# agent-charon/MinGraph-UNet

Hardware: AMD Instinct MI355X
Metric: segmented Mpix/sec, full MinGraph-UNet forward (U-Net + patch-graph GAT), 512x512 batch (higher is better)
Workload: dtype f32

## Files before the change

### include/mgunet.h

```cpp
#ifndef MGUNET_H
#define MGUNET_H

#include <stddef.h>
#include <stdint.h>

#ifdef __cplusplus
extern "C" {
#endif

#define MGU_OK 0
#define MGU_ERR_INVALID -1
#define MGU_ERR_HIP -2
#define MGU_ERR_STATE -3
#define MGU_ERR_NOMEM -4

#define MGU_DTYPE_F32 0
#define MGU_DTYPE_BF16 1

typedef struct mgu_ctx mgu_ctx;

typedef struct {
  const char* name;
  const void* ptr;
  int64_t numel;
} mgu_tensor_desc;

int mgu_create(int device_id, mgu_ctx** out);
void mgu_destroy(mgu_ctx* ctx);
const char* mgu_last_error(mgu_ctx* ctx);
const char* mgu_version(void);

int mgu_unet_configure(mgu_ctx* ctx, int in_channels, int num_classes, int init_features, int depth, int dtype);
int64_t mgu_unet_param_count(mgu_ctx* ctx);
int mgu_unet_load_weights(mgu_ctx* ctx, const mgu_tensor_desc* named, int n, void* hip_stream);
int mgu_unet_refresh_weights(mgu_ctx* ctx, void* hip_stream);

int mgu_unet_workspace_bytes(mgu_ctx* ctx, int B, int H, int W, int training, size_t* out);
int mgu_unet_reserve(mgu_ctx* ctx, int B, int H, int W, int training);
int mgu_unet_forward(mgu_ctx* ctx, const void* x_dev, int B, int H, int W,
                     int64_t xs_n, int64_t xs_c, int64_t xs_h, int64_t xs_w,
                     void* logits_dev, void* const* cat_dev, void* const* feat_dev,
                     int training, void* hip_stream);
int mgu_conv2d_nhwc(mgu_ctx* ctx, const void* in_dev, int B, int H, int W, int Cin, const void* w_oihw_dev,
                    const void* bias_dev, const void* scale_dev, const void* shift_dev, int Cout, int ksize,
                    int relu, void* out_dev, int ld_out, int c_off, void* hip_stream);
typedef struct mgu_conv_weights mgu_conv_weights;
int mgu_conv2d_prepare(mgu_ctx* ctx, const void* w_oihw_dev, int Cout, int Cin, int ksize, mgu_conv_weights** out, void* hip_stream);
void mgu_conv2d_release(mgu_ctx* ctx, mgu_conv_weights* w);
int mgu_conv2d_prepared_nhwc(mgu_ctx* ctx, const mgu_conv_weights* w, const void* in_dev, int B, int H, int W, const void* bias_dev,
                             const void* scale_dev, const void* shift_dev, int relu, void* out_dev, int ld_out, int c_off,
                             void* hip_stream);
int mgu_conv_transpose2x2_nhwc(mgu_ctx* ctx, const void* in_dev, int B, int H, int W, int Cin, const void* w_iohw_dev,
                               const void* bias_dev, int Cout, void* out_dev, int ld_out, int c_off, void* hip_stream);
int mgu_maxpool2x2_nhwc(mgu_ctx* ctx, const void* in_dev, int ld_in, int B, int H, int W, int C, void* out_dev,
                        void* hip_stream);
int mgu_argmax_classes(mgu_ctx* ctx, const void* logits_dev, int64_t npix, int num_classes,
                       int64_t* pred_dev, void* hip_stream);

int64_t mgu_unet_param_offset(mgu_ctx* ctx, const char* name);
int mgu_cross_entropy(mgu_ctx* ctx, const void* logits_dev, const int64_t* labels_dev, int64_t npix, int num_classes,
                      float grad_scale, void* dlogits_dev, float* loss_dev, void* hip_stream);
int mgu_sync_check(mgu_ctx* ctx, void* hip_stream);
int mgu_unet_backward(mgu_ctx* ctx, const void* dlogits_dev, void* flat_grad_dev, void* hip_stream);
int mgu_unet_train_record_dims(mgu_ctx* ctx, const char* layer, int* B_out, int* H_out, int* W_out, int* Cin_out, int* Cout_out);
int mgu_unet_train_record_copy(mgu_ctx* ctx, const char* layer, void* in_dev, void* z_dev, void* y_dev, void* mean_dev, void* invstd_dev,
                               void* hip_stream);
int mgu_conv2d_wgrad_nhwc(mgu_ctx* ctx, const void* in_dev, int ld_in, const void* dz_dev, int B, int H, int W, int Cin, int Cout,
                          int ksize, void* dw_oihw_dev, void* hip_stream);
int mgu_conv2d_dgrad_nhwc(mgu_ctx* ctx, const void* dz_dev, const void* w_oihw_dev, int B, int H, int W, int Cin, int Cout, int ksize,
                          void* din_dev, int ld_out, void* hip_stream);
int mgu_conv_transpose2x2_wgrad_nhwc(mgu_ctx* ctx, const void* in_dev, const void* dout_dev, int ld_d, int c_off, int B, int H, int W,
                                     int Cin, int Cout, void* dw_iohw_dev, void* dbias_dev, void* hip_stream);
int mgu_conv_transpose2x2_dgrad_nhwc(mgu_ctx* ctx, const void* dout_dev, int ld_d, int c_off, const void* w_iohw_dev, int B, int H,
                                     int W, int Cin, int Cout, void* din_dev , void* hip_stream);
int mgu_bn_relu_train_nhwc(mgu_ctx* ctx, const void* z_dev, const void* gamma_dev, const void* beta_dev, int64_t M, int C, void* y_dev,
                           int ld_y, void* mean_dev, void* invstd_dev, void* run_mean_dev, void* run_var_dev, void* hip_stream);
int mgu_bn_relu_backward_nhwc(mgu_ctx* ctx, const void* dy_dev, int ld_dy, const void* z_dev, const void* gamma_dev, const void* beta_dev,
                              const void* mean_dev, const void* invstd_dev, int64_t M, int C, void* dz_dev, void* dgamma_dev,
                              void* dbeta_dev, void* dbias_dev, void* hip_stream);
int mgu_conv_bn_relu_train_nhwc(mgu_ctx* ctx, const void* in_dev, int ld_in, int B, int H, int W, int Cin, const void* w_oihw_dev,
                                const void* bias_dev, const void* gamma_dev, const void* beta_dev, int Cout, void* z_dev, void* y_dev,
                                int ld_y, void* pooled_dev, void* mean_dev, void* invstd_dev, void* run_mean_dev, void* run_var_dev,
                                int* stats_fused_out, int* pool_fused_out, void* hip_stream);
int mgu_bn_relu_conv_backward_nhwc(mgu_ctx* ctx, const void* in_dev, int ld_in, const void* z_dev, const void* dy_dev, int ld_dy,
                                   const void* gamma_dev, const void* beta_dev, const void* mean_dev, const void* invstd_dev,
                                   const void* w_oihw_dev, int B, int H, int W, int Cin, int Cout, void* dz_dev, void* dgamma_dev,
                                   void* dbeta_dev, void* dbias_dev, void* dw_oihw_dev, void* din_dev, int ld_din, void* hip_stream);
int mgu_reduction_slots_absmax(mgu_ctx* ctx, double* absmax_out, void* hip_stream);
int mgu_maxpool2x2_backward_nhwc(mgu_ctx* ctx, const void* y_dev, int ld_y, const void* dpool_dev, void* dskip_dev, int ld_d, int B, int H,
                                 int W, int C, void* hip_stream);

int mgu_adam_step(mgu_ctx* ctx, void* flat_param_dev, const void* flat_grad_dev, void* exp_avg_dev, void* exp_avg_sq_dev,
                  int64_t n, float lr, double beta1, double beta2, float eps, float weight_decay, int step,
                  float grad_scale, void* hip_stream);

int mgu_sgd_step(mgu_ctx* ctx, void* flat_param_dev, const void* flat_grad_dev, void* momentum_buf_dev, int64_t n, float lr,
                 float momentum, float weight_decay, int step, float grad_scale, void* hip_stream);

#define MGU_OPTIM_CTRL_BYTES 64
#define MGU_OPTIM_ADAM 0
#define MGU_OPTIM_ADAMW 1
#define MGU_OPTIM_SGD 2
typedef struct {
  int kind;
  float lr;
  double beta1, beta2;
  float eps, weight_decay;
  float momentum;
  float grad_scale;
  float max_norm;
  int skip_nonfinite;
  float ema_decay;
  int ema_warmup;
} mgu_optim_desc;
int64_t mgu_grad_norm_chunk(int64_t n);
int mgu_grad_norm_blocks(int64_t n);
int mgu_grad_norm(mgu_ctx* ctx, const void* grad_dev, int64_t n, float grad_scale, void* ctrl_dev, void* hip_stream);
int mgu_optim_step(mgu_ctx* ctx, const mgu_optim_desc* desc, void* flat_param_dev, const void* flat_grad_dev, void* exp_avg_dev,
                   void* exp_avg_sq_dev, void* ema_dev, void* ctrl_dev, int64_t n, void* hip_stream);
int mgu_grad_accumulate(mgu_ctx* ctx, void* acc_dev, const void* grad_dev, int64_t n, int first, void* hip_stream);

#define MGU_COMM_ID_BYTES 128
int mgu_comm_get_unique_id(void* id_out );
int mgu_comm_init_rank(mgu_ctx* ctx, const void* id , int rank, int world_size);
int mgu_comm_destroy(mgu_ctx* ctx);
void* mgu_comm_handle(mgu_ctx* ctx);
int mgu_comm_world_size(mgu_ctx* ctx);
int mgu_allreduce_grads(mgu_ctx* ctx, void* flat_grad_dev, int64_t n, void* rccl_comm, void* hip_stream);
int mgu_unet_backward_allreduce(mgu_ctx* ctx, const void* dlogits_dev, void* flat_grad_dev, void* hip_stream);

int mgu_unet_request_patch_mean(mgu_ctx* ctx, int patch, void* out_dev);

int mgu_csr_transpose_device(mgu_ctx* ctx, const int32_t* rowptr_dev, const int32_t* col_dev, int64_t E, int num_nodes,
                             int32_t* rowptr_src_dev, int32_t* eid_src_dev, int32_t* tgt_of_edge_dev, void* hip_stream);
int mgu_gat_layer_backward(mgu_ctx* ctx, const void* X_dev, int N, int Fin, const int32_t* rowptr_dev, const int32_t* col_dev, int64_t E,
                           const int32_t* rowptr_src_dev, const int32_t* eid_src_dev, const int32_t* tgt_of_edge_dev,
                           const int32_t* graph_ptr_dev, int num_graphs, const void* W_dev, const void* a_dev, int heads, int Fout_head,
                           int concat, float alpha, const void* dout_dev, void* dX_dev, void* dW_dev, void* da_dev, void* hip_stream);
int mgu_dropout_mask(mgu_ctx* ctx, unsigned long long seed, unsigned long long stream, int64_t n, float p, void* mask_dev, void* hip_stream);
int mgu_gat_layer_forward_train(mgu_ctx* ctx, const void* X_dev, int N, int Fin, const int32_t* rowptr_dev, const int32_t* col_dev, int64_t E,
                                const int32_t* graph_ptr_dev, int num_graphs, const void* W_dev, const void* a_dev, int heads, int Fout_head,
                                int concat, float alpha, const void* edge_mask_dev, const void* out_mask_dev, void* out_dev, void* hip_stream);
int mgu_gat_layer_backward_train(mgu_ctx* ctx, const void* X_dev, int N, int Fin, const int32_t* rowptr_dev, const int32_t* col_dev, int64_t E,
                                 const int32_t* rowptr_src_dev, const int32_t* eid_src_dev, const int32_t* tgt_of_edge_dev,
                                 const int32_t* graph_ptr_dev, int num_graphs, const void* W_dev, const void* a_dev, int heads, int Fout_head,
                                 int concat, float alpha, const void* edge_mask_dev, const void* out_mask_dev, const void* dout_dev,
                                 void* dX_dev, void* dW_dev, void* da_dev, void* hip_stream);

int mgu_patch_graph_build(int H, int W, int patch, int64_t* coo, int32_t* rowptr, int32_t* col,
                          int64_t* E_out, int* nph_out, int* npw_out);
int mgu_coo_to_csr(const int64_t* coo, int64_t E, int num_nodes, int32_t* rowptr, int32_t* col);
int mgu_coo_to_csr_device(mgu_ctx* ctx, const int64_t* coo_dev, int64_t E, int num_nodes, int32_t* rowptr_dev, int32_t* col_dev,
                          int* status_dev, void* hip_stream);
int mgu_patch_mean(mgu_ctx* ctx, const void* feat_dev, int feat_dtype , int B, int H, int W, int C,
                   int patch, void* out_dev, void* hip_stream);

int mgu_gat_layer_forward(mgu_ctx* ctx, const void* X_dev, int N, int Fin,
                          const int32_t* rowptr_dev, const int32_t* col_dev, int64_t E,
                          const int32_t* graph_ptr_dev, int num_graphs,
                          const void* W_dev, const void* a_dev, int heads, int Fout_head,
                          int concat, float alpha, void* out_dev, void* hip_stream);

typedef struct mgu_gat_weights mgu_gat_weights;
int mgu_gat_prepare(mgu_ctx* ctx, const void* W_dev, const void* a_dev, int heads, int Fout_head, int Fin, int has_edges,
                    mgu_gat_weights** out, void* hip_stream);
void mgu_gat_release(mgu_ctx* ctx, mgu_gat_weights* w);
int mgu_gat_layer_forward_prepared(mgu_ctx* ctx, const mgu_gat_weights* w, const void* X_dev, int N, const int32_t* rowptr_dev,
                                   const int32_t* col_dev, int64_t E, const int32_t* graph_ptr_dev, int num_graphs, int concat,
                                   float alpha, void* out_dev, void* hip_stream);

int mgu_ncut_edge_weights(mgu_ctx* ctx, const float* feats_dev, int N, int D, const int64_t* edge_index_dev, int64_t E,
                          float* w_dev, void* hip_stream);
int mgu_ncut_forward(mgu_ctx* ctx, const float* feats_dev, int N, int D, const int32_t* rowptr_src_dev,
                     const int32_t* col_tgt_dev, int64_t E, const float* assign_dev, int K, int assign_is_logits,
                     float* soft_dev, int32_t* hard_dev, float* loss_dev, void* hip_stream);
int mgu_ncut_backward(mgu_ctx* ctx, const float* feats_dev, int N, int D, const int32_t* rowptr_src_dev, const int32_t* col_tgt_dev,
                      const int32_t* rowptr_tgt_dev, const int32_t* col_src_dev, int64_t E, const float* soft_dev, int K,
                      int assign_is_logits, const float* gloss_dev, const float* gsoft_dev, float* dassign_dev, float* dfeats_dev,
                      void* hip_stream);
int mgu_relu_backward(mgu_ctx* ctx, const float* dy_dev, const float* y_dev, int64_t n, float* dz_dev, void* hip_stream);

int mgu_region_mean_pool(mgu_ctx* ctx, const float* feats_dev, const int32_t* hard_dev, int B, int Np, int D, int K,
                         float* out_dev, void* hip_stream);
int mgu_region_fuse_nhwc(mgu_ctx* ctx, const float* fu_nhwc_dev, int Cu, const float* region_emb_dev, const int32_t* hard_dev,
                         int B, int H, int W, int nph, int npw, int K, int D, float* out_nhwc_dev, void* hip_stream);

int mgu_tv_loss(mgu_ctx* ctx, const void* x_dev, int B, int C, int H, int W, int64_t xs_n, int64_t xs_c, int64_t xs_h, int64_t xs_w,
                float weight, float* loss_dev, void* hip_stream);
int mgu_dice_loss(mgu_ctx* ctx, const void* logits_dev, const int64_t* labels_dev, int B, int64_t HW, int num_classes, int64_t ls_n,
                  int64_t ls_c, int64_t ls_p, float smooth, float* loss_dev, void* hip_stream);
int mgu_feature_consistency_loss(mgu_ctx* ctx, const void* f_unet_dev, const void* f_graph_dev, const void* y_dev, int B, int N, int D,
                                 float margin, float* loss_dev, void* hip_stream);
int mgu_tv_loss_backward(mgu_ctx* ctx, const void* x_dev, int B, int C, int H, int W, int64_t xs_n, int64_t xs_c, int64_t xs_h,
                         int64_t xs_w, float weight, float grad_scale, const float* grad_scale_dev, void* dx_dev, int64_t ds_n,
                         int64_t ds_c, int64_t ds_h, int64_t ds_w, void* hip_stream);
int mgu_dice_loss_backward(mgu_ctx* ctx, const void* logits_dev, const int64_t* labels_dev, int B, int64_t HW, int num_classes,
                           int64_t ls_n, int64_t ls_c, int64_t ls_p, float smooth, float grad_scale, const float* grad_scale_dev,
                           void* dlogits_dev, int64_t ds_n, int64_t ds_c, int64_t ds_p, int accumulate, float* loss_dev, void* hip_stream);
int mgu_feature_consistency_loss_backward(mgu_ctx* ctx, const void* f_unet_dev, const void* f_graph_dev, const void* y_dev, int B, int N,
                                          int D, float margin, float grad_scale, const float* grad_scale_dev, void* d_f_unet_dev,
                                          void* d_f_graph_dev, void* hip_stream);
int mgu_loss_sync_check(mgu_ctx* ctx, void* hip_stream);
int mgu_lovasz_softmax(mgu_ctx* ctx, const void* logits_dev, const int64_t* labels_dev, int B, int64_t HW, int num_classes, int64_t ls_n,
                       int64_t ls_c, int64_t ls_p, int classes_mode, int per_image, int64_t ignore_index, float* loss_dev,
                       float* errors_dev, int32_t* ranks_dev, void* hip_stream);
int mgu_lovasz_softmax_backward(mgu_ctx* ctx, const void* logits_dev, const int64_t* labels_dev, int B, int64_t HW, int num_classes,
                                int64_t ls_n, int64_t ls_c, int64_t ls_p, int classes_mode, int per_image, int64_t ignore_index,
                                float grad_scale, const float* grad_scale_dev, void* dlogits_dev, int64_t ds_n, int64_t ds_c, int64_t ds_p,
                                int accumulate, float* loss_dev, void* hip_stream);
int mgu_lovasz_tile(void);
int mgu_pixel_ce(mgu_ctx* ctx, const void* logits_dev, const int64_t* labels_dev, int B, int64_t HW, int num_classes, int64_t ls_n,
                 int64_t ls_c, int64_t ls_p, const float* class_weight_dev, float label_smoothing, float focal_gamma,
                 double keep_fraction, int64_t min_kept, int per_image, int64_t ignore_index, float* loss_dev, float* pixel_loss_dev,
                 int32_t* kept_dev, void* hip_stream);
int mgu_pixel_ce_backward(mgu_ctx* ctx, const void* logits_dev, const int64_t* labels_dev, int B, int64_t HW, int num_classes,
                          int64_t ls_n, int64_t ls_c, int64_t ls_p, const float* class_weight_dev, float label_smoothing,
                          float focal_gamma, double keep_fraction, int64_t min_kept, int per_image, int64_t ignore_index,
                          float grad_scale, const float* grad_scale_dev, void* dlogits_dev, int64_t ds_n, int64_t ds_c, int64_t ds_p,
                          int accumulate, int zero_to, float* loss_dev, void* hip_stream);
int mgu_pixel_ce_map(mgu_ctx* ctx, const void* logits_dev, const int64_t* labels_dev, int B, int64_t HW, int num_classes, int64_t ls_n,
                     int64_t ls_c, int64_t ls_p, const float* class_weight_dev, const float* pixel_weight_dev, float label_smoothing,
                     float focal_gamma, double keep_fraction, int64_t min_kept, int per_image, int64_t ignore_index, float* loss_dev,
                     float* pixel_loss_dev, int32_t* kept_dev, void* hip_stream);
int mgu_pixel_ce_map_backward(mgu_ctx* ctx, const void* logits_dev, const int64_t* labels_dev, int B, int64_t HW, int num_classes,
                              int64_t ls_n, int64_t ls_c, int64_t ls_p, const float* class_weight_dev, const float* pixel_weight_dev,
                              float label_smoothing, float focal_gamma, double keep_fraction, int64_t min_kept, int per_image,
                              int64_t ignore_index, float grad_scale, const float* grad_scale_dev, void* dlogits_dev, int64_t ds_n,
                              int64_t ds_c, int64_t ds_p, int accumulate, int zero_to, float* loss_dev, void* hip_stream);
int mgu_pixel_ce_tile(void);
int mgu_elliptical_shape_loss_masks(mgu_ctx* ctx, const uint8_t* masks_dev, int num_objects, int H, int W, float epsilon, float* loss_dev,
                                    void* hip_stream);
int mgu_elliptical_shape_loss_probs(mgu_ctx* ctx, const void* probs_dev, int B, int num_classes, int H, int W, int64_t ps_n, int64_t ps_c,
                                    int64_t ps_p, float epsilon, float* loss_dev, void* hip_stream);

int mgu_segmentation_eval(mgu_ctx* ctx, const void* logits_dev, const int64_t* labels_dev, int B, int64_t HW, int num_classes,
                          int64_t* confusion_dev, int64_t* pred_dev, int loss_kind, float dice_smooth, double* loss_acc_dev,
                          void* hip_stream);
int mgu_confusion_matrix(mgu_ctx* ctx, const int64_t* true_dev, const int64_t* pred_dev, int64_t n, int num_classes,
                         int64_t* confusion_dev, void* hip_stream);

int mgu_connected_components(mgu_ctx* ctx, const void* src_dev, int src_kind, int B, int H, int W, int C, int connectivity, int64_t background,
                             int64_t num_classes, int min_area, int32_t* labels_dev, int64_t* counts_dev, int64_t* offsets_dev,
                             void* hip_stream);
int mgu_object_stats(mgu_ctx* ctx, const int32_t* labels_dev, const void* src_dev, int src_kind, int B, int H, int W, int C,
                     const int64_t* offsets_dev, int64_t capacity, int64_t* class_dev, int64_t* area_dev, int32_t* bbox_dev, int64_t* sums_dev,
                     void* hip_stream);
int mgu_match_objects(mgu_ctx* ctx, int B, const int64_t* gt_offsets_dev, const int64_t* gt_class_dev, const int32_t* gt_bbox_dev,
                      int64_t gt_capacity, const int64_t* pred_offsets_dev, const int64_t* pred_class_dev, const int32_t* pred_bbox_dev,
                      int64_t pred_capacity, double iou_thresh, int64_t* totals_dev, void* hip_stream);
int mgu_object_scores(mgu_ctx* ctx, const int32_t* labels_dev, const float* probs_dev, int B, int H, int W, int C, const int64_t* offsets_dev,
                      int64_t capacity, const int64_t* class_dev, const int64_t* area_dev, float* scores_dev, void* hip_stream);

#define MGU_D2_NONE (1 << 30)
int mgu_distance_transform(mgu_ctx* ctx, const int32_t* labels_dev, int B, int H, int W, int32_t* d2_dev, void* hip_stream);
int mgu_split_objects(mgu_ctx* ctx, const int32_t* labels_dev, int B, int H, int W, int min_distance, int64_t min_radius_sq, int min_area,
                      int32_t* labels_out_dev, int64_t* counts_dev, int64_t* offsets_dev, int32_t* d2_out_dev, uint8_t* seeds_out_dev,
                      void* hip_stream);

int mgu_border_weights(mgu_ctx* ctx, const int32_t* labels_dev, int B, int H, int W, const int64_t* classes_dev, const float* class_weight_dev,
                       int num_classes, double w0, double sigma, int64_t background_class, int32_t* d1sq_dev, int32_t* d2sq_dev,
                       int32_t* nearest_dev, float* weight_dev, int64_t* target_dev, void* hip_stream);

int mgu_clean_masks(mgu_ctx* ctx, const void* src_dev, int src_kind, int B, int H, int W, int C, int64_t num_classes, int close_radius_sq,
                    int fill_holes, int64_t max_hole_area, int open_radius_sq, int64_t* out_dev, int64_t* counts_dev, void* hip_stream);

int mgu_boundary_tables(mgu_ctx* ctx, const void* pred_dev, int pred_kind, const int64_t* target_dev, int B, int H, int W, int C,
                        int64_t num_classes, int max_d2, int band_r2, int64_t* hist_dev, int64_t* stats_dev, int64_t* band_dev,
                        void* hip_stream);

int mgu_object_overlaps(mgu_ctx* ctx, const int32_t* gt_labels_dev, const int64_t* gt_offsets_dev, int64_t gt_capacity,
                        const int32_t* pred_labels_dev, const int64_t* pred_offsets_dev, int64_t pred_capacity, int B, int H, int W,
                        int64_t pair_capacity, int64_t* pair_ptr_dev, int64_t* pair_gt_dev, int64_t* pair_inter_dev, int32_t* status_dev,
                        void* hip_stream);
int mgu_match_masks(mgu_ctx* ctx, int B, const int64_t* pair_ptr_dev, const int64_t* pair_gt_dev, const int64_t* pair_inter_dev,
                    int64_t pair_capacity, const int64_t* gt_offsets_dev, const int64_t* gt_class_dev, const int64_t* gt_area_dev,
                    int64_t gt_capacity, const int64_t* pred_offsets_dev, const int64_t* pred_class_dev, const int64_t* pred_area_dev,
                    int64_t pred_capacity, const float* scores_dev, const double* thresholds_dev, int T, int64_t* match_gt_dev,
                    double* match_iou_dev, int64_t* totals_dev, void* hip_stream);
int mgu_panoptic_totals(mgu_ctx* ctx, int B, const int64_t* pair_ptr_dev, const int64_t* pair_gt_dev, const int64_t* pair_inter_dev,
                        int64_t pair_capacity, const int64_t* gt_offsets_dev, const int64_t* gt_class_dev, const int64_t* gt_area_dev,
                        int64_t gt_capacity, const int64_t* pred_offsets_dev, const int64_t* pred_class_dev, const int64_t* pred_area_dev,
                        int64_t pred_capacity, int num_classes, uint64_t* pq_dev, void* hip_stream);

int mgu_object_moments(mgu_ctx* ctx, const int32_t* labels_dev, int B, int H, int W, const int64_t* offsets_dev, int64_t capacity,
                       const int32_t* bbox_dev, uint64_t* moments_dev, void* hip_stream);
int mgu_object_shapes(mgu_ctx* ctx, const int32_t* labels_dev, int B, int H, int W, const int64_t* offsets_dev, int64_t capacity,
                      const int64_t* area_dev, const int32_t* bbox_dev, const int64_t* sums_dev, const uint64_t* moments_dev, float epsilon,
                      int min_pixels, float* centroid_dev, float* cov_dev, float* axes_dev, float* angle_dev, float* fill_dev, float* term_dev,
                      uint8_t* status_dev, void* hip_stream);
int mgu_elliptical_shape_loss_objects(mgu_ctx* ctx, int B, const int64_t* offsets_dev, int64_t capacity, const float* term_dev,
                                      const uint8_t* status_dev, const int64_t* class_dev, int64_t keep_class, float* loss_dev,
                                      void* hip_stream);

int mgu_tta_views(mgu_ctx* ctx, const float* img_dev, int B, int C, int H, int W, const int64_t* in_strides, int G, const int32_t* views,
                  float* out_dev, void* hip_stream);
int mgu_tta_merge(mgu_ctx* ctx, const float* logits0_dev, const float* logits1_dev, int B, int C, int H, int W, int K, const int32_t* views,
                  float* probs_dev, int64_t* labels_dev, float* conf_dev, void* hip_stream);

int mgu_tile_gather(mgu_ctx* ctx, const float* img_dev, int B, int C, int H, int W, const int64_t* in_strides, int Th, int Tw, int overlap_y,
                    int overlap_x, int t0, int n, float* out_dev, void* hip_stream);
int mgu_tile_gather_u8(mgu_ctx* ctx, const uint8_t* img_dev, int B, int H, int W, int bgr, const float* mean3, const float* std3, int Th, int Tw,
                       int overlap_y, int overlap_x, int t0, int n, float* out_dev, void* hip_stream);
int mgu_tile_accumulate(mgu_ctx* ctx, const float* tiles_dev, int is_prob, int B, int C, int H, int W, int Th, int Tw, int overlap_y, int overlap_x,
                        const float* wy_dev, const float* wx_dev, int t0, int n, float* acc_dev,
                        int64_t* labels_dev, float* conf_dev, void* hip_stream);
int mgu_tile_finish(mgu_ctx* ctx, const float* acc_dev, int B, int C, int H, int W, int64_t* labels_dev, float* conf_dev, void* hip_stream);

int mgu_resize_bilinear_nhwc(mgu_ctx* ctx, const void* in_dev, int ld_in, int B, int Hi, int Wi, int C, void* out_dev, int ld_out, int c_off,
                             int Ho, int Wo, void* hip_stream);
int mgu_region_map_gather_nhwc(mgu_ctx* ctx, const float* table_dev, int R, int D, const int64_t* ids_dev, int64_t npix, float* out_dev,
                               int ld_out, int c_off, void* hip_stream);

int mgu_preprocess_image_u8(mgu_ctx* ctx, const uint8_t* img_dev, int Hs, int Ws, int channels , int bgr, int H, int W,
                            const float* mean3, const float* std3, void* out_dev, int64_t os_c, int64_t os_h, int64_t os_w, void* hip_stream);
int mgu_preprocess_mask_u8(mgu_ctx* ctx, const uint8_t* mask_dev, int Hs, int Ws, int H, int W, int num_classes, int64_t* out_dev,
                           void* hip_stream);
int mgu_augment_flip_rotate(mgu_ctx* ctx, const float* img_in, float* img_out, int B, int C, int H, int W, const int64_t* in_strides,
                            const int64_t* out_strides, const float* fill_c, const int64_t* mask_in, int64_t* mask_out, int64_t mask_fill,
                            const int32_t* params_dev, void* hip_stream);
int mgu_preprocess_image_u8_aug(mgu_ctx* ctx, const uint8_t* img_dev, int Hs, int Ws, int channels, int bgr, int H, int W, const float* mean3,
                                const float* std3, void* out_dev, int64_t os_c, int64_t os_h, int64_t os_w, int flip, const int32_t* fix6,
                                void* hip_stream);
int mgu_preprocess_mask_u8_aug(mgu_ctx* ctx, const uint8_t* mask_dev, int Hs, int Ws, int H, int W, int num_classes, int flip, const int32_t* fix6,
                               int64_t mask_fill, int64_t* out_dev, void* hip_stream);
int mgu_augment_affine_color(mgu_ctx* ctx, const uint8_t* img_u8, int B, int Hs, int Ws, int bgr, const uint8_t* mask_u8, int num_classes,
                             float* out, int H, int W, const int64_t* out_strides, const float* mean3, const float* std3,
                             const uint8_t* fill_rgb, int64_t* mask_out, int64_t mask_fill, const int32_t* params_dev, int need_mean,
                             void* hip_stream);
int mgu_augment_luma_tile(void);
int mgu_augment_luma_sums(mgu_ctx* ctx, const uint8_t* img_u8, int B, int Hs, int Ws, int bgr, int64_t* sums_dev, void* hip_stream);
int mgu_sobel_edges_u8(mgu_ctx* ctx, const uint8_t* rgb_dev, int H, int W, uint8_t* out_dev, void* hip_stream);
int mgu_equalize_hist_rgb_u8(mgu_ctx* ctx, const uint8_t* rgb_dev, int H, int W, uint8_t* out_dev, void* hip_stream);
int mgu_patch_mean_u8(mgu_ctx* ctx, const uint8_t* img_dev, int H, int W, int channels, int patch, int per_channel, float* out_dev,
                      void* hip_stream);
int mgu_gaussian_blur_u8(mgu_ctx* ctx, const uint8_t* img_dev, int B, int H, int W, int channels, const int32_t* kx_host, int kw,
                         const int32_t* ky_host, int kh, uint8_t* out_dev, void* hip_stream);
int mgu_patch_smooth_mean_u8(mgu_ctx* ctx, const uint8_t* rgb_dev, int B, int H, int W, int patch, const int32_t* kx_host, int kw,
                             const int32_t* ky_host, int kh, int per_channel, float* out_dev, int ld_out, int col0, void* hip_stream);
int mgu_clahe_u8(mgu_ctx* ctx, const uint8_t* img_dev, int B, int H, int W, int channels, int grid_y, int grid_x, double clip_limit,
                 uint8_t* out_dev, uint8_t* luts_dev, void* hip_stream);
int mgu_patch_clahe_mean_u8(mgu_ctx* ctx, const uint8_t* rgb_dev, int B, int H, int W, int patch, int grid_y, int grid_x, double clip_limit,
                            int per_channel, float* out_dev, int ld_out, int col0, void* hip_stream);
int mgu_refine_probs(mgu_ctx* ctx, const float* src_dev, int is_prob, const uint8_t* guide_dev, int B, int H, int W, int C, int G, int radius,
                     const int32_t* space_lut, const int32_t* range_lut, int shift, int iterations, float* probs_dev, int64_t* labels_dev,
                     float* conf_dev, int64_t* changed_dev, void* hip_stream);
int mgu_slic_labels(mgu_ctx* ctx, const uint8_t* rgb_dev, int B, int H, int W, int step, int mq, int passes, const uint16_t* lin_host,
                    const int32_t* m_host, const uint16_t* f_host, int32_t* raw_labels_dev, int32_t* centres_dev, void* hip_stream);
int mgu_regions_connect(mgu_ctx* ctx, const int32_t* raw_labels_dev, int B, int H, int W, int min_area, int rounds, int32_t* labels_dev,
                        int64_t* counts_dev, int64_t* offsets_dev, void* hip_stream);
int mgu_regions_adjacency(mgu_ctx* ctx, const int32_t* labels_dev, const int64_t* offsets_dev, int B, int H, int W, int64_t node_capacity,
                          int64_t edge_capacity, int32_t* rowptr_dev, int32_t* col_dev, int32_t* border_dev, int32_t* status_dev,
                          void* hip_stream);
int mgu_regions_features_u8(mgu_ctx* ctx, const uint8_t* rgb_dev, const int32_t* labels_dev, const int64_t* offsets_dev, int B, int H, int W,
                            const uint16_t* lin_host, const int32_t* m_host, const uint16_t* f_host, int64_t node_capacity, float* feat_dev,
                            int64_t* stats_dev, void* hip_stream);
int mgu_regions_pool_nhwc(mgu_ctx* ctx, const float* feat_dev, int ld, int c_off, int D, const int32_t* labels_dev, const int64_t* offsets_dev,
                          int B, int H, int W, int64_t node_capacity, float* out_dev, void* hip_stream);
int mgu_patch_node_features_u8(mgu_ctx* ctx, const uint8_t* rgb_dev, int B, int H, int W, int patch, const float* img_dev, int64_t is_n,
                               int64_t is_c, int64_t is_h, int64_t is_w, int repeat, const float* unet_rows_dev, int unet_cols, int per_channel,
                               float* out_dev, int ld_out, void* hip_stream);
int mgu_patch_labels(mgu_ctx* ctx, const void* src_dev, int src_kind, int B, int H, int W, int C, int patch, int32_t* counts_dev,
                     int64_t* labels_dev, float* purity_dev, void* hip_stream);
int mgu_graphcut_rev_index(mgu_ctx* ctx, const int64_t* coo_dev, int64_t E, int num_nodes, const int32_t* rowptr_dev, const int32_t* col_dev,
                           int32_t* rev_dev, int32_t* perm_dev, int* status_dev, void* hip_stream);
int mgu_graphcut_capacities(mgu_ctx* ctx, int B, int N, const int64_t* coo_dev, int64_t E, const float* prior_dev, const int32_t* counts_dev,
                            int num_classes, int fg_class, const float* intensity_dev, const float* feat_dev, int D, float gamma,
                            float sigma_intensity, float sigma_features, float smoothness, float unit, int32_t* cap_source_dev,
                            int32_t* cap_sink_dev, int32_t* cap_edge_dev, void* hip_stream);
int mgu_graphcut_solve(mgu_ctx* ctx, int B, int N, int64_t E, const int32_t* rowptr_dev, const int32_t* col_dev, const int32_t* rev_dev,
                       const int32_t* perm_dev, const int32_t* cap_source_dev, const int32_t* cap_sink_dev, const int32_t* cap_edge_dev,
                       int max_rounds, int relabel_period, int threads, uint8_t* labels_dev, int64_t* flow_dev, int32_t* rounds_dev,
                       int32_t* converged_dev, void* hip_stream);
int mgu_graphcut_energy(mgu_ctx* ctx, int B, int N, const int64_t* coo_dev, int64_t E, const uint8_t* labels_dev, const int32_t* cap_source_dev,
                        const int32_t* cap_sink_dev, const int32_t* cap_edge_dev, int64_t* energy_dev, void* hip_stream);
int mgu_graphcut_label_costs(mgu_ctx* ctx, int64_t rows, int K, const float* prob_dev, const int32_t* counts_dev, float unit, int32_t* costs_dev,
                             void* hip_stream);
int mgu_graphcut_expand(mgu_ctx* ctx, int B, int N, int64_t E, int K, const int32_t* rowptr_dev, const int32_t* col_dev, const int32_t* rev_dev,
                        const int32_t* perm_dev, const int32_t* costs_dev, const int32_t* cap_edge_dev, const uint8_t* init_dev, int max_cycles,
                        int max_rounds, int relabel_period, int threads, uint8_t* labels_dev, int64_t* energy_dev, int32_t* moves_dev,
                        int32_t* accepted_dev, int32_t* rounds_dev, int32_t* converged_dev, void* hip_stream);
int mgu_graphcut_energy_multi(mgu_ctx* ctx, int B, int N, const int64_t* coo_dev, int64_t E, int K, const uint8_t* labels_dev, const int32_t* costs_dev,
                              const int32_t* cap_edge_dev, int64_t* energy_dev, void* hip_stream);
int mgu_colorize_labels(mgu_ctx* ctx, const int64_t* labels_dev, int64_t npix, const uint8_t* palette_dev, int num_classes, uint8_t* vis_dev,
                        uint8_t* labels_u8_dev, void* hip_stream);

int mgu_channel_affine_nhwc(mgu_ctx* ctx, const float* x_dev, int ldx, int64_t M, int C, const float* scale_dev,
                            const float* shift_dev, int act, float* y_dev, int ldy, void* hip_stream);
int mgu_channel_sum_nhwc(mgu_ctx* ctx, const float* x_dev, int ldx, int64_t M, int C, float* out_dev, void* hip_stream);

int mgu_channel_sum_images_nhwc(mgu_ctx* ctx, const float* x_dev, int ldx, int B, int64_t M, int C, float* out_dev, void* hip_stream);

int mgu_frame_sad_tile(void);
int mgu_frame_shifts(mgu_ctx* ctx, const uint8_t* frames_u8, int T, int H, int W, int channels, int bgr, int radius, int factor,
                     int32_t* shifts_dev, int64_t* cost_dev, int64_t* surface_dev, void* hip_stream);
int mgu_track_align(mgu_ctx* ctx, const int32_t* labels_dev, const int64_t* offsets_dev, int64_t capacity, const int32_t* shifts_dev, int T,
                    int H, int W, int32_t* prev_aligned_dev, int32_t* next_cropped_dev, int64_t* vis_prev_dev, int64_t* vis_next_dev,
                    void* hip_stream);
int mgu_track_ids(mgu_ctx* ctx, const int64_t* offsets_dev, int T, int64_t capacity, const int64_t* link_dev, const int64_t* class_dev,
                  const int64_t* first_ids_dev, int64_t* next_id_dev, int64_t* track_id_dev, int32_t* track_len_dev, int64_t* track_class_dev,
                  int64_t track_capacity, int32_t* status_dev, void* hip_stream);

int mgu_mask_runs(mgu_ctx* ctx, const int32_t* labels_dev, const int64_t* offsets_dev, int64_t capacity, int B, int H, int W,
                  int64_t run_capacity, int64_t* run_ptr_dev, int32_t* run_start_dev, int32_t* run_length_dev, int32_t* status_dev,
                  void* hip_stream);
int mgu_runs_to_labels(mgu_ctx* ctx, const int64_t* run_ptr_dev, const int32_t* run_start_dev, const int32_t* run_length_dev,
                       int64_t run_capacity, const int64_t* offsets_dev, int64_t capacity, int B, int H, int W, int32_t* labels_dev,
                       int32_t* status_dev, void* hip_stream);
int mgu_object_outlines(mgu_ctx* ctx, const int32_t* labels_dev, const int64_t* offsets_dev, int64_t capacity, int B, int H, int W,
                        int connectivity, int64_t loop_capacity, int64_t vertex_capacity, int64_t* loop_ptr_dev, int64_t* vertex_ptr_dev,
                        int32_t* vertices_dev, int64_t* loop_area2_dev, int32_t* status_dev, void* hip_stream);
int mgu_polygons_to_labels(mgu_ctx* ctx, const int64_t* loop_ptr_dev, const int64_t* vertex_ptr_dev, const int32_t* vertices_dev,
                           int64_t loop_capacity, int64_t vertex_capacity, const int64_t* offsets_dev, int64_t capacity, int B, int H, int W,
                           int frac_bits, int64_t crossing_capacity, int32_t* labels_dev, int32_t* status_dev, void* hip_stream);

double mgu_unet_flops(mgu_ctx* ctx, int B, int H, int W);
double mgu_unet_mfma_flops(mgu_ctx* ctx, int B, int H, int W);
int mgu_profile_enable(mgu_ctx* ctx, int on);
typedef struct {
  const char* name;
  double ms, flops_alg, flops_mfma;
  int launches, pipe;
} mgu_kernel_stat;
int mgu_profile_read_kernels(mgu_ctx* ctx, mgu_kernel_stat* out, int cap, int* n_out);
int mgu_profile_read(mgu_ctx* ctx, double* conv_ms, int* conv_launches, double* total_ms);
int64_t mgu_convt_asm_launches(mgu_ctx* ctx);

#ifdef __cplusplus
}
#endif
#endif
```

### mingraph-unet_amd/csrc/common.h

```cpp
#pragma once
#include <hip/hip_runtime.h>
#include <stdint.h>

#include "device.h"

namespace mgu {

inline int grid_for(int64_t work, int threads, int cap) {
  int64_t b = (work + threads - 1) / threads;
  if (b < 1) b = 1;
  if (b > cap) b = cap;
  return (int)b;
}
inline bool aligned16(const void* p) { return ((uintptr_t)p & 15) == 0; }

struct Tuning {
  bool first_mfma = true;
  bool use_wino = true;
  int wino_prec = 1;
  bool convt_frag = true;
  bool wino_cp = true;
  int wino_ppb_cap = 32;
  bool wgrad_halo = true;
  bool wino_wgrad = true;
  bool convt_dgrad_x3 = true;
  bool wgrad_x3 = true;
  bool wgrad_thin = true;
  bool wino_dgrad = true;
  bool gat_fused = true;
  bool head_fused = true;
  bool wino_asm = true;
  bool convt_asm = true;
  int fwd_groups = 2;
  int lovasz_passes = 4;
};
const Tuning& default_tuning();
hipError_t ensure_dyn_lds(const void* func, size_t bytes, bool (&done)[64]);

struct IgemmDesc {
  const Tuning* tn;
  const float* in;
  const float* w;
  const float* wu;
  const float* scale;
  const float* shift;
  float* out;
  int M;
  int H, W;
  int Cp;
  int ldin;
  int KS;
  int K;
  int Kp;
  int N;
  int ldout;
  int coff;
  int relu;
  int out_mode;
  int ct_cout;
  int Hout, Wout;
  float* pool;
  int ldpool;
  double* stat_slots;
  int split_n;
  float* out2;
  int ld2;
};

struct WinoHead {
  const float* w;
  const float* b;
  float* logits;
  float* psum;
  int ncls;
  int psum_bytes;
};
inline size_t wino_head_psum_bytes(int B, int H, int W) { return (size_t)B * (H / 16) * (W / 16) * 8 * 32 * sizeof(float); }

inline const Tuning& tun(const IgemmDesc& d) { return d.tn ? *d.tn : default_tuning(); }
enum class ConvKernel {
  None,
  WinoAsmWide, WinoAsmCp1r2, WinoAsmCp1r4,
  WinoAsmCp1r2Head,
  WinoCp2, WinoCp1, WinoCp2Stats, WinoCp1Stats,
  WinoCp1Head,
  WinoF32Wide, WinoF32Narrow,
  WinoX3Wide, WinoX3Narrow,
  HaloF32, HaloBf16Np8, HaloBf16Np4,
  TilesF32, TilesBf16,
  ConvtX3, ConvtBf16f, ConvtX3Dgrad,
  ConvtX3Asm,
};
ConvKernel pick_conv(const IgemmDesc& d, int dtype, const WinoHead* head = nullptr);
hipError_t launch_conv(const IgemmDesc& d, ConvKernel k, int dtype, hipStream_t s, const WinoHead* head = nullptr);
inline bool conv_fuses_head(ConvKernel k) { return k == ConvKernel::WinoAsmCp1r2Head || k == ConvKernel::WinoCp1Head; }
inline hipError_t launch_igemm_f32(const IgemmDesc& d, hipStream_t s) { return launch_conv(d, pick_conv(d, 0), 0, s); }
inline hipError_t launch_igemm_bf16(const IgemmDesc& d, hipStream_t s) { return launch_conv(d, pick_conv(d, 1), 1, s); }
const char* conv_kernel_name(ConvKernel k, const IgemmDesc& d);
const char* conv_dgrad_name(ConvKernel k, const IgemmDesc& d);
struct ConvCost {
  double mfma;
  int pipe;
};
ConvCost conv_cost(ConvKernel k, const IgemmDesc& d);
inline bool conv_is_wino(ConvKernel k) { return k >= ConvKernel::WinoAsmWide && k <= ConvKernel::WinoX3Narrow; }
inline bool conv_fuses_pool(ConvKernel k) {
  return conv_is_wino(k) || (k >= ConvKernel::HaloF32 && k <= ConvKernel::HaloBf16Np4);
}
inline bool conv_reads_panel(ConvKernel k) {
  return !conv_is_wino(k) && k != ConvKernel::ConvtX3 && k != ConvKernel::ConvtX3Asm && k != ConvKernel::ConvtBf16f &&
         k != ConvKernel::ConvtX3Dgrad;
}
inline bool conv_reads_convt_x3(ConvKernel k) {
  return k == ConvKernel::ConvtX3 || k == ConvKernel::ConvtX3Asm;
}
bool wino_layer(const Tuning& t, int KS, int Cp);
bool wino_dgrad_layer(const Tuning& t, int KS, int Cop);
bool convt_x3_layer(const Tuning& t, int Cin, int Cout);
bool convt_x3_dgrad_layer(const Tuning& t, int Cin, int Cout);
bool convt_bf16f_layer(const Tuning& t, int Cin, int Cout);
bool wino_head_layer(const Tuning& t, int dtype, int Cin, int ncls, int patch, int B, int H, int W);
inline bool wino_wide(const IgemmDesc& d) { return d.N > 32; }
struct WinoPlan {
  int tiles_x, tiles_y, total, nblk, ppb, ngroups, per_xcd;
};
WinoPlan wino_plan(const IgemmDesc& d);
int wino_grid_blocks(const IgemmDesc& d);
hipError_t launch_convt_x3(const IgemmDesc& d, hipStream_t s);
bool convt_x3_asm_shape(const IgemmDesc& d);
hipError_t launch_convt_x3_asm(const IgemmDesc& d, hipStream_t s);
hipError_t launch_convt_bf16f(const IgemmDesc& d, hipStream_t s);
hipError_t launch_convt_x3_dgrad(const IgemmDesc& d, hipStream_t s);
bool first_mfma_applicable(int dtype, int Cin, int Cp, int Cout, int ldout, int coff, int64_t H, int64_t W);
hipError_t launch_first_mfma(int dtype, const void* in, const float* wfm, const float* scale, const float* shift, void* out, int B, int H,
                             int W, int ldout, int coff, int relu, hipStream_t s);
hipError_t launch_first_mfma_direct(int dtype, const float* x, int64_t sn, int64_t sc, int64_t sh, int64_t sw, int cin, const float* wfm,
                                    const float* scale, const float* shift, void* out, int B, int H, int W, int ldout, int coff, int relu,
                                    hipStream_t s);
bool first_conv_applicable(int dtype, int Cin, int Cp, int Cout, int ldout, int coff);
hipError_t launch_first_conv(int dtype, const void* in, const float* wf, const float* scale, const float* shift, void* out, int B, int H, int W,
                             int Cin, int Cout, int ldout, int coff, int relu, hipStream_t s);
hipError_t launch_wino_f32(const IgemmDesc& d, ConvKernel k, hipStream_t s, const WinoHead* head = nullptr);
hipError_t launch_patch_sum_combine(const float* psum, float* out, int nodes, hipStream_t s);
hipError_t launch_wino_cp_asm(const IgemmDesc& d, ConvKernel k, hipStream_t s, const WinoHead* head = nullptr);

struct PackItem {
  const float* w;
  float* U;
  int Cout, Cin, Cp, Np, dgrad;
  unsigned blk0;
  int kind;
  int mode;
};
static_assert(sizeof(PackItem) == 48, "PackItem must have no padding");
PackItem pack_wino(const float* w, float* U, int Cout, int Cin, int Cp, int dgrad, int prec);
PackItem pack_first_w(const float* w, float* wf, int Cout, int Cin);
PackItem pack_first_mfma(const float* w, float* wfm, int Cout, int Cin);
PackItem pack_convt_x3(const float* w, float* Wx, int Cin, int Cout, int dgrad);
PackItem pack_bias_tile(const float* bias, float* shift, int C, int reps);
PackItem pack_dgrad_panel(const float* w, float* wp, int Cout, int Cin, int Cop, int KS, int Kp);
PackItem pack_conv_panel(const float* w, void* wp, int dtype, int Cout, int Cin, int Cp, int KS, int Kp);
PackItem pack_convt_panel(const float* w, void* wp, int dtype, int Cin, int Cout, int Kp);
PackItem pack_convt_bf16f(const float* w, float* Wf, int Cin, int Cout);
PackItem pack_convt_dgrad_panel(const float* w, float* wp, int Cin, int Cout, int Kp);
size_t wino_u_floats(int Cout, int Cp);
size_t convt_x3_floats(int Cin, int Cout);
size_t convt_x3_dgrad_floats(int Cin, int Cout);
size_t convt_bf16f_floats(int Cin, int Cout);
size_t first_mfma_floats();
constexpr int PACK_MAX = 64;
struct PackBatch {
  int n;
  unsigned total_blocks;
  PackItem it[PACK_MAX];
};
bool pack_batch_prepare(PackBatch& b);
hipError_t launch_pack_batch(const PackBatch* batch_dev, unsigned total_blocks, hipStream_t s);
hipError_t launch_pack_one(const PackItem& it, hipStream_t s);

struct WgradDesc {
  const Tuning* tn;
  const float* z;
  int ldz, zoff;
  const float* in;
  int ldin, inoff, Cp;
  int KS;
  int M, H, W;
  int Hs, Ws;
  int N, K, Kp;
  float* dw;
  size_t dw_capacity;
  int groups;
  int rows_per_split;
};
inline const Tuning& tun(const WgradDesc& d) { return d.tn ? *d.tn : default_tuning(); }
enum class WgradKernel {
  Thin,
  WinoX3,
  Wino,
  Halo,
  Tiles,
};
WgradKernel pick_wgrad(const WgradDesc& d);
const char* wgrad_kernel_name(WgradKernel k);
struct WgradCost {
  double mfma;
  int pipe;
};
WgradCost wgrad_cost(WgradKernel k, double alg);
hipError_t launch_wgrad_f32(WgradDesc& d, hipStream_t s);
hipError_t launch_wino_wgrad_f32(WgradDesc& d, bool x3, hipStream_t s);
hipError_t launch_wgrad_thin(WgradDesc& d, hipStream_t s);

constexpr int STAT_ROWS = 576;
constexpr int CHAN_REDUCE_ROWS = 512;
size_t chan_reduce_work_bytes(int Cmax);
hipError_t launch_bn_stats(const float* z, int ldz, int64_t M, int C, double* work, double* sums, hipStream_t s);
hipError_t launch_bn_finalize(const double* sum, const double* sumsq, int64_t M, float eps, float momentum,
                              const float* gamma, const float* beta, float* mean, float* invstd, float* scale,
                              float* shift, float* run_mean, float* run_var, int C, hipStream_t s);
hipError_t launch_bn_finalize_slots(double* slots, int nrows, double* sums, int64_t M, float eps, float momentum, const float* gamma,
                                    const float* beta, float* mean, float* invstd, float* scale, float* shift, float* run_mean,
                                    float* run_var, int C, hipStream_t s);
hipError_t launch_bn_apply_relu(const float* z, const float* scale, const float* shift, float* y, int ldy, int64_t M, int C,
                                hipStream_t s);
hipError_t launch_bn_apply_relu_pool(const float* z, const float* scale, const float* shift, float* y, int ldy, float* pooled, int B, int H,
                                     int W, int C, hipStream_t s);
hipError_t launch_bn_bwd_reduce(const float* dy, int lddy, const float* fwd_scale, const float* fwd_shift, const float* z, int ldz,
                                const float* mean, const float* invstd, int64_t M, int C, double* work, double* sums,
                                float* dbeta, float* dgamma, hipStream_t s);
hipError_t launch_bn_bwd_apply(const float* dy, int lddy, const float* fwd_scale, const float* fwd_shift, const float* z, const float* mean,
                               const float* invstd, const float* gamma, const double* sums, int64_t M, int C, float* dz,
                               double* work, float* dbias, hipStream_t s);
hipError_t launch_bn_bwd_apply_deferred(const float* dy, int lddy, const float* fsc, const float* fsh, const float* z, const float* mean,
                                        const float* invstd, const float* gamma, const double* sums, int64_t M, int C, float* dz,
                                        double* work, int* rows, hipStream_t s);
hipError_t launch_colsum(const float* z, int ldz, int64_t M, int C, double* work, float* out, hipStream_t s);
hipError_t launch_maxpool2_bwd_add(const float* y, int ldy, const float* dpool, float* dskip, int ldd, int B, int H, int W,
                                   int C, hipStream_t s);
hipError_t launch_zero_pad_region(float* buf, int ld, int coff, int C, int B, int H, int W, int h2, int w2, hipStream_t s);
hipError_t launch_ce(const float* logits, const int64_t* labels, int64_t M, int C, long long ignore_index, float grad_scale,
                     float* dlogits, int ldd, double* acc, int* err_word, float* loss_out, hipStream_t s);
hipError_t launch_unpack_conv_grad(const float* dwp, int groups, size_t panel_stride, float* g, int Cout, int Cin, int Cp, int KS,
                                   int Kp, hipStream_t s, double* fold_slots = nullptr, int fold_rows = 0, int fold_n = 0, float* fold_out = nullptr);
hipError_t launch_unpack_convt_grad(const float* dwp, int groups, size_t panel_stride, float* g, int Cin, int Cout, int Kp, hipStream_t s);
hipError_t launch_sgd(float* p, const float* g, float* buf, int64_t n, float lr, float momentum, float wd, int step, float grad_scale,
                      hipStream_t s);
hipError_t launch_adam(float* p, const float* g, float* m, float* v, int64_t n, float lr, double b1, double b2, float eps,
                       float wd, int step, float grad_scale, hipStream_t s);

hipError_t launch_pack_input(const float* x, void* out, int dtype, int B, int C, int Cp, int H, int W, int64_t sn, int64_t sc,
                             int64_t sh, int64_t sw, hipStream_t s);
hipError_t launch_maxpool2(const void* in, int ldin, void* out, int dtype, int B, int H, int W, int C, hipStream_t s);
bool patch_mean_head_fusable(int dtype, int C, int ncls);
hipError_t launch_patch_mean(const void* feat, int dtype, float* out, int B, int H, int W, int C, int patch, hipStream_t s,
                             const float* head_w = nullptr, const float* head_b = nullptr, float* logits = nullptr, int ncls = 0);
hipError_t launch_bn_fold(const float* bias, const float* gamma, const float* beta, const float* mean, const float* var,
                          float eps, float* scale, float* shift, int C, hipStream_t s);
hipError_t launch_conv1x1_head(const void* in, int dtype, int ldin, int C, const float* w, const float* bias, float* out,
                               int ldout, int ncls, int64_t npix, hipStream_t s);
hipError_t launch_argmax(const float* logits, int64_t npix, int C, int64_t* pred, hipStream_t s);

hipError_t launch_gat_wa_rows(const float* W, const float* a, float* panel, int row0, int heads, int Fh, int Fin, int Kp, hipStream_t s);
bool gat_fused_applicable(int Fin, int heads, int Fh, int64_t E);
size_t gat_fused_scratch_floats(int Fin, int heads, int Fh);
hipError_t launch_gat_prep(const float* W, const float* a, float* wa, unsigned* Wx, int heads, int Fh, int Fin, hipStream_t s);
hipError_t launch_gat_stmax(const float* x, const float* wa, int N, int Fin, int heads, const int32_t* rowptr, const int32_t* col,
                            const int32_t* gp, int G, float alpha, float* st, int32_t* node_graph, unsigned long long* gmax, int gstride,
                            unsigned gen, hipStream_t s);
hipError_t launch_gat_fused(const float* x, int Fin, const float* st, const int32_t* rowptr, const int32_t* col, const int32_t* gp, int G,
                            const unsigned long long* gmax, const unsigned* Wx, int N, int heads, int Fh, int concat, float alpha, float* out,
                            int gstride, unsigned gen, hipStream_t s);
hipError_t launch_gat_node_graph(const int32_t* gp, int G, int nodes_per_graph, int N, int32_t* node_graph, hipStream_t s);
hipError_t launch_gat_edge_max(const float* st, const int32_t* rowptr, const int32_t* col, const int32_t* node_graph, int N,
                               int heads, float alpha, unsigned long long* gmax_enc, int gstride, unsigned gen, hipStream_t s);
hipError_t launch_gat_aggregate(const float* wh, int P, const float* st, const int32_t* rowptr, const int32_t* col,
                                const int32_t* node_graph, const unsigned long long* gmax_enc, int N, int64_t E, int heads, int Fh,
                                int concat, float alpha, float* out, int gstride, unsigned gen, hipStream_t s);

}
```

### mingraph-unet_amd/csrc/ctx.h

```cpp
#pragma once
#include <stdarg.h>
#include <stdio.h>
#include <stdlib.h>
#include <string.h>

#include <map>
#include <string>
#include <vector>

#include "../../include/mgunet.h"
#include "common.h"

struct Layer {
  std::string prefix;
  std::string conv;
  std::string bn;
  int Cin = 0, Cp = 0, Cout = 0, KS = 3;
  bool convt = false;
  int K = 0, Kp = 0, N = 0, Np = 0;
  float *wp = nullptr, *scale = nullptr, *shift = nullptr;
  bool first = false;
  bool ctb = false;
  bool ctx3 = false;
  bool wino = false;
  mutable bool wp_dirty = false;
  float* wu = nullptr;
  float* wug = nullptr;
  mutable bool wug_valid = false;
  float* wf = nullptr;
  float* wfm = nullptr;
  float* wxg = nullptr;
  mutable bool wxg_valid = false;
  const float *w_src = nullptr, *b_src = nullptr, *gamma = nullptr, *beta = nullptr;
  float *run_mean = nullptr, *run_var = nullptr;
  int64_t off_w = 0, off_b = 0, off_gamma = 0, off_beta = 0;
  float *mean = nullptr, *invstd = nullptr, *tscale = nullptr, *tshift = nullptr;
  int level = 0;
};

struct FwdRecord {
  const float* in = nullptr;
  int ldin = 0;
  float* z = nullptr;
  float* y = nullptr;
  int ldy = 0;
  int B = 0, H = 0, W = 0;
};

struct Block {
  int up = -1;
  int conv1 = 0, conv2 = 0;
  int level = 0;
};

struct mgu_ctx {
  int device = 0;
  mgu::Tuning tn;
  std::string err;
  bool configured = false, loaded = false;
  std::vector<mgu::PackBatch> pack_host;
  mgu::PackBatch* pack_dev = nullptr;
  int pack_dev_cap = 0;
  bool want_train = false;
  bool fold_dirty = false;
  int* err_word = nullptr;
  void* redws = nullptr;
  size_t redws_bytes = 0;
  void* pm_out = nullptr;
  int pm_patch = 0;
  void* pmws = nullptr;
  size_t pmws_bytes = 0;
  void* wuws = nullptr;
  size_t wuws_bytes = 0;
  unsigned long long* gmaxbuf = nullptr;
  int gmax_cap = 0;
  unsigned gmax_gen = 0;
  struct mgu_gat_weights* gat_tmp = nullptr;
  void* lossws = nullptr;
  size_t lossws_bytes = 0;
  void* optws = nullptr;
  size_t optws_bytes = 0;
  void* imgws = nullptr;
  size_t imgws_bytes = 0;
  void* ncws = nullptr;
  size_t ncws_bytes = 0;
  void* objws = nullptr;
  size_t objws_bytes = 0;
  void* labtab = nullptr;
  std::vector<unsigned char> labtab_host;
  int in_ch = 0, ncls = 0, feat = 0, depth = 0, dtype = 0, Cp0 = 0;
  std::vector<Layer> layers;
  std::vector<Block> enc, dec;
  Block bott;
  int head = 0;
  int64_t nparams = 0;
  float* arena = nullptr;
  size_t arena_floats = 0;
  void* ws = nullptr;
  size_t ws_bytes = 0;
  void* gbws = nullptr;
  size_t gbws_bytes = 0;
  void* gws = nullptr;
  size_t gws_bytes = 0;
  void* tws = nullptr;
  size_t tws_bytes = 0;
  bool have_train_fwd = false;
  int tB = 0, tH = 0, tW = 0;
  std::vector<FwdRecord> fwd;
  void* comm = nullptr;
  int comm_world = 1, comm_rank = 0;
  hipStream_t comm_stream = nullptr;
  hipEvent_t comm_ev[16] = {};
  int comm_ev_next = 0;
  bool prof = false;
  std::vector<hipEvent_t> ev;
  struct ProfRec {
    const char* name;
    double alg, mfma;
    int pipe;
  };
  std::vector<ProfRec> prec;
  int ev_used = 0;
  hipEvent_t ev_total[2] = {nullptr, nullptr};
  hipStream_t fwd_stream = nullptr;
  hipEvent_t fwd_ev[2] = {nullptr, nullptr};
  int64_t convt_asm_launches = 0;
  int panel_packs = 0;
};

namespace mgud {

inline int rup(int v, int m) { return (v + m - 1) / m * m; }
extern std::string g_create_err;

inline Layer make_layer(int dtype, int Cin, int Cp, int Cout, int KS, bool convt) {
  Layer L;
  L.Cin = Cin, L.Cp = Cp, L.Cout = Cout, L.KS = KS, L.convt = convt;
  L.K = KS * KS * Cp, L.Kp = rup(L.K, dtype == MGU_DTYPE_BF16 ? 64 : 32);
  L.N = convt ? 4 * Cout : Cout, L.Np = rup(L.N, 128);
  return L;
}

inline int fail(mgu_ctx* c, int code, const char* fmt, ...) {
  char buf[512];
  va_list ap;
  va_start(ap, fmt);
  vsnprintf(buf, sizeof buf, fmt, ap);
  va_end(ap);
  if (c) c->err = buf; else g_create_err = buf;
  return code;
}

#define HIPCHK(c, call)                                                                                       \
  do {                                                                                                        \
    hipError_t e_ = (call);                                                                                   \
    if (e_ != hipSuccess) return mgud::fail(c, MGU_ERR_HIP, "%s failed: %s", #call, hipGetErrorString(e_));   \
  } while (0)

inline int ensure(mgu_ctx* c, void** p, size_t* have, size_t need) {
  if (*have >= need) return MGU_OK;
  if (*p) {
    HIPCHK(c, hipDeviceSynchronize());
    HIPCHK(c, hipFree(*p));
    *p = nullptr;
    *have = 0;
  }
  hipError_t e = hipMalloc(p, need);
  if (e != hipSuccess) return fail(c, MGU_ERR_NOMEM, "hipMalloc(%zu) failed: %s", need, hipGetErrorString(e));
  *have = need;
  return MGU_OK;
}

inline int err_word_dev(mgu_ctx* c, int** dev) {
  if (!c->err_word) {
    HIPCHK(c, hipHostMalloc((void**)&c->err_word, sizeof(int), hipHostMallocMapped));
    *c->err_word = 0;
  }
  HIPCHK(c, hipHostGetDevicePointer((void**)dev, c->err_word, 0));
  return MGU_OK;
}
inline const char* err_word_message(int w) {
  return (w & 2) ? "the GAT backward found no edge whose score equals the forward's graph-wide maximum (mgu_gat_layer_backward): its "
                   "max term was not applied"
                 : "a label outside [0, num_classes) (and != ignore_index -100) reached a loss kernel of this context (mgu_cross_entropy / "
                   "mgu_dice_loss; F.one_hot / CrossEntropyLoss raise on it)";
}

struct Carve {
  size_t off = 0;
  size_t take(size_t bytes) {
    const size_t o = off;
    off += (bytes + 255) / 256 * 256;
    return o;
  }
};

struct ProfScope {
  mgu_ctx* c;
  hipStream_t s;
  int idx = -1;
  ProfScope(mgu_ctx* c_, hipStream_t s_, const char* name = "conv/GEMM", double alg = 0, double mfma = 0, int pipe = -1) : c(c_), s(s_) {
    if (!c || !c->prof) return;
    if ((size_t)c->ev_used >= c->prec.size()) c->prec.resize(c->ev_used + 1);
    c->prec[c->ev_used] = {name, alg, mfma, pipe};
    if ((size_t)(2 * c->ev_used + 2) > c->ev.size()) {
      hipEvent_t a, b;
      if (hipEventCreate(&a) != hipSuccess || hipEventCreate(&b) != hipSuccess) return;
      c->ev.push_back(a);
      c->ev.push_back(b);
    }
    idx = c->ev_used++;
    (void)hipEventRecord(c->ev[2 * idx], s);
  }
  ~ProfScope() {
    if (idx >= 0) (void)hipEventRecord(c->ev[2 * idx + 1], s);
  }
};

inline void level_dims(int H, int W, int depth, std::vector<int>& hs, std::vector<int>& wsz) {
  hs.assign(depth + 1, 0);
  wsz.assign(depth + 1, 0);
  hs[0] = H;
  wsz[0] = W;
  for (int i = 1; i <= depth; ++i) {
    hs[i] = hs[i - 1] / 2;
    wsz[i] = wsz[i - 1] / 2;
  }
}

inline mgu::IgemmDesc layer_desc(const mgu_ctx* c, const Layer& L, const void* in, int ldin, int B, int H, int W, void* out, int ldout, int coff) {
  mgu::IgemmDesc d;
  memset(&d, 0, sizeof d);
  d.tn = &c->tn;
  d.in = (const float*)in;
  d.w = L.wp, d.wu = L.wu, d.out = (float*)out;
  d.M = B * H * W, d.H = H, d.W = W;
  d.Cp = L.Cp, d.ldin = ldin, d.KS = L.KS, d.K = L.K, d.Kp = L.Kp;
  d.N = L.N, d.ldout = ldout, d.coff = coff;
  d.out_mode = L.convt ? 1 : 0, d.ct_cout = L.Cout;
  return d;
}
inline mgu::IgemmDesc dgrad_desc(const mgu_ctx* c, const Layer& L, const FwdRecord& r, const float* dz, int lddz, const float* panel,
                            float* out, int ldout, int Hout = 0, int Wout = 0) {
  const int KS = L.convt ? 2 : L.KS, Cop = rup(L.Cout, 4);
  mgu::IgemmDesc d;
  memset(&d, 0, sizeof d);
  d.tn = &c->tn;
  d.in = dz, d.w = panel, d.out = out;
  d.M = r.B * r.H * r.W, d.H = r.H, d.W = r.W;
  d.Cp = Cop, d.ldin = lddz, d.KS = KS, d.K = KS * KS * Cop, d.Kp = rup(d.K, 32);
  d.N = L.Cin, d.ldout = ldout, d.Hout = Hout, d.Wout = Wout;
  return d;
}
inline mgu::IgemmDesc gemm_desc(const mgu_ctx* c, const float* in, int M, int K, const float* panel, int Kp, int N, float* out, int ldout,
                           int split_n, float* out2, int ld2) {
  mgu::IgemmDesc d;
  memset(&d, 0, sizeof d);
  d.tn = &c->tn;
  d.in = in, d.w = panel, d.out = out;
  d.M = M, d.H = 1, d.W = M;
  d.Cp = K, d.ldin = K, d.KS = 1, d.K = K, d.Kp = Kp;
  d.N = N, d.ldout = ldout;
  d.split_n = split_n, d.out2 = out2, d.ld2 = ld2;
  return d;
}
inline mgu::WgradDesc wgrad_desc(const mgu_ctx* c, const float* z, int ldz, const float* in, int ldin, int inoff, int Cp, int KS, int B, int H,
                            int W, int Hs, int Ws, int N, float* dw, size_t dw_capacity) {
  mgu::WgradDesc d;
  memset(&d, 0, sizeof d);
  d.tn = &c->tn;
  d.z = z, d.ldz = ldz;
  d.in = in, d.ldin = ldin, d.inoff = inoff, d.Cp = Cp;
  d.KS = KS;
  d.M = B * H * W, d.H = H, d.W = W, d.Hs = Hs, d.Ws = Ws;
  d.N = N, d.K = KS * KS * Cp, d.Kp = rup(d.K, 32);
  d.dw = dw, d.dw_capacity = dw_capacity;
  return d;
}

struct ConvReq {
  const void* in = nullptr;
  int ldin = 0, B = 0, H = 0, W = 0;
  void* out = nullptr;
  int ldout = 0, coff = 0, relu = 0;
  const float *scale = nullptr, *shift = nullptr;
  int Hout = 0, Wout = 0;
};
struct ConvFusions {
  void* pool = nullptr;
  int ldpool = 0;
  double* stat_slots = nullptr;
  const mgu::WinoHead* head = nullptr;
};
struct ConvTaken {
  bool pool = false, stats = false, head = false;
  int stat_rows = 0;
};
int run_layer(mgu_ctx* c, const Layer& L, const ConvReq& q, hipStream_t s, const ConvFusions& f = {}, ConvTaken* took = nullptr);
inline int red_cleared_on_error(mgu_ctx* c, int rc, hipStream_t s) {
  if (rc != MGU_OK && c && c->redws) (void)hipMemsetAsync(c->redws, 0, c->redws_bytes, s);
  return rc;
}

void gat_destroy(mgu_ctx* c);
int gat_check_layer(mgu_ctx* c, const char* fn, int Fin, int heads, int Fh, bool train = false, int N = 0);
int gmax_buffer(mgu_ctx* c, const int32_t** graph_ptr, int* num_graphs, int heads, unsigned long long** buf, unsigned* gen);
size_t gat_panel_floats(int heads, int Fh, int Fin);
int gat_pack_panel(mgu_ctx* c, const float* W, const float* a, float* panel, int heads, int Fh, int Fin, bool clear, hipStream_t s);
int gat_prologue(mgu_ctx* c, const float* X, int N, int Fin, const float* panel, int heads, int Fh, const int32_t* rowptr, const int32_t* col,
                 int64_t E, const int32_t* gp, int G, float alpha, unsigned long long* gmax, unsigned gen, float* wh, float* st,
                 int32_t* node_graph, float* gm, bool record, hipStream_t s);

int64_t cc_chunks(int64_t HW);
int cc_roots_i32(mgu_ctx* c, const int32_t* map, int B, int H, int W, int* P, hipStream_t s, bool conn8 = true);
int cc_number_roots(mgu_ctx* c, int* P, unsigned* area, int min_area, int B, int64_t HW, int* cnt, long long* choff, int32_t* labels,
                    int64_t* counts, int64_t* offsets, hipStream_t s);

int comm_bucket(mgu_ctx* c, float* flat, int64_t lo, int64_t hi, hipStream_t s);
int comm_join(mgu_ctx* c, hipStream_t s);

int repack_weights(mgu_ctx* c, hipStream_t s);
struct BwdScratch {
  float *dwp = nullptr, *dgp = nullptr;
  size_t dwp_floats = 0, dgp_floats = 0;
  double *red = nullptr, *sums = nullptr;
  bool clear = false;
};
int conv_dgrad(mgu_ctx* c, const Layer& L, const FwdRecord& r, const float* dz, float* out, int ldout, const BwdScratch& w, bool record,
               hipStream_t s);
int convt_dgrad(mgu_ctx* c, const Layer& U, const FwdRecord& r, const float* dout, int ld_d, int Hout, int Wout, float* out,
                const BwdScratch& w, bool record, hipStream_t s);
int conv_wgrad(mgu_ctx* c, const Layer& L, const FwdRecord& r, const float* dz, float* dw, const BwdScratch& w, bool record, hipStream_t s,
               int* fold_rows = nullptr, float* dbias = nullptr);
int convt_wgrad(mgu_ctx* c, const Layer& U, const FwdRecord& r, const float* dout, int ld_d, int c_off, int Hout, int Wout, float* dw,
                const BwdScratch& w, hipStream_t s);
int ensure_red(mgu_ctx* c, int Cmax);
int conv_bn_relu_train(mgu_ctx* c, const Layer& L, const FwdRecord& r, double* sums, double* red, hipStream_t s, float* pooled = nullptr,
                       ConvTaken* took = nullptr);
struct LayerGrads {
  float *dw = nullptr, *dbias = nullptr, *dgamma = nullptr, *dbeta = nullptr;
};
int conv_bn_relu_backward(mgu_ctx* c, const Layer& L, const FwdRecord& r, const float* dy, int lddy, float* dz, const LayerGrads& g,
                          float* din, int ld_din, const BwdScratch& w, hipStream_t s);
size_t train_ws_bytes(const mgu_ctx* c, int B, int H, int W);
int unet_forward_train(mgu_ctx* c, const float* x, int64_t xs_n, int64_t xs_c, int64_t xs_h, int64_t xs_w, int B, int H,
                       int W, float* logits, void* const* cat_dev, void* const* feat_dev, hipStream_t s);

}
```

### mingraph-unet_amd/csrc/gat_api.hip

```cpp
#include <algorithm>

#include "ctx.h"

using namespace mgu;
using namespace mgud;

struct mgu_gat_weights {
  int heads = 0, Fh = 0, Fin = 0;
  bool fused = false;
  float* buf = nullptr;
};

int mgud::gat_check_layer(mgu_ctx* c, const char* fn, int Fin, int heads, int Fh, bool train, int N) {
  if (heads < 1 || Fh < 4 || (Fh & 3) || Fin < 4 || (Fin & 3))
    return fail(c, MGU_ERR_INVALID, "%s needs Fin %% 4 == 0, Fout_head %% 4 == 0, heads >= 1 (Fin=%d Fout=%d heads=%d)", fn, Fin, Fh, heads);
  const int64_t HF = (int64_t)heads * Fh;
  if (!train && (heads > 32 || HF > 1024))
    return fail(c, MGU_ERR_INVALID, "%s supports heads <= 32 and heads * Fout_head <= 1024 (got %d x %d)", fn, heads, Fh);
  if (train && HF > 256) return fail(c, MGU_ERR_INVALID, "%s supports heads * Fout_head <= 256 (got %d x %d)", fn, heads, Fh);
  if (train && N * HF >= (1ll << 31)) return fail(c, MGU_ERR_INVALID, "%s: N * heads * Fout_head must be < 2^31", fn);
  return MGU_OK;
}

size_t mgud::gat_panel_floats(int heads, int Fh, int Fin) { return (size_t)rup(heads * Fh + 2 * heads, 128) * rup(Fin, 32); }

int mgud::gat_pack_panel(mgu_ctx* c, const float* W, const float* a, float* panel, int heads, int Fh, int Fin, bool clear, hipStream_t s) {
  const int HF = heads * Fh, Kp = rup(Fin, 32);
  if (clear) HIPCHK(c, hipMemsetAsync(panel, 0, gat_panel_floats(heads, Fh, Fin) * sizeof(float), s));
  HIPCHK(c, launch_pack_one(pack_conv_panel(W, panel, 0, HF, Fin, Fin, 1, Kp), s));
  HIPCHK(c, launch_gat_wa_rows(W, a, panel, HF, heads, Fh, Fin, Kp, s));
  return MGU_OK;
}

int mgud::gmax_buffer(mgu_ctx* c, const int32_t** graph_ptr, int* num_graphs, int heads, unsigned long long** buf, unsigned* gen) {
  if (*num_graphs < 1 || !*graph_ptr) *num_graphs = 1, *graph_ptr = nullptr;
  const int need = *num_graphs * heads;
  if (need > c->gmax_cap) {
    const int cap = (std::max(need, 256) + 15) / 16 * 16;
    if (c->gmaxbuf) {
      HIPCHK(c, hipDeviceSynchronize());
      HIPCHK(c, hipFree(c->gmaxbuf));
      c->gmaxbuf = nullptr;
    }
    HIPCHK(c, hipMalloc((void**)&c->gmaxbuf, (size_t)64 * cap * sizeof(unsigned long long)));
    HIPCHK(c, hipMemset(c->gmaxbuf, 0, (size_t)64 * cap * sizeof(unsigned long long)));
    c->gmax_cap = cap, c->gmax_gen = 0;
  }
  if (c->gmax_gen == 0xffffffffu) {
    HIPCHK(c, hipDeviceSynchronize());
    HIPCHK(c, hipMemset(c->gmaxbuf, 0, (size_t)64 * c->gmax_cap * sizeof(unsigned long long)));
    c->gmax_gen = 0;
  }
  *buf = c->gmaxbuf;
  *gen = ++c->gmax_gen;
  return MGU_OK;
}

namespace {

int prepare_into(mgu_ctx* c, mgu_gat_weights* p, const float* W, const float* a, int heads, int Fh, int Fin, int64_t E_hint, hipStream_t s) {
  const bool fused = c->tn.gat_fused && gat_fused_applicable(Fin, heads, Fh, E_hint);
  const bool fresh = !p->buf || p->heads != heads || p->Fh != Fh || p->Fin != Fin || p->fused != fused;
  if (fresh) {
    if (p->buf) {
      HIPCHK(c, hipDeviceSynchronize());
      (void)hipFree(p->buf);
      p->buf = nullptr;
    }
    p->heads = heads, p->Fh = Fh, p->Fin = Fin, p->fused = fused;
    const size_t bytes = (fused ? gat_fused_scratch_floats(Fin, heads, Fh) : gat_panel_floats(heads, Fh, Fin)) * sizeof(float);
    hipError_t e = hipMalloc((void**)&p->buf, bytes);
    if (e != hipSuccess) return fail(c, MGU_ERR_NOMEM, "hipMalloc(%zu) failed: %s", bytes, hipGetErrorString(e));
  }
  if (!fused) return gat_pack_panel(c, W, a, p->buf, heads, Fh, Fin, fresh, s);
  HIPCHK(c, launch_gat_prep(W, a, p->buf, reinterpret_cast<unsigned*>(p->buf + (size_t)2 * heads * Fin), heads, Fh, Fin, s));
  return MGU_OK;
}

void free_weights(mgu_gat_weights* p) {
  if (p->buf) (void)hipFree(p->buf);
  delete p;
}

int forward_prepared(mgu_ctx* c, const mgu_gat_weights* p, const float* X, int N, const int32_t* rowptr, const int32_t* col, int64_t E,
                     const int32_t* graph_ptr, int num_graphs, int concat, float alpha, float* out, hipStream_t s) {
  const int heads = p->heads, Fh = p->Fh, Fin = p->Fin, HF = heads * Fh;
  unsigned long long* gmax;
  unsigned gen;
  int rc = gmax_buffer(c, &graph_ptr, &num_graphs, heads, &gmax, &gen);
  if (rc) return rc;
  Carve cv;
  if (p->fused && E > 0) {
    const size_t o_st = cv.take((size_t)N * 2 * heads * 4);
    if ((rc = ensure(c, &c->gws, &c->gws_bytes, cv.off))) return rc;
    float* st = (float*)((char*)c->gws + o_st);
    int32_t* node_graph = nullptr;
    const float* wa = p->buf;
    const unsigned* wx = reinterpret_cast<const unsigned*>(p->buf + (size_t)2 * heads * Fin);
    {
      ProfScope ps(c, s, "gat_stmax_kernel");
      HIPCHK(c, launch_gat_stmax(X, wa, N, Fin, heads, rowptr, col, graph_ptr, num_graphs, alpha, st, node_graph, gmax, c->gmax_cap, gen, s));
    }
    ProfScope ps(c, s, "gat_fused2_kernel");
    HIPCHK(c, launch_gat_fused(X, Fin, st, rowptr, col, graph_ptr, num_graphs, gmax, wx, N, heads, Fh, concat, alpha, out, c->gmax_cap, gen, s));
    return MGU_OK;
  }
  if (p->fused) return fail(c, MGU_ERR_STATE, "internal: aggregate-first weights on the gather path");
  const size_t o_wh = cv.take((size_t)N * HF * 4), o_st = cv.take((size_t)N * 2 * heads * 4), o_ng = cv.take((size_t)N * 4);
  if ((rc = ensure(c, &c->gws, &c->gws_bytes, cv.off))) return rc;
  char* g = (char*)c->gws;
  float *wh = (float*)(g + o_wh), *st = (float*)(g + o_st);
  int32_t* node_graph = num_graphs > 1 ? (int32_t*)(g + o_ng) : nullptr;
  if ((rc = gat_prologue(c, X, N, Fin, p->buf, heads, Fh, rowptr, col, E, graph_ptr, num_graphs, alpha, gmax, gen, wh, st, node_graph, nullptr,
                         true, s)))
    return rc;
  ProfScope ps(c, s, "gat_aggregate_kernel");
  HIPCHK(c, launch_gat_aggregate(wh, HF, st, rowptr, col, node_graph, gmax, N, E, heads, Fh, concat, alpha, out, c->gmax_cap, gen, s));
  return MGU_OK;
}

}

extern "C" {

int mgu_gat_prepare(mgu_ctx* c, const void* W_dev, const void* a_dev, int heads, int Fout_head, int Fin, int has_edges,
                    mgu_gat_weights** out, void* hip_stream) {
  if (!c) return MGU_ERR_INVALID;
  if (!W_dev || !a_dev || !out) return fail(c, MGU_ERR_INVALID, "NULL buffer");
  int rc = gat_check_layer(c, "mgu_gat_prepare", Fin, heads, Fout_head);
  if (rc) return rc;
  HIPCHK(c, hipSetDevice(c->device));
  mgu_gat_weights* p = new mgu_gat_weights();
  rc = prepare_into(c, p, (const float*)W_dev, (const float*)a_dev, heads, Fout_head, Fin, has_edges ? 1 : 0, (hipStream_t)hip_stream);
  if (rc) {
    free_weights(p);
    return rc;
  }
  *out = p;
  return MGU_OK;
}

void mgu_gat_release(mgu_ctx* c, mgu_gat_weights* p) {
  if (!p) return;
  if (c) (void)hipSetDevice(c->device);
  (void)hipDeviceSynchronize();
  free_weights(p);
}

int mgu_gat_layer_forward_prepared(mgu_ctx* c, const mgu_gat_weights* p, const void* X_dev, int N, const int32_t* rowptr_dev,
                                   const int32_t* col_dev, int64_t E, const int32_t* graph_ptr_dev, int num_graphs, int concat, float alpha,
                                   void* out_dev, void* hip_stream) {
  if (!c) return MGU_ERR_INVALID;
  if (!p || N < 0 || E < 0) return fail(c, MGU_ERR_INVALID, "bad GAT arguments");
  if (N == 0) return MGU_OK;
  if (!X_dev || !rowptr_dev || !out_dev || (E > 0 && !col_dev)) return fail(c, MGU_ERR_INVALID, "NULL buffer");
  if (p->fused && E == 0) return fail(c, MGU_ERR_INVALID, "weights were prepared with has_edges = 1 but the graph has no edges");
  HIPCHK(c, hipSetDevice(c->device));
  return forward_prepared(c, p, (const float*)X_dev, N, rowptr_dev, col_dev, E, graph_ptr_dev, num_graphs, concat, alpha, (float*)out_dev,
                          (hipStream_t)hip_stream);
}

int mgu_gat_layer_forward(mgu_ctx* c, const void* X_dev, int N, int Fin, const int32_t* rowptr_dev, const int32_t* col_dev, int64_t E,
                          const int32_t* graph_ptr_dev, int num_graphs, const void* W_dev, const void* a_dev, int heads,
                          int Fout_head, int concat, float alpha, void* out_dev, void* hip_stream) {
  if (!c) return MGU_ERR_INVALID;
  if (N < 0 || E < 0) return fail(c, MGU_ERR_INVALID, "bad GAT arguments");
  int rc = gat_check_layer(c, "mgu_gat_layer_forward", Fin, heads, Fout_head);
  if (rc) return rc;
  if (N == 0) return MGU_OK;
  if (!X_dev || !rowptr_dev || !W_dev || !a_dev || !out_dev || (E > 0 && !col_dev)) return fail(c, MGU_ERR_INVALID, "NULL buffer");
  HIPCHK(c, hipSetDevice(c->device));
  hipStream_t s = (hipStream_t)hip_stream;
  if (!c->gat_tmp) c->gat_tmp = new mgu_gat_weights();
  if ((rc = prepare_into(c, c->gat_tmp, (const float*)W_dev, (const float*)a_dev, heads, Fout_head, Fin, E, s))) return rc;
  return forward_prepared(c, c->gat_tmp, (const float*)X_dev, N, rowptr_dev, col_dev, E, graph_ptr_dev, num_graphs, concat, alpha,
                          (float*)out_dev, s);
}

}

void mgud::gat_destroy(mgu_ctx* c) {
  if (c->gat_tmp) free_weights(c->gat_tmp);
  c->gat_tmp = nullptr;
  if (c->gmaxbuf) (void)hipFree(c->gmaxbuf);
  c->gmaxbuf = nullptr;
}
```

### mingraph-unet_amd/csrc/gat_fused.hip

```cpp
#include <algorithm>

#include "common.h"
#include <atomic>
#include "gat_common.h"

namespace mgu {


__device__ __forceinline__ int gf_graph_of(const int32_t* __restrict__ gp, int G, int node) {
  int lo = 0, hi = G;
  while (hi - lo > 1) {
    const int mid = (lo + hi) >> 1;
    if (gp[mid] <= node) lo = mid; else hi = mid;
  }
  return lo;
}

template <int CTRL>
__device__ __forceinline__ float dpp_add(float v) {
  return v + __int_as_float(__builtin_amdgcn_update_dpp(0, __float_as_int(v), CTRL, 0xF, 0xF, true));
}
template <int LPN>
__device__ __forceinline__ float node_sum(float v) {
  v = dpp_add<0xB1>(v);
  v = dpp_add<0x4E>(v);
  v = dpp_add<0x104>(v);
  if (LPN == 16) v = dpp_add<0x108>(v);
  return v;
}

template <int FIN, int H>
__global__ __launch_bounds__(256) void gat_stmax_kernel(const float* __restrict__ x, const float* __restrict__ wa, int N,
                                                        const int32_t* __restrict__ rowptr, const int32_t* __restrict__ col,
                                                        const int32_t* __restrict__ gp, int G, float alpha, float* __restrict__ st,
                                                        int32_t* __restrict__ node_graph, gmax_t* __restrict__ gmax, int gstride, unsigned gen) {
  constexpr int LPN = FIN / 4;
  constexpr int NPW = 64 / LPN;
  constexpr int EPT = 4;
  const int lane = threadIdx.x & 63;
  const int q = lane % LPN, ln = lane / LPN;
  const int n = (blockIdx.x * 4 + (threadIdx.x >> 6)) * NPW + ln;
  const bool live = n < N;
  const int nd = live ? n : N - 1;
  f32x4 ws[H], wt[H];
#pragma unroll
  for (int h = 0; h < H; ++h) {
    ws[h] = *reinterpret_cast<const f32x4*>(wa + h * FIN + 4 * q);
    wt[h] = *reinterpret_cast<const f32x4*>(wa + (H + h) * FIN + 4 * q);
  }
  auto dot = [](const f32x4 a, const f32x4 b) { return fmaf(a[0], b[0], fmaf(a[1], b[1], fmaf(a[2], b[2], a[3] * b[3]))); };
  const int k0 = rowptr[nd], deg = (rowptr[nd + 1] - k0) & (live ? -1 : 0);
  const f32x4 xv = *reinterpret_cast<const f32x4*>(x + (size_t)nd * FIN + 4 * q);
  float s[H], t[H], m[H];
#pragma unroll
  for (int h = 0; h < H; ++h) {
    s[h] = node_sum<LPN>(dot(xv, ws[h]));
    t[h] = node_sum<LPN>(dot(xv, wt[h]));
    m[h] = -INFINITY;
  }
  int g = 0;
  if (gp && G > 1) {
    const int n_first = (blockIdx.x * 4 + (threadIdx.x >> 6)) * NPW;
    const int g_first = gf_graph_of(gp, G, min(n_first, N - 1));
    g = g_first;
    if (min(n_first + NPW - 1, N - 1) >= gp[g_first + 1]) g = gf_graph_of(gp, G, nd);
  }
  if (live && q == 0) {
#pragma unroll
    for (int h = 0; h < H; ++h) {
      st[(size_t)n * (2 * H) + h] = s[h];
      st[(size_t)n * (2 * H) + H + h] = t[h];
    }
    if (node_graph) node_graph[n] = g;
  }
  const int maxdeg = (int)wave_max_u32((unsigned)deg);
  for (int e0 = 0; e0 < maxdeg; e0 += EPT) {
    f32x4 xs[EPT];
#pragma unroll
    for (int u = 0; u < EPT; ++u) {
      const int j = col[e0 + u < deg ? k0 + e0 + u : 0];
      xs[u] = *reinterpret_cast<const f32x4*>(x + (size_t)j * FIN + 4 * q);
    }
#pragma unroll
    for (int u = 0; u < EPT; ++u)
#pragma unroll
      for (int h = 0; h < H; ++h) {
        const float sv = node_sum<LPN>(dot(xs[u], ws[h]));
        m[h] = e0 + u < deg ? fmaxf(m[h], sv) : m[h];
      }
  }
  const int g0 = __builtin_amdgcn_readfirstlane(g);
  const bool uniform = __all(g == g0 || !live);
  const int slot = (blockIdx.x * 4 + (threadIdx.x >> 6)) & (GMAX_SLOTS - 1);
  __shared__ float wmax_s[4][H];
  __shared__ int wgraph_s[4];
  const int wv = threadIdx.x >> 6;
  float ew[H];
#pragma unroll
  for (int h = 0; h < H; ++h) {
    float e = -INFINITY;
    if (q == 0 && deg > 0) {
      e = m[h] + t[h];
      e = e > 0.f ? e : alpha * e;
    }
    if (uniform) e = wave_max_f32(e);
    ew[h] = e;
  }
  if (lane == 0) {
    wgraph_s[wv] = uniform ? g0 : -1;
#pragma unroll
    for (int h = 0; h < H; ++h) wmax_s[wv][h] = ew[h];
  }
  constexpr int nwaves = 4;
  __syncthreads();
  bool merged = uniform;
  for (int w2 = 0; w2 < nwaves; ++w2) merged = merged && wgraph_s[w2] == g0;
  if (merged) {
    if (wv == 0 && lane < H) {
      float e = wmax_s[0][lane];
      for (int w2 = 1; w2 < nwaves; ++w2) e = fmaxf(e, wmax_s[w2][lane]);
      if (e > -INFINITY) gmax_add(gmax, gstride, slot, g0 * H + lane, gen, e);
    }
  } else {
#pragma unroll
    for (int h = 0; h < H; ++h) {
      if (uniform) {
        if (lane == 0 && ew[h] > -INFINITY) gmax_add(gmax, gstride, slot, g0 * H + h, gen, ew[h]);
      } else if (ew[h] > -INFINITY) {
        gmax_add(gmax, gstride, slot, g * H + h, gen, ew[h]);
      }
    }
  }
}

hipError_t launch_gat_stmax(const float* x, const float* wa, int N, int Fin, int heads, const int32_t* rowptr, const int32_t* col,
                            const int32_t* gp, int G, float alpha, float* st, int32_t* node_graph, unsigned long long* gmax, int gstride,
                            unsigned gen, hipStream_t s) {
  if (N == 0) return hipSuccess;
  const int npw = 64 / (Fin / 4);
  const dim3 grid((N + 4 * npw - 1) / (4 * npw)), block(256);
#define MGU_SM(FIN, H) hipLaunchKernelGGL((gat_stmax_kernel<FIN, H>), grid, block, 0, s, x, wa, N, rowptr, col, gp, G, alpha, st, node_graph, gmax, gstride, gen)
  if (Fin == 32 && heads == 1) MGU_SM(32, 1);
  else if (Fin == 32 && heads == 2) MGU_SM(32, 2);
  else if (Fin == 32 && heads == 4) MGU_SM(32, 4);
  else if (Fin == 64 && heads == 1) MGU_SM(64, 1);
  else if (Fin == 64 && heads == 2) MGU_SM(64, 2);
  else if (Fin == 64 && heads == 4) MGU_SM(64, 4);
  else return hipErrorInvalidValue;
#undef MGU_SM
  return hipGetLastError();
}

__global__ __launch_bounds__(256) void gat_prep_kernel(const float* __restrict__ W, const float* __restrict__ a, float* __restrict__ wa,
                                                       unsigned* __restrict__ Wx, int heads, int Fh, int Fin, int nb_wx) {
  const int b = blockIdx.x, t = threadIdx.x;
  if (b < 2 * heads) {
    __shared__ float red[256];
    const int which = b / heads, h = b - which * heads;
    const int nfl = 256 / Fin, kl = t % Fin, fl = t / Fin;
    float sum = 0.f;
    if (fl < nfl)
      for (int f = fl; f < Fh; f += nfl) sum += a[h * 2 * Fh + which * Fh + f] * W[(size_t)(h * Fh + f) * Fin + kl];
    red[t] = sum;
    __syncthreads();
    if (fl == 0) {
      float tot = 0.f;
      for (int i = 0; i < nfl; ++i) tot += red[i * Fin + kl];
      wa[b * Fin + kl] = tot;
    }
  } else if (b < 2 * heads + nb_wx) {
    const int i = (b - 2 * heads) * 256 + t;
    const int nks = Fin / 16, nnt = Fh / 32;
    if (i < heads * nnt * nks * 64) {
      const int lane = i & 63, ks = (i >> 6) % nks, item = (i >> 6) / nks;
      const int h = item / nnt, nt = item % nnt;
      const float* wr = W + (size_t)(h * Fh + 32 * nt + (lane & 31)) * Fin + 16 * ks + 8 * (lane >> 5);
      u32x4 p0, p1, p2;
#pragma unroll
      for (int e = 0; e < 4; ++e) {
        unsigned q0, q1, q2;
        split3_pack(wr[2 * e], wr[2 * e + 1], q0, q1, q2);
        p0[e] = q0, p1[e] = q1, p2[e] = q2;
      }
      u32x4* dst = reinterpret_cast<u32x4*>(Wx) + ((size_t)(item * nks + ks) * 3) * 64 + lane;
      dst[0] = p0, dst[64] = p1, dst[128] = p2;
    }
  }
}

size_t gat_fused_scratch_floats(int Fin, int heads, int Fh) { return (size_t)2 * heads * Fin + (size_t)heads * Fh * Fin * 3 / 2 + 64; }

hipError_t launch_gat_prep(const float* W, const float* a, float* wa, unsigned* Wx, int heads, int Fh, int Fin, hipStream_t s) {
  const int nb_wx = (heads * (Fh / 32) * (Fin / 16) * 64 + 255) / 256;
  hipLaunchKernelGGL(gat_prep_kernel, dim3(2 * heads + nb_wx), dim3(256), 0, s, W, a, wa, Wx, heads, Fh, Fin, nb_wx);
  return hipGetLastError();
}


template <int FIN, int NT, int H>
__global__ __launch_bounds__(256, FIN == 32 ? 3 : 2) void gat_fused2_kernel(const float* __restrict__ x, const float* __restrict__ st,
                                                         const int32_t* __restrict__ rowptr, const int32_t* __restrict__ col,
                                                         const int32_t* __restrict__ gp, int G, const gmax_t* __restrict__ gmax,
                                                         const unsigned* __restrict__ Wx, int N, int ntiles, int concat, float alpha,
                                                         float* __restrict__ out, int gstride, unsigned gen) {
  constexpr int LPN = FIN / 4;
  constexpr int NPW = 64 / LPN;
  constexpr int NPP = 4 * NPW;
  constexpr int PASSES = 32 / NPP;
  constexpr int TRIP = FIN == 32 ? 4 : 8;
  constexpr int P2 = 2 * H;
  constexpr int FO = 32 * NT;
  constexpr int KS = FIN / 16;
  constexpr int NG = 4 / NT;
  constexpr int HPW = (H + NG - 1) / NG;
  constexpr int NGE = H < NG ? H : NG;
  static_assert(H == 1 || H == 2 || H == 4, "heads");
  static_assert(NT == 1 || NT == 2, "n tiles");
  using fH = f32x4;
  constexpr int APITCH = FIN * 2 + 16;
  __shared__ __attribute__((aligned(16))) unsigned char agg_s[H][3][32 * APITCH];
  constexpr int RLD = 32 + 4;
  __shared__ __attribute__((aligned(16))) float exch_s[NT][NGE][32 * RLD];
  __shared__ __attribute__((aligned(16))) float wts_s[32][TRIP][4];
  __shared__ __attribute__((aligned(16))) int cols_s[32][TRIP];
  auto load_heads = [](const float* p) {
    fH v = {0.f, 0.f, 0.f, 0.f};
    if constexpr (H == 4) {
      v = *reinterpret_cast<const fH*>(p);
    } else if constexpr (H == 2) {
      const f32x2 t = *reinterpret_cast<const f32x2*>(p);
      v[0] = t[0], v[1] = t[1];
    } else {
      v[0] = p[0];
    }
    return v;
  };
  const int lane = threadIdx.x & 63;
  const int wave = __builtin_amdgcn_readfirstlane(threadIdx.x >> 6);
  const int q = lane % LPN, ln = lane / LPN;
  const int lr = lane & 31, lh = lane >> 5;
  const int wnt = wave % NT, wg = wave / NT;
  const bool gemm_wave = wg < H;

  u32x4 bw[HPW][KS][3];
#pragma unroll
  for (int k = 0; k < HPW; ++k)
#pragma unroll
    for (int ks = 0; ks < KS; ++ks)
#pragma unroll
      for (int pc = 0; pc < 3; ++pc) {
        const int item = min(wg + k * NG, H - 1) * NT + wnt;
        bw[k][ks][pc] = *reinterpret_cast<const u32x4*>(Wx + ((size_t)((item * KS + ks) * 3 + pc) * 64 + lane) * 4);
      }

  const int nwg = gridDim.x, b = blockIdx.x;
  const int xcd = b & 7, wgx = nwg >> 3;
  const int tq = ntiles >> 3, tr = ntiles & 7;
  const int t_begin = xcd < tr ? xcd * (tq + 1) : tr * (tq + 1) + (xcd - tr) * tq;
  const int t_count = tq + (xcd < tr ? 1 : 0);
  int g_cur = 0, g_hi = (gp && G > 1) ? 0 : N;
  int g_cached = -1;
  fH gm_cached = {0.f, 0.f, 0.f, 0.f};
  constexpr bool XPF = FIN == 32;
  struct Meta {
    int rs[PASSES], deg[PASSES], c0[PASSES];
    fH tj[PASSES];
  };
  Meta m_cur, m_nxt, m_nn;
  auto meta_rows = [&](const int n0t, Meta& m, const bool with_t) {
#pragma unroll
    for (int p = 0; p < PASSES; ++p) {
      const int node = n0t + p * NPP + wave * NPW + ln;
      const bool live = node < N;
      const int nd = live ? node : min(n0t, N - 1);
      m.rs[p] = rowptr[nd];
      m.deg[p] = (rowptr[nd + 1] - m.rs[p]) & (live ? -1 : 0);
      if (with_t) m.tj[p] = load_heads(st + (size_t)nd * P2 + H);
    }
  };
  auto meta_t = [&](const int n0t, Meta& m) {
#pragma unroll
    for (int p = 0; p < PASSES; ++p) {
      const int node = n0t + p * NPP + wave * NPW + ln;
      m.tj[p] = load_heads(st + (size_t)(node < N ? node : min(n0t, N - 1)) * P2 + H);
    }
  };
  auto meta_cols = [&](Meta& m) {
#pragma unroll
    for (int p = 0; p < PASSES; ++p) m.c0[p] = col[(q < TRIP && q < m.deg[p]) ? m.rs[p] + q : 0];
  };
  f32x4 xj0[XPF ? PASSES : 1][TRIP];
  fH sj0[XPF ? PASSES : 1];
  auto fetch_rows = [&](const int nl, const int c_own, f32x4 (&xr)[TRIP], fH& sr) {
    if (q < TRIP) cols_s[nl][q] = c_own;
    sr = load_heads(st + (size_t)c_own * P2);
    __builtin_amdgcn_wave_barrier();
    int cs[TRIP];
#pragma unroll
    for (int u4 = 0; u4 < TRIP; u4 += 4) {
      const int4 ca = *reinterpret_cast<const int4*>(&cols_s[nl][u4]);
      cs[u4] = ca.x, cs[u4 + 1] = ca.y, cs[u4 + 2] = ca.z, cs[u4 + 3] = ca.w;
    }
#pragma unroll
    for (int u = 0; u < TRIP; ++u)
      xr[u] = *reinterpret_cast<const f32x4*>(x + (size_t)cs[u] * FIN + 4 * q);
    __builtin_amdgcn_wave_barrier();
  };
  auto fetch_trip0 = [&](const Meta& m) {
    if constexpr (XPF) {
#pragma unroll
      for (int p = 0; p < PASSES; ++p) fetch_rows(p * NPP + wave * NPW + ln, m.c0[p], xj0[p], sj0[p]);
    }
  };
  const int ti0 = b >> 3;
  auto tile_n0 = [&](const int ti) { return (t_begin + min(ti, t_count - 1)) * 32; };
  if (ti0 < t_count) {
    meta_rows(tile_n0(ti0), m_cur, true);
    meta_cols(m_cur);
    meta_rows(tile_n0(ti0 + wgx), m_nxt, true);
    fetch_trip0(m_cur);
    meta_cols(m_nxt);
  }
  m_nn = m_nxt;
  for (int ti = ti0; ti < t_count; ti += wgx) {
    const int n0 = tile_n0(ti);
    meta_rows(tile_n0(ti + 2 * wgx), m_nn, false);
    if (n0 >= g_hi) {
      g_cur = gf_graph_of(gp, G, n0);
      g_hi = gp[g_cur + 1];
    }
    const bool one_graph = min(n0 + 31, N - 1) < g_hi;
    if (one_graph && g_cur != g_cached) {
#pragma unroll
      for (int h = 0; h < H; ++h) gm_cached[h] = gmax_read_wave(gmax, gstride, g_cur * H + h, gen);
      g_cached = g_cur;
    }
#pragma unroll
    for (int p = 0; p < PASSES; ++p) {
      const int nl = p * NPP + wave * NPW + ln;
      const int rs = m_cur.rs[p], deg = m_cur.deg[p];
      const fH tj = m_cur.tj[p];
      fH gm = gm_cached;
      if (!one_graph) {
        const int g = gf_graph_of(gp, G, min(n0 + nl, N - 1));
#pragma unroll
        for (int h = 0; h < H; ++h) gm[h] = gmax_read_lane(gmax, gstride, g * H + h, gen);
      }
      f32x4 acc[H];
      fH D = {0.f, 0.f, 0.f, 0.f};
#pragma unroll
      for (int h = 0; h < H; ++h) acc[h] = f32x4{0.f, 0.f, 0.f, 0.f};
      const int maxdeg = (int)wave_max_u32((unsigned)deg);
      const bool single = maxdeg <= TRIP;
      for (int e0 = 0; e0 < maxdeg; e0 += TRIP) {
        const bool own = q < TRIP && e0 + q < deg;
        f32x4 xj[TRIP];
        fH sj;
        if (XPF && e0 == 0) {
#pragma unroll
          for (int u = 0; u < TRIP; ++u) xj[u] = xj0[XPF ? p : 0][u];
          sj = sj0[XPF ? p : 0];
        } else {
          const int c_own = e0 == 0 ? m_cur.c0[p] : col[own ? rs + e0 + q : 0];
          fetch_rows(nl, c_own, xj, sj);
        }
        fH w = {0.f, 0.f, 0.f, 0.f};
#pragma unroll
        for (int h = 0; h < H; ++h) {
          float ev = sj[h] + tj[h];
          ev = fmaxf(ev, alpha * ev);
          w[h] = own ? __expf(ev - gm[h]) : 0.f;
        }
        if (single) {
#pragma unroll
          for (int h = 0; h < H; ++h) {
            float d = w[h];
            d = dpp_add<0xB1>(d);
            d = dpp_add<0x4E>(d);
            if (TRIP == 8) d = dpp_add<0x141>(d);
            w[h] *= __builtin_amdgcn_rcpf(d + 1e-10f);
          }
        }
        if (q < TRIP) *reinterpret_cast<fH*>(&wts_s[nl][q][0]) = w;
        __builtin_amdgcn_wave_barrier();
#pragma unroll
        for (int u = 0; u < TRIP; ++u) {
          const fH wu = *reinterpret_cast<const fH*>(&wts_s[nl][u][0]);
          if (!single) D += wu;
#pragma unroll
          for (int h = 0; h < H; ++h) acc[h] += wu[h] * xj[u];
        }
        __builtin_amdgcn_wave_barrier();
      }
#pragma unroll
      for (int h = 0; h < H; ++h) {
        f32x4 a = acc[h];
        if (!single) a = a * __builtin_amdgcn_rcpf(D[h] + 1e-10f);
        unsigned p0a, p1a, p2a, p0b, p1b, p2b;
        split3_pack(a[0], a[1], p0a, p1a, p2a);
        split3_pack(a[2], a[3], p0b, p1b, p2b);
        *reinterpret_cast<u32x2*>(&agg_s[h][0][nl * APITCH + 8 * q]) = u32x2{p0a, p0b};
        *reinterpret_cast<u32x2*>(&agg_s[h][1][nl * APITCH + 8 * q]) = u32x2{p1a, p1b};
        *reinterpret_cast<u32x2*>(&agg_s[h][2][nl * APITCH + 8 * q]) = u32x2{p2a, p2b};
      }
    }
    m_cur = m_nxt;
    fetch_trip0(m_cur);
#pragma unroll
    for (int p = 0; p < PASSES; ++p) m_nxt.rs[p] = m_nn.rs[p], m_nxt.deg[p] = m_nn.deg[p];
    meta_t(tile_n0(ti + 2 * wgx), m_nxt);
    lds_barrier_fenced();
    f32x16 c[HPW];
#pragma unroll
    for (int k = 0; k < HPW; ++k)
#pragma unroll
      for (int r = 0; r < 16; ++r) c[k][r] = 0.f;
#pragma unroll
    for (int k = 0; k < HPW; ++k) {
      const int hh = min(wg + k * NG, H - 1);
#pragma unroll
      for (int ks = 0; ks < KS; ++ks) {
        u32x4 pa[3];
#pragma unroll
        for (int pc = 0; pc < 3; ++pc) pa[pc] = *reinterpret_cast<const u32x4*>(&agg_s[hh][pc][lr * APITCH + ks * 32 + lh * 16]);
        f32x16 t = c[k];
        t = mfma_bf16(pa[2], bw[k][ks][0], t);
        t = mfma_bf16(pa[0], bw[k][ks][2], t);
        t = mfma_bf16(pa[1], bw[k][ks][1], t);
        t = mfma_bf16(pa[1], bw[k][ks][0], t);
        t = mfma_bf16(pa[0], bw[k][ks][1], t);
        t = mfma_bf16(pa[0], bw[k][ks][0], t);
        c[k] = t;
      }
    }
    __builtin_amdgcn_sched_barrier(0);
    meta_cols(m_nxt);
    asm volatile("" ::"v"(c[0][0]));
    auto elu = [](const float v) { return v > 0.f ? v : (__expf(v) - 1.f); };
    static_assert(H % NG == 0 || H < NG, "head groups are full");
    const bool full = n0 + 32 <= N;
    int et = threadIdx.x;
    asm volatile("" : "+v"(et));
    const int elr = et & 31, elh = (et >> 5) & 1;
    if (concat) {
      if (gemm_wave) {
#pragma unroll
        for (int k = 0; k < HPW; ++k) {
          const int hh = wg + k * NG;
          float* const o = out + (size_t)n0 * (H * FO) + hh * FO + wnt * 32 + elr;
#pragma unroll
          for (int r4 = 0; r4 < 16; r4 += 4) {
            float v[4];
#pragma unroll
            for (int e = 0; e < 4; ++e) v[e] = elu(c[k][r4 + e]);
#pragma unroll
            for (int e = 0; e < 4; ++e) {
              const int row = e + 8 * (r4 >> 2) + 4 * elh;
              if (full || n0 + row < N) o[(size_t)row * (H * FO)] = v[e];
            }
            __builtin_amdgcn_sched_barrier(0);
          }
        }
      }
      lds_barrier_fenced();
    } else {
      if (gemm_wave) {
#pragma unroll
        for (int r4 = 0; r4 < 16; r4 += 4) {
#pragma unroll
          for (int r = r4; r < r4 + 4; ++r) {
            float sum = elu(c[0][r]);
#pragma unroll
            for (int k = 1; k < HPW; ++k) sum += elu(c[k][r]);
            const int row = (r & 3) + 8 * (r >> 2) + 4 * elh;
            exch_s[wnt][wg][row * RLD + elr] = sum;
          }
          __builtin_amdgcn_sched_barrier(0);
        }
      }
      lds_barrier_fenced();
      constexpr float invH = 1.f / H;
      const int row = et >> 3, qd = et & 7;
#pragma unroll
      for (int nt = 0; nt < NT; ++nt) {
        f32x4 sum = *reinterpret_cast<const f32x4*>(&exch_s[nt][0][row * RLD + 4 * qd]);
#pragma unroll
        for (int g2 = 1; g2 < NGE; ++g2) sum += *reinterpret_cast<const f32x4*>(&exch_s[nt][g2][row * RLD + 4 * qd]);
        if (full || n0 + row < N)
          *reinterpret_cast<f32x4*>(out + (size_t)(n0 + row) * FO + nt * 32 + 4 * qd) = sum * invH;
      }
    }
  }
}

bool gat_fused_applicable(int Fin, int heads, int Fh, int64_t E) {
  return (Fin == 32 || Fin == 64) && (Fh == 32 || Fh == 64) && (heads == 1 || heads == 2 || heads == 4) && Fin <= Fh && E > 0;
}

template <int FIN, int NT, int H>
static hipError_t launch_fused2_t(const float* x, const float* st, const int32_t* rowptr, const int32_t* col, const int32_t* gp, int G,
                                  const unsigned long long* gmax, const unsigned* Wx, int N, int concat, float alpha, float* out, int gstride,
                                  unsigned gen, hipStream_t s) {
  const int ntiles = (N + 31) / 32;
  static std::atomic<int> resident_of[64];
  int dev = 0;
  (void)hipGetDevice(&dev);
  std::atomic<int>& slot = resident_of[dev >= 0 && dev < 64 ? dev : 0];
  int resident = slot.load(std::memory_order_relaxed);
  if (!resident) {
    int cus = 256, occ = 2;
    (void)hipDeviceGetAttribute(&cus, hipDeviceAttributeMultiprocessorCount, dev);
    if (hipOccupancyMaxActiveBlocksPerMultiprocessor(&occ, reinterpret_cast<const void*>(&gat_fused2_kernel<FIN, NT, H>), 256, 0) != hipSuccess || occ < 1)
      occ = 2;
    resident = std::max(8, cus * occ / 8 * 8);
    slot.store(resident, std::memory_order_relaxed);
  }
  const int nwg = std::min((ntiles + 7) / 8 * 8, resident);
  hipLaunchKernelGGL((gat_fused2_kernel<FIN, NT, H>), dim3(nwg), dim3(256), 0, s, x, st, rowptr, col, gp, G, gmax, Wx, N, ntiles,
                     concat, alpha, out, gstride, gen);
  return hipGetLastError();
}

hipError_t launch_gat_fused(const float* x, int Fin, const float* st, const int32_t* rowptr, const int32_t* col, const int32_t* gp, int G,
                            const unsigned long long* gmax, const unsigned* Wx, int N, int heads, int Fh, int concat, float alpha, float* out,
                            int gstride, unsigned gen, hipStream_t s) {
  if (N == 0) return hipSuccess;
#define MGU_GF2(FIN, NT, H) return launch_fused2_t<FIN, NT, H>(x, st, rowptr, col, gp, G, gmax, Wx, N, concat, alpha, out, gstride, gen, s)
#define MGU_GF2_H(FIN, NT)               \
  do {                                   \
    if (heads == 1) MGU_GF2(FIN, NT, 1); \
    if (heads == 2) MGU_GF2(FIN, NT, 2); \
    if (heads == 4) MGU_GF2(FIN, NT, 4); \
  } while (0)
  if (Fin == 32 && Fh == 32) MGU_GF2_H(32, 1);
  if (Fin == 32 && Fh == 64) MGU_GF2_H(32, 2);
  if (Fin == 64 && Fh == 64) MGU_GF2_H(64, 2);
#undef MGU_GF2_H
#undef MGU_GF2
  return hipErrorInvalidValue;
}

}
```

### mingraph-unet_amd/csrc/mgunet_api.hip

```cpp
#include "ctx.h"

#include <algorithm>

using namespace mgu;
using namespace mgud;

namespace mgud {
std::string g_create_err;
}

namespace {

struct WsPlan {
  size_t xin, tmp, tmp_slice, bott, total;
  std::vector<size_t> pooled;
};

int fwd_groups(const mgu_ctx* c, int B) { return c->tn.fwd_groups >= 2 && B >= 2 ? 2 : 1; }
int group_images(const mgu_ctx* c, int B) { return (B + fwd_groups(c, B) - 1) / fwd_groups(c, B); }

WsPlan plan_ws(const mgu_ctx* c, int B, int H, int W) {
  std::vector<int> hs, wsz;
  level_dims(H, W, c->depth, hs, wsz);
  auto out = [&](const Block& b, int l) { return (size_t)B * hs[l] * wsz[l] * c->layers[b.conv2].Cout; };
  WsPlan p;
  Carve k;
  const size_t es = c->dtype == MGU_DTYPE_BF16 ? 2 : 4;
  p.xin = k.take((size_t)B * H * W * c->Cp0 * es);
  size_t tmax = out(c->bott, c->bott.level);
  for (const Block& b : c->enc) tmax = std::max(tmax, out(b, b.level));
  const int G = fwd_groups(c, B);
  p.tmp_slice = (tmax / B * group_images(c, B) * es + 255) / 256 * 256;
  p.tmp = k.take(G == 1 ? tmax * es : G * p.tmp_slice);
  for (const Block& b : c->enc) p.pooled.push_back(k.take(out(b, b.level + 1) * es));
  p.bott = k.take(out(c->bott, c->bott.level) * es);
  p.total = k.off;
  return p;
}

template <class F>
void weight_forms(const mgu_ctx* c, Layer& L, F form) {
  const int dtype = c->dtype;
  L.wino = dtype == MGU_DTYPE_F32 && !L.convt && wino_layer(c->tn, L.KS, L.Cp);
  L.ctx3 = dtype == MGU_DTYPE_F32 && L.convt && convt_x3_layer(c->tn, L.Cin, L.Cout);
  L.ctb = dtype == MGU_DTYPE_BF16 && L.convt && convt_bf16f_layer(c->tn, L.Cin, L.Cout);
  L.first = !L.convt && L.KS == 3 && first_conv_applicable(dtype, L.Cin, L.Cp, L.Cout, 8, 0);
  form(L.wp, (size_t)L.Np * L.Kp);
  form(L.scale, (size_t)L.Np);
  form(L.shift, (size_t)L.Np);
  if (L.wino) form(L.wu, wino_u_floats(L.Cout, L.Cp));
  if (L.wino && rup(L.Cout, 4) % 16 == 0) form(L.wug, wino_u_floats(L.Cin, rup(L.Cout, 4)));
  if (L.ctx3) form(L.wu, convt_x3_floats(L.Cin, L.Cout));
  if (L.ctb) form(L.wu, convt_bf16f_floats(L.Cin, L.Cout));
  if (L.ctx3) form(L.wxg, convt_x3_dgrad_floats(L.Cin, L.Cout));
  if (dtype == MGU_DTYPE_F32 && !L.convt && L.bn.empty())
    form(L.wxg, (size_t)rup(L.Cin, 128) * rup(L.KS * L.KS * rup(L.Cout, 4), 32));
  if (L.first) form(L.wf, 9 * 4 * (size_t)L.Cout);
  if (L.first) form(L.wfm, first_mfma_floats());
  if (!L.bn.empty()) {
    form(L.mean, (size_t)L.Np);
    form(L.invstd, (size_t)L.Np);
    form(L.tscale, (size_t)L.Np);
    form(L.tshift, (size_t)L.Np);
  }
}

}

extern "C" {

const char* mgu_version(void) { return "mgunet 0.2 (gfx950: fp32 Winograd / bf16 MFMA forward, fp32 training step, GAT, RCCL gradient exchange)"; }

int mgu_create(int device_id, mgu_ctx** out) {
  if (!out) return fail(nullptr, MGU_ERR_INVALID, "out == NULL");
  int n = 0;
  hipError_t e = hipGetDeviceCount(&n);
  if (e != hipSuccess || n <= 0)
    return fail(nullptr, MGU_ERR_HIP, "no HIP device available (%s): libmgunet has no CPU fallback",
                e != hipSuccess ? hipGetErrorString(e) : "device count 0");
  if (device_id < 0 || device_id >= n) return fail(nullptr, MGU_ERR_INVALID, "device %d out of range [0,%d)", device_id, n);
  e = hipSetDevice(device_id);
  if (e != hipSuccess) return fail(nullptr, MGU_ERR_HIP, "hipSetDevice: %s", hipGetErrorString(e));
  mgu_ctx* c = new mgu_ctx();
  c->device = device_id;
  auto flag = [](const char* name) { const char* v = getenv(name); return v && v[0] == '1'; };
  auto num = [](const char* name, int dflt) { const char* v = getenv(name); return v && v[0] ? atoi(v) : dflt; };
  Tuning& t = c->tn;
  t.first_mfma = !flag("MGU_NO_FIRST_MFMA");
  t.use_wino = !flag("MGU_NO_WINOGRAD");
  t.wino_prec = num("MGU_WINO_PREC", t.wino_prec) ? 1 : 0;
  t.wino_cp = !flag("MGU_NO_WINO_CP");
  t.convt_frag = !flag("MGU_NO_CONVT_FRAG");
  t.wino_ppb_cap = std::max(1, num("MGU_WINO_PPB_CAP", 32));
  t.wgrad_halo = !flag("MGU_NO_WGRAD_HALO");
  t.wino_wgrad = !flag("MGU_NO_WINO_WGRAD");
  t.wgrad_x3 = !flag("MGU_NO_WGRAD_X3");
  t.convt_dgrad_x3 = !flag("MGU_NO_CONVT_DGRAD_X3");
  t.wgrad_thin = !flag("MGU_NO_THIN_WGRAD");
  t.wino_dgrad = !flag("MGU_NO_WINO_DGRAD");
  t.gat_fused = !flag("MGU_NO_GAT_FUSED");
  t.wino_asm = num("MGU_WINO_ASM", 1) > 0;
  t.convt_asm = num("MGU_CONVT_ASM", 1) > 0;
  t.head_fused = num("MGU_HEAD_FUSED", 1) > 0;
  t.fwd_groups = num("MGU_FWD_GROUPS", t.fwd_groups) >= 2 ? 2 : 1;
  t.lovasz_passes = num("MGU_LOVASZ_PASSES", t.lovasz_passes) == 3 ? 3 : 4;
  *out = c;
  return MGU_OK;
}

void mgu_destroy(mgu_ctx* c) {
  if (!c) return;
  (void)hipSetDevice(c->device);
  (void)hipDeviceSynchronize();
  (void)mgu_comm_destroy(c);
  if (c->arena) (void)hipFree(c->arena);
  if (c->ws) (void)hipFree(c->ws);
  if (c->gws) (void)hipFree(c->gws);
  if (c->pmws) (void)hipFree(c->pmws);
  if (c->gbws) (void)hipFree(c->gbws);
  if (c->pack_dev) (void)hipFree(c->pack_dev);
  if (c->tws) (void)hipFree(c->tws);
  if (c->redws) (void)hipFree(c->redws);
  if (c->wuws) (void)hipFree(c->wuws);
  if (c->ncws) (void)hipFree(c->ncws);
  if (c->objws) (void)hipFree(c->objws);
  if (c->labtab) (void)hipFree(c->labtab);
  if (c->lossws) (void)hipFree(c->lossws);
  if (c->imgws) (void)hipFree(c->imgws);
  if (c->optws) (void)hipFree(c->optws);
  gat_destroy(c);
  if (c->err_word) (void)hipHostFree(c->err_word);
  for (auto e : c->ev) (void)hipEventDestroy(e);
  for (auto e : c->ev_total)
    if (e) (void)hipEventDestroy(e);
  for (auto e : c->fwd_ev)
    if (e) (void)hipEventDestroy(e);
  if (c->fwd_stream) (void)hipStreamDestroy(c->fwd_stream);
  delete c;
}

const char* mgu_last_error(mgu_ctx* c) { return c ? c->err.c_str() : g_create_err.c_str(); }

int mgu_unet_configure(mgu_ctx* c, int in_ch, int ncls, int feat, int depth, int dtype) {
  if (!c) return MGU_ERR_INVALID;
  if (in_ch < 1 || ncls < 1 || feat < 4 || (feat & 3) || depth < 1 || depth > 8)
    return fail(c, MGU_ERR_INVALID, "unsupported UNet(%d,%d,%d,%d): init_features must be a positive multiple of 4, depth 1..8",
                in_ch, ncls, feat, depth);
  if (dtype != MGU_DTYPE_F32 && dtype != MGU_DTYPE_BF16) return fail(c, MGU_ERR_INVALID, "unknown dtype %d", dtype);
  if (dtype == MGU_DTYPE_BF16 && ((feat & 7) || ncls > 4))
    return fail(c, MGU_ERR_INVALID, "bf16 storage needs init_features %% 8 == 0 (16-byte lanes of 8 bf16) and <= 4 classes");
  HIPCHK(c, hipSetDevice(c->device));
  c->in_ch = in_ch, c->ncls = ncls, c->feat = feat, c->depth = depth, c->dtype = dtype;
  c->Cp0 = rup(in_ch, dtype == MGU_DTYPE_BF16 ? 8 : 4);
  c->layers.clear();
  c->enc.clear();
  c->dec.clear();
  auto add = [&](const std::string& prefix, const char* conv, const char* bn, int cin, int cp, int cout, int KS, bool convt, int level) {
    Layer L = make_layer(dtype, cin, cp, cout, KS, convt);
    L.prefix = prefix, L.conv = conv, L.bn = bn, L.level = level;
    c->layers.push_back(L);
    return (int)c->layers.size() - 1;
  };
  auto add_block = [&](const std::string& prefix, int cin, int cp, int cout, int level, int up) {
    Block b;
    b.up = up, b.level = level;
    b.conv1 = add(prefix, "conv1", "bn1", cin, cp, cout, 3, false, level);
    b.conv2 = add(prefix, "conv2", "bn2", cout, cout, cout, 3, false, level);
    return b;
  };
  int cin = in_ch, cp = c->Cp0, f = feat;
  for (int i = 0; i < depth; ++i) {
    c->enc.push_back(add_block("encoder.encoder_blocks." + std::to_string(i) + ".", cin, cp, f, i, -1));
    cin = cp = f;
    f *= 2;
  }
  c->bott = add_block("encoder.bottleneck.", cin, cp, f, depth, -1);
  int prev = f;
  for (int b = 0; b < depth; ++b) {
    const int i = depth - 1 - b, ci = feat << i;
    const std::string prefix = "decoder.decoder_blocks." + std::to_string(b) + ".";
    const int up = add(prefix, "upsample", "", prev, prev, prev / 2, 1, true, i + 1);
    c->dec.push_back(add_block(prefix + "conv_block.", ci + prev / 2, ci + prev / 2, ci, i, up));
    prev = ci;
  }
  c->head = add("decoder.", "final_conv", "", prev, prev, ncls, 1, false, 0);
  c->fwd.assign(c->layers.size(), FwdRecord{});
  {
    int64_t off = 0;
    auto conv = [&](Layer& L) {
      L.off_w = off, off += (int64_t)L.Cout * L.Cin * L.KS * L.KS * (L.convt ? 4 : 1);
      L.off_b = off, off += L.Cout;
    };
    auto bn = [&](Layer& L) {
      L.off_gamma = off, off += L.Cout;
      L.off_beta = off, off += L.Cout;
    };
    auto block = [&](const Block& b) {
      if (b.up >= 0) conv(c->layers[b.up]);
      conv(c->layers[b.conv1]), conv(c->layers[b.conv2]);
      bn(c->layers[b.conv1]), bn(c->layers[b.conv2]);
    };
    for (const Block& b : c->enc) block(b);
    block(c->bott);
    for (const Block& b : c->dec) block(b);
    conv(c->layers[c->head]);
    c->nparams = off;
  }
  size_t total = 0;
  for (auto& L : c->layers) weight_forms(c, L, [&](float*&, size_t n) { total += n; });
  if (c->arena) HIPCHK(c, hipFree(c->arena));
  c->arena = nullptr;
  HIPCHK(c, hipMalloc((void**)&c->arena, total * sizeof(float)));
  HIPCHK(c, hipMemset(c->arena, 0, total * sizeof(float)));
  c->arena_floats = total;
  float* p = c->arena;
  for (auto& L : c->layers) weight_forms(c, L, [&](float*& form, size_t n) { form = p, p += n; });
  c->configured = true;
  c->have_train_fwd = false;
  c->loaded = false;
  return MGU_OK;
}

int64_t mgu_unet_param_count(mgu_ctx* c) {
  if (!c || !c->configured) return -1;
  return c->nparams;
}

int64_t mgu_unet_param_offset(mgu_ctx* c, const char* name) {
  if (!c || !c->configured || !name) return -1;
  const std::string key(name);
  for (auto& L : c->layers) {
    if (key == L.prefix + L.conv + ".weight") return L.off_w;
    if (key == L.prefix + L.conv + ".bias") return L.off_b;
    if (!L.bn.empty()) {
      if (key == L.prefix + L.bn + ".weight") return L.off_gamma;
      if (key == L.prefix + L.bn + ".bias") return L.off_beta;
    }
  }
  return -1;
}

int mgu_unet_load_weights(mgu_ctx* c, const mgu_tensor_desc* named, int n, void* hip_stream) {
  if (!c) return MGU_ERR_INVALID;
  if (!c->configured) return fail(c, MGU_ERR_STATE, "mgu_unet_configure must precede mgu_unet_load_weights");
  if (!named || n <= 0) return fail(c, MGU_ERR_INVALID, "empty state_dict");
  HIPCHK(c, hipSetDevice(c->device));
  hipStream_t s = (hipStream_t)hip_stream;
  std::map<std::string, const mgu_tensor_desc*> sd;
  for (int i = 0; i < n; ++i)
    if (named[i].name) sd[named[i].name] = &named[i];
  auto get = [&](const std::string& key, int64_t numel, const float** out) -> int {
    auto it = sd.find(key);
    if (it == sd.end()) return fail(c, MGU_ERR_INVALID, "state_dict is missing key '%s'", key.c_str());
    if (it->second->numel != numel)
      return fail(c, MGU_ERR_INVALID, "state_dict key '%s' has %lld elements, expected %lld", key.c_str(),
                  (long long)it->second->numel, (long long)numel);
    if (!it->second->ptr) return fail(c, MGU_ERR_INVALID, "state_dict key '%s' has a NULL pointer", key.c_str());
    *out = (const float*)it->second->ptr;
    return MGU_OK;
  };
  for (auto& L : c->layers) {
    const float *w, *b;
    const std::string cw = L.prefix + L.conv;
    int rc;
    if (L.convt) {
      if ((rc = get(cw + ".weight", (int64_t)L.Cin * L.Cout * 4, &w))) return rc;
      if ((rc = get(cw + ".bias", L.Cout, &b))) return rc;
      L.w_src = w, L.b_src = b;
    } else {
      if ((rc = get(cw + ".weight", (int64_t)L.Cout * L.Cin * L.KS * L.KS, &w))) return rc;
      if ((rc = get(cw + ".bias", L.Cout, &b))) return rc;
      L.w_src = w, L.b_src = b;
      if (!L.bn.empty()) {
        const float *g, *be, *rm, *rv;
        const std::string bn = L.prefix + L.bn;
        if ((rc = get(bn + ".weight", L.Cout, &g))) return rc;
        if ((rc = get(bn + ".bias", L.Cout, &be))) return rc;
        if ((rc = get(bn + ".running_mean", L.Cout, &rm))) return rc;
        if ((rc = get(bn + ".running_var", L.Cout, &rv))) return rc;
        L.gamma = g, L.beta = be, L.run_mean = const_cast<float*>(rm), L.run_var = const_cast<float*>(rv);
      }
    }
  }
  int rc = repack_weights(c, s);
  if (rc) return rc;
  c->loaded = true;
  return MGU_OK;
}

int mgu_unet_refresh_weights(mgu_ctx* c, void* hip_stream) {
  if (!c) return MGU_ERR_INVALID;
  if (!c->configured || !c->loaded) return fail(c, MGU_ERR_STATE, "mgu_unet_refresh_weights needs a preceding mgu_unet_load_weights");
  HIPCHK(c, hipSetDevice(c->device));
  return repack_weights(c, (hipStream_t)hip_stream);
}

int mgu_unet_workspace_bytes(mgu_ctx* c, int B, int H, int W, int training, size_t* out) {
  if (!c || !out) return MGU_ERR_INVALID;
  if (!c->configured) return fail(c, MGU_ERR_STATE, "not configured");
  *out = training ? train_ws_bytes(c, B, H, W) : plan_ws(c, B, H, W).total;
  return MGU_OK;
}

int mgu_unet_reserve(mgu_ctx* c, int B, int H, int W, int training) {
  size_t need = 0;
  int rc = mgu_unet_workspace_bytes(c, B, H, W, training, &need);
  if (rc) return rc;
  HIPCHK(c, hipSetDevice(c->device));
  return training ? ensure(c, &c->tws, &c->tws_bytes, need) : ensure(c, &c->ws, &c->ws_bytes, need);
}

}

int mgud::repack_weights(mgu_ctx* c, hipStream_t s) {
  std::vector<PackItem> items;
  for (auto& L : c->layers) {
    const float *w = L.w_src, *b = L.b_src;
    L.wxg_valid = false;
    if (L.convt) {
      L.wp_dirty = L.ctx3;
      if (!L.ctx3) items.push_back(pack_convt_panel(w, L.wp, c->dtype, L.Cin, L.Cout, L.Kp));
      if (L.ctb) items.push_back(pack_convt_bf16f(w, L.wu, L.Cin, L.Cout));
      if (L.ctx3) items.push_back(pack_convt_x3(w, L.wu, L.Cin, L.Cout, 0));
      items.push_back(pack_bias_tile(b, L.shift, L.Cout, 4));
      if (L.wxg && c->want_train && convt_x3_dgrad_layer(c->tn, L.Cin, L.Cout)) {
        items.push_back(pack_convt_x3(w, L.wxg, L.Cin, L.Cout, 1));
        L.wxg_valid = true;
      }
    } else {
      L.wp_dirty = true;
      if (L.wu) items.push_back(pack_wino(w, L.wu, L.Cout, L.Cin, L.Cp, 0, c->tn.wino_prec));
      L.wug_valid = false;
      if (L.wug && c->want_train && wino_dgrad_layer(c->tn, L.KS, rup(L.Cout, 4))) {
        items.push_back(pack_wino(w, L.wug, L.Cin, L.Cout, rup(L.Cout, 4), 1, c->tn.wino_prec));
        L.wug_valid = true;
      }
      const bool head_kernel = L.bn.empty() && c->ncls <= 4;
      if (!L.wu && !L.first && !head_kernel) {
        items.push_back(pack_conv_panel(w, L.wp, c->dtype, L.Cout, L.Cin, L.Cp, L.KS, L.Kp));
        L.wp_dirty = false;
      }
      if (L.wf) items.push_back(pack_first_w(w, L.wf, L.Cout, L.Cin));
      if (L.wfm && L.Cout == 32 && L.Cin <= 3) items.push_back(pack_first_mfma(w, L.wfm, L.Cout, L.Cin));
      if (!L.bn.empty()) c->fold_dirty = true;
      else items.push_back(pack_bias_tile(b, L.shift, L.Cout, 1));
      if (L.bn.empty() && L.wxg && c->want_train) {
        const int Cop = rup(L.Cout, 4);
        items.push_back(pack_dgrad_panel(w, L.wxg, L.Cout, L.Cin, Cop, L.KS, rup(L.KS * L.KS * Cop, 32)));
        L.wxg_valid = true;
      }
    }
  }
  std::vector<PackBatch> batches;
  for (size_t i0 = 0; i0 < items.size(); i0 += PACK_MAX) {
    PackBatch b;
    memset(&b, 0, sizeof b);
    b.n = (int)std::min<size_t>(PACK_MAX, items.size() - i0);
    for (int i = 0; i < b.n; ++i) b.it[i] = items[i0 + i];
    if (!pack_batch_prepare(b)) return fail(c, MGU_ERR_STATE, "internal: a weight form is not packable");
    batches.push_back(b);
  }
  const bool same = batches.size() == c->pack_host.size() &&
                    (batches.empty() || memcmp(batches.data(), c->pack_host.data(), batches.size() * sizeof(PackBatch)) == 0);
  if (!same) {
    if ((int)batches.size() > c->pack_dev_cap) {
      if (c->pack_dev) HIPCHK(c, hipFree(c->pack_dev));
      c->pack_dev = nullptr;
      HIPCHK(c, hipMalloc((void**)&c->pack_dev, batches.size() * sizeof(PackBatch)));
      c->pack_dev_cap = (int)batches.size();
    }
    HIPCHK(c, hipStreamSynchronize(s));
    HIPCHK(c, hipMemcpy(c->pack_dev, batches.data(), batches.size() * sizeof(PackBatch), hipMemcpyHostToDevice));
    c->pack_host = batches;
  }
  for (size_t k = 0; k < batches.size(); ++k) HIPCHK(c, launch_pack_batch(c->pack_dev + k, batches[k].total_blocks, s));
  return MGU_OK;
}

int mgud::run_layer(mgu_ctx* c, const Layer& L, const ConvReq& q, hipStream_t s, const ConvFusions& f, ConvTaken* took) {
  IgemmDesc d = layer_desc(c, L, q.in, q.ldin, q.B, q.H, q.W, q.out, q.ldout, q.coff);
  d.scale = q.scale, d.shift = q.shift, d.relu = q.relu, d.Hout = q.Hout, d.Wout = q.Wout;
  ConvTaken t;
  if (took) *took = t;
  if (L.wfm && c->tn.first_mfma && q.ldin == L.Cp && first_mfma_applicable(c->dtype, L.Cin, L.Cp, L.Cout, q.ldout, q.coff, q.H, q.W)) {
    const double alg = 2.0 * d.M * 9.0 * L.Cin * L.Cout;
    ProfScope ps(c, s, "conv3x3_first_mfma_kernel", alg, 2.0 * d.M * 32.0 * 32.0 * (c->dtype == MGU_DTYPE_F32 ? 6.0 : 3.0), 1);
    HIPCHK(c, launch_first_mfma(c->dtype, q.in, L.wfm, q.scale, q.shift, q.out, q.B, q.H, q.W, q.ldout, q.coff, q.relu, s));
    return MGU_OK;
  }
  if (L.wf && q.ldin == L.Cp && first_conv_applicable(c->dtype, L.Cin, L.Cp, L.Cout, q.ldout, q.coff) &&
      (int64_t)q.B * q.H * q.W * std::max(q.ldout, 8) < (1ll << 31)) {
    ProfScope ps(c, s, "conv3x3_first_kernel", 2.0 * d.M * 9.0 * L.Cin * L.Cout, 0, -1);
    HIPCHK(c, launch_first_conv(c->dtype, q.in, L.wf, q.scale, q.shift, q.out, q.B, q.H, q.W, L.Cin, L.Cout, q.ldout, q.coff, q.relu, s));
    return MGU_OK;
  }
  ConvKernel k = pick_conv(d, c->dtype, f.head);
  if (f.stat_slots && conv_is_wino(k) && wino_grid_blocks(d) <= STAT_ROWS) {
    d.stat_slots = f.stat_slots;
    t.stats = true, t.stat_rows = wino_grid_blocks(d);
  }
  if (f.pool && conv_fuses_pool(k)) {
    d.pool = (float*)f.pool, d.ldpool = f.ldpool;
    t.pool = true;
  }
  if (d.stat_slots || d.pool) k = pick_conv(d, c->dtype, f.head);
  t.head = conv_fuses_head(k);
  const WinoHead* head = t.head ? f.head : nullptr;
  if (took) *took = t;
  if (L.wp_dirty && conv_reads_panel(k)) {
    HIPCHK(c, launch_pack_one(L.convt ? pack_convt_panel(L.w_src, L.wp, c->dtype, L.Cin, L.Cout, L.Kp)
                                      : pack_conv_panel(L.w_src, L.wp, c->dtype, L.Cout, L.Cin, L.Cp, L.KS, L.Kp), s));
    L.wp_dirty = false;
    ++c->panel_packs;
  }
  double alg = L.convt ? 2.0 * d.M * (double)L.Cin * L.Cout * 4.0 : 2.0 * d.M * (double)L.KS * L.KS * L.Cin * L.Cout;
  if (head) alg += 2.0 * d.M * (double)L.Cout * head->ncls;
  const ConvCost cost = conv_cost(k, d);
  ProfScope ps(c, s, conv_kernel_name(k, d), alg, cost.mfma, cost.pipe);
  HIPCHK(c, launch_conv(d, k, c->dtype, s, head));
  c->convt_asm_launches += k == ConvKernel::ConvtX3Asm;
  return MGU_OK;
}

extern "C" {

int mgu_unet_forward(mgu_ctx* c, const void* x_dev, int B, int H, int W, int64_t xs_n, int64_t xs_c, int64_t xs_h,
                     int64_t xs_w, void* logits_dev, void* const* cat_dev, void* const* feat_dev, int training,
                     void* hip_stream) {
  if (!c) return MGU_ERR_INVALID;
  if (!c->configured || !c->loaded) return fail(c, MGU_ERR_STATE, "configure + load_weights must precede forward");
  if (!x_dev || !logits_dev || !cat_dev || !feat_dev) return fail(c, MGU_ERR_INVALID, "NULL buffer");
  const int depth = c->depth;
  if (B < 1 || H < (1 << depth) || W < (1 << depth))
    return fail(c, MGU_ERR_INVALID, "input %dx%dx%d too small for depth %d", B, H, W, depth);
  if ((int64_t)B * H * W >= (1ll << 31)) return fail(c, MGU_ERR_INVALID, "B*H*W must be < 2^31");
  for (int i = 0; i < depth; ++i)
    if (!cat_dev[i] || !feat_dev[i]) return fail(c, MGU_ERR_INVALID, "NULL cat/feat buffer %d", i);
  HIPCHK(c, hipSetDevice(c->device));
  hipStream_t s = (hipStream_t)hip_stream;
  if (training && c->dtype != MGU_DTYPE_F32)
    return fail(c, MGU_ERR_STATE, "training runs in fp32 only (bf16 storage is an inference mode)");
  if (training) {
    int rc = unet_forward_train(c, (const float*)x_dev, xs_n, xs_c, xs_h, xs_w, B, H, W, (float*)logits_dev, cat_dev, feat_dev, s);
    if (rc == MGU_OK && c->pm_out) {
      ProfScope ps(c, s, "patch_mean_kernel", 0, 0, -1);
      HIPCHK(c, launch_patch_mean(feat_dev[0], 0, (float*)c->pm_out, B, H, W, c->feat, c->pm_patch, s));
      c->pm_out = nullptr;
    }
    return rc;
  }
  const WsPlan plan = plan_ws(c, B, H, W);
  int rc = ensure(c, &c->ws, &c->ws_bytes, plan.total);
  if (rc) return rc;
  const Layer& F = c->layers[c->head];
  WinoHead head_args{};
  bool head_done = false;
  const bool head_wanted = c->pm_out && F.w_src && F.b_src && wino_head_layer(c->tn, c->dtype, F.Cin, c->ncls, c->pm_patch, B, H, W);
  if (head_wanted) {
    if ((rc = ensure(c, &c->pmws, &c->pmws_bytes, wino_head_psum_bytes(B, H, W)))) return rc;
    head_args = WinoHead{F.w_src, F.b_src, (float*)logits_dev, (float*)c->pmws, c->ncls, (int)wino_head_psum_bytes(B, H, W)};
  }
  if (c->fold_dirty) {
    for (auto& L : c->layers)
      if (!L.bn.empty()) HIPCHK(c, launch_bn_fold(L.b_src, L.gamma, L.beta, L.run_mean, L.run_var, 1e-5f, L.scale, L.shift, L.Cout, s));
    c->fold_dirty = false;
  }
  char* ws = (char*)c->ws;
  const size_t es = c->dtype == MGU_DTYPE_BF16 ? 2 : 4;
  void* xin = ws + plan.xin;
  void* bott = ws + plan.bott;
  std::vector<int> hs, wsz;
  level_dims(H, W, depth, hs, wsz);

  if (c->prof) {
    for (auto& e : c->ev_total)
      if (!e) HIPCHK(c, hipEventCreate(&e));
    HIPCHK(c, hipEventRecord(c->ev_total[0], s));
  }

  for (const Block& b : c->enc) {
    const int i = b.level;
    if (2 * hs[i + 1] != hs[i] || 2 * wsz[i + 1] != wsz[i])
      HIPCHK(c, hipMemsetAsync(cat_dev[i], 0, (size_t)B * hs[i] * wsz[i] * 2 * c->layers[b.conv2].Cout * es, s));
  }

  const Layer& L0 = c->layers[c->enc[0].conv1];
  const bool first_direct = L0.wfm && c->tn.first_mfma && first_mfma_applicable(c->dtype, L0.Cin, L0.Cp, L0.Cout, c->feat, 0, H, W) &&
                            (int64_t)B * H * W < (1ll << 31);
  if (!first_direct) HIPCHK(c, launch_pack_input((const float*)x_dev, xin, c->dtype, B, c->in_ch, c->Cp0, H, W, xs_n, xs_c, xs_h, xs_w, s));

  auto walk = [&](hipStream_t gs, int img0, int nb, void* tmp, bool* head_done) -> int {
    auto at = [&](const void* base, int level, int ch) { return (char*)base + (size_t)img0 * hs[level] * wsz[level] * ch * es; };
    WinoHead head = head_args;
    if (head_wanted) {
      head.logits += (size_t)img0 * H * W * c->ncls;
      head.psum = (float*)((char*)head.psum + wino_head_psum_bytes(img0, H, W));
      head.psum_bytes = (int)wino_head_psum_bytes(nb, H, W);
    }
    auto conv = [&](int l, int lvl, ConvReq q, const ConvFusions& f = {}, ConvTaken* took = nullptr) {
      const Layer& L = c->layers[l];
      q.B = nb, q.H = hs[lvl], q.W = wsz[lvl], q.scale = L.bn.empty() ? nullptr : L.scale, q.shift = L.shift;
      return run_layer(c, L, q, gs, f, took);
    };
    const void* cur = at(xin, 0, c->Cp0);
    int cur_ld = c->Cp0;
    for (const Block& b : c->enc) {
      const int i = b.level, C = c->layers[b.conv1].Cout;
      if (&b == &c->enc.front() && first_direct) {
        if (c->fold_dirty) return fail(c, MGU_ERR_STATE, "internal: eval scale/shift not folded");
        const double alg = 2.0 * nb * H * W * 9.0 * L0.Cin * L0.Cout;
        ProfScope ps(c, gs, "conv3x3_first_mfma_kernel", alg, 2.0 * nb * H * W * 32.0 * 32.0 * (c->dtype == MGU_DTYPE_F32 ? 6.0 : 3.0), 1);
        HIPCHK(c, launch_first_mfma_direct(c->dtype, (const float*)x_dev + (int64_t)img0 * xs_n, xs_n, xs_c, xs_h, xs_w, c->in_ch, L0.wfm,
                                           L0.bn.empty() ? nullptr : L0.scale, L0.shift, tmp, nb, H, W, C, 0, 1, gs));
      } else if ((rc = conv(b.conv1, i, {.in = cur, .ldin = cur_ld, .out = tmp, .ldout = C, .relu = 1}))) return rc;
      void *cat = at(cat_dev[i], i, 2 * C), *pooled = at(ws + plan.pooled[i], i + 1, C);
      ConvTaken took;
      if ((rc = conv(b.conv2, i, {.in = tmp, .ldin = C, .out = cat, .ldout = 2 * C, .relu = 1}, {.pool = pooled, .ldpool = C}, &took))) return rc;
      if (!took.pool) {
        ProfScope ps(c, gs, "maxpool2", 0, 0, -1);
        HIPCHK(c, launch_maxpool2(cat, 2 * C, pooled, c->dtype, nb, hs[i], wsz[i], C, gs));
      }
      cur = pooled, cur_ld = C;
    }
    {
      const Block& b = c->bott;
      const int i = b.level, C = c->layers[b.conv1].Cout;
      if ((rc = conv(b.conv1, i, {.in = cur, .ldin = cur_ld, .out = tmp, .ldout = C, .relu = 1}))) return rc;
      if ((rc = conv(b.conv2, i, {.in = tmp, .ldin = C, .out = at(bott, i, C), .ldout = C, .relu = 1}))) return rc;
      cur = at(bott, i, C), cur_ld = C;
    }
    for (const Block& b : c->dec) {
      const int i = b.level, C = c->layers[b.conv1].Cout;
      const bool last = head_wanted && i == 0;
      void *cat = at(cat_dev[i], i, 2 * C), *feat = at(feat_dev[i], i, C);
      if ((rc = conv(b.up, i + 1, {.in = cur, .ldin = cur_ld, .out = cat, .ldout = 2 * C, .coff = C, .Hout = hs[i], .Wout = wsz[i]}))) return rc;
      if ((rc = conv(b.conv1, i, {.in = cat, .ldin = 2 * C, .out = tmp, .ldout = C, .relu = 1}))) return rc;
      ConvTaken took;
      if ((rc = conv(b.conv2, i, {.in = tmp, .ldin = C, .out = feat, .ldout = C, .relu = 1}, {.head = last ? &head : nullptr}, &took))) return rc;
      if (last) *head_done = took.head;
      cur = feat, cur_ld = C;
    }
    return MGU_OK;
  };
  const int G = c->prof ? 1 : fwd_groups(c, B);
  if (G == 1) {
    if ((rc = walk(s, 0, B, ws + plan.tmp, &head_done))) return rc;
  } else {
    if (!c->fwd_stream) HIPCHK(c, hipStreamCreateWithFlags(&c->fwd_stream, hipStreamNonBlocking));
    for (auto& e : c->fwd_ev)
      if (!e) HIPCHK(c, hipEventCreateWithFlags(&e, hipEventDisableTiming));
    const int n0 = group_images(c, B), packs = c->panel_packs;
    bool done1 = false;
    HIPCHK(c, hipEventRecord(c->fwd_ev[0], s));
    HIPCHK(c, hipStreamWaitEvent(c->fwd_stream, c->fwd_ev[0], 0));
    rc = walk(s, 0, n0, ws + plan.tmp, &head_done);
    if (rc == MGU_OK && c->panel_packs != packs) {
      HIPCHK(c, hipEventRecord(c->fwd_ev[0], s));
      HIPCHK(c, hipStreamWaitEvent(c->fwd_stream, c->fwd_ev[0], 0));
    }
    const int rc1 = rc == MGU_OK ? walk(c->fwd_stream, n0, B - n0, ws + plan.tmp + plan.tmp_slice, &done1) : MGU_OK;
    HIPCHK(c, hipEventRecord(c->fwd_ev[1], c->fwd_stream));
    HIPCHK(c, hipStreamWaitEvent(s, c->fwd_ev[1], 0));
    if (rc || rc1) return rc ? rc : rc1;
    if (done1 != head_done) return fail(c, MGU_ERR_STATE, "internal: the image groups disagree on the head-fused kernel");
  }
  const void* cur = feat_dev[0];
  const int cur_ld = c->layers[c->dec.back().conv1].Cout;
  {
    const int pm_dtype = c->dtype;
    if (head_done) {
      ProfScope ps(c, s, "patch_sum_combine_kernel", 0, 0, -1);
      HIPCHK(c, launch_patch_sum_combine((const float*)c->pmws, (float*)c->pm_out, B * (H / 16) * (W / 16), s));
      c->pm_out = nullptr;
    } else if (c->pm_out && F.w_src && F.b_src && patch_mean_head_fusable(pm_dtype, F.Cin, c->ncls) && F.Cin <= 256) {
      ProfScope ps(c, s, "patch_mean_kernel (1x1 head + patch means)", 2.0 * B * H * W * F.Cin * c->ncls, 0, -1);
      HIPCHK(c, launch_patch_mean(cur, pm_dtype, (float*)c->pm_out, B, H, W, F.Cin, c->pm_patch, s, F.w_src, F.b_src,
                                  (float*)logits_dev, c->ncls));
      c->pm_out = nullptr;
    } else if (c->ncls <= 4 && F.w_src && F.b_src) {
      ProfScope ps(c, s, "conv1x1_head_kernel", 2.0 * B * H * W * F.Cin * c->ncls, 0, -1);
      HIPCHK(c, launch_conv1x1_head(cur, c->dtype, cur_ld, F.Cin, F.w_src, F.b_src, (float*)logits_dev, c->ncls, c->ncls,
                                    (int64_t)B * H * W, s));
    } else if ((rc = run_layer(c, F, {.in = cur, .ldin = cur_ld, .B = B, .H = H, .W = W, .out = logits_dev, .ldout = c->ncls, .shift = F.shift}, s))) {
      return rc;
    }
  }
  if (c->pm_out) {
    ProfScope ps(c, s, "patch_mean_kernel", 0, 0, -1);
    HIPCHK(c, launch_patch_mean(cur, c->dtype, (float*)c->pm_out, B, H, W, F.Cin, c->pm_patch, s));
    c->pm_out = nullptr;
  }
  if (c->prof) HIPCHK(c, hipEventRecord(c->ev_total[1], s));
  return MGU_OK;
}

int mgu_unet_request_patch_mean(mgu_ctx* c, int patch, void* out_dev) {
  if (!c) return MGU_ERR_INVALID;
  if (!c->configured) return fail(c, MGU_ERR_STATE, "not configured");
  if (!out_dev) {
    c->pm_out = nullptr;
    return MGU_OK;
  }
  if (patch < 1) return fail(c, MGU_ERR_INVALID, "bad patch_mean request");
  const int C = c->layers[c->head].Cin, vec = c->dtype == MGU_DTYPE_BF16 ? 8 : 4;
  if ((C % vec) || C > 256) return fail(c, MGU_ERR_INVALID, "patch means need init_features %% %d == 0 and <= 256 (got %d)", vec, C);
  c->pm_patch = patch;
  c->pm_out = out_dev;
  return MGU_OK;
}

struct mgu_conv_weights {
  Layer L;
};

static int conv2d_launch(mgu_ctx* c, const Layer& L, const void* in_dev, int B, int H, int W, const void* bias_dev, const void* scale_dev,
                         const void* shift_dev, int relu, void* out_dev, int ld_out, int c_off, hipStream_t s) {
  IgemmDesc d = layer_desc(c, L, in_dev, L.Cin, B, H, W, out_dev, ld_out, c_off);
  d.relu = relu;
  if (scale_dev && shift_dev) {
    d.scale = (const float*)scale_dev;
    d.shift = (const float*)shift_dev;
  } else if (bias_dev) {
    HIPCHK(c, launch_pack_one(pack_bias_tile((const float*)bias_dev, L.shift, L.Cout, 1), s));
    d.shift = L.shift;
  }
  const ConvKernel k = pick_conv(d, 0);
  ProfScope ps(c, s, conv_kernel_name(k, d));
  HIPCHK(c, launch_conv(d, k, 0, s));
  return MGU_OK;
}

int mgu_conv2d_prepare(mgu_ctx* c, const void* w_dev, int Cout, int Cin, int ksize, mgu_conv_weights** out, void* hip_stream) {
  if (!c) return MGU_ERR_INVALID;
  if (!w_dev || !out || Cout < 1 || (ksize != 1 && ksize != 3)) return fail(c, MGU_ERR_INVALID, "bad conv2d_prepare args (ksize must be 1 or 3)");
  if (Cin < 4 || (Cin & 3)) return fail(c, MGU_ERR_INVALID, "conv2d needs Cin %% 4 == 0 (got %d)", Cin);
  HIPCHK(c, hipSetDevice(c->device));
  hipStream_t s = (hipStream_t)hip_stream;
  mgu_conv_weights* p = new mgu_conv_weights();
  Layer& L = p->L;
  L = make_layer(MGU_DTYPE_F32, Cin, Cin, Cout, ksize, false);
  const bool wino = wino_layer(c->tn, ksize, Cin);
  const size_t panel = (size_t)L.Np * L.Kp, total = panel + L.Np + (wino ? wino_u_floats(Cout, Cin) : 0);
  hipError_t e = hipMalloc((void**)&L.wp, total * sizeof(float));
  if (e != hipSuccess) {
    delete p;
    return fail(c, MGU_ERR_NOMEM, "hipMalloc(%zu) failed: %s", total * sizeof(float), hipGetErrorString(e));
  }
  L.shift = L.wp + panel;
  e = hipMemsetAsync(L.wp, 0, (panel + L.Np) * sizeof(float), s);
  if (e == hipSuccess) e = launch_pack_one(pack_conv_panel((const float*)w_dev, L.wp, 0, Cout, Cin, Cin, ksize, L.Kp), s);
  if (e == hipSuccess && wino) {
    L.wu = L.shift + L.Np;
    e = launch_pack_one(pack_wino((const float*)w_dev, L.wu, Cout, Cin, Cin, 0, c->tn.wino_prec), s);
  }
  if (e != hipSuccess) {
    (void)hipFree(L.wp);
    delete p;
    return fail(c, MGU_ERR_HIP, "conv2d_prepare: %s", hipGetErrorString(e));
  }
  *out = p;
  return MGU_OK;
}

void mgu_conv2d_release(mgu_ctx* c, mgu_conv_weights* p) {
  if (!p) return;
  if (c) (void)hipSetDevice(c->device);
  (void)hipDeviceSynchronize();
  if (p->L.wp) (void)hipFree(p->L.wp);
  delete p;
}

int mgu_conv2d_prepared_nhwc(mgu_ctx* c, const mgu_conv_weights* p, const void* in_dev, int B, int H, int W, const void* bias_dev,
                             const void* scale_dev, const void* shift_dev, int relu, void* out_dev, int ld_out, int c_off,
                             void* hip_stream) {
  if (!c) return MGU_ERR_INVALID;
  if (!p || !in_dev || !out_dev || B < 1 || H < 1 || W < 1) return fail(c, MGU_ERR_INVALID, "bad conv2d args");
  if (ld_out < c_off + p->L.Cout) return fail(c, MGU_ERR_INVALID, "ld_out %d < c_off %d + Cout %d", ld_out, c_off, p->L.Cout);
  if ((int64_t)B * H * W >= (1ll << 31)) return fail(c, MGU_ERR_INVALID, "B*H*W must be < 2^31");
  HIPCHK(c, hipSetDevice(c->device));
  return conv2d_launch(c, p->L, in_dev, B, H, W, bias_dev, scale_dev, shift_dev, relu, out_dev, ld_out, c_off, (hipStream_t)hip_stream);
}

int mgu_conv2d_nhwc(mgu_ctx* c, const void* in_dev, int B, int H, int W, int Cin, const void* w_dev, const void* bias_dev,
                    const void* scale_dev, const void* shift_dev, int Cout, int ksize, int relu, void* out_dev,
                    int ld_out, int c_off, void* hip_stream) {
  if (!c) return MGU_ERR_INVALID;
  if (!in_dev || !w_dev || !out_dev || B < 1 || H < 1 || W < 1 || Cout < 1 || (ksize != 1 && ksize != 3))
    return fail(c, MGU_ERR_INVALID, "bad conv2d args (ksize must be 1 or 3)");
  if (Cin < 4 || (Cin & 3)) return fail(c, MGU_ERR_INVALID, "conv2d needs Cin %% 4 == 0 (got %d)", Cin);
  if (ld_out < c_off + Cout) return fail(c, MGU_ERR_INVALID, "ld_out %d < c_off %d + Cout %d", ld_out, c_off, Cout);
  if ((int64_t)B * H * W >= (1ll << 31)) return fail(c, MGU_ERR_INVALID, "B*H*W must be < 2^31");
  HIPCHK(c, hipSetDevice(c->device));
  hipStream_t s = (hipStream_t)hip_stream;
  Layer L = make_layer(MGU_DTYPE_F32, Cin, Cin, Cout, ksize, false);
  const size_t need = ((size_t)L.Np * L.Kp + 2 * (size_t)L.Np) * sizeof(float);
  int rc = ensure(c, &c->gws, &c->gws_bytes, need);
  if (rc) return rc;
  L.wp = (float*)c->gws;
  L.shift = L.wp + (size_t)L.Np * L.Kp + L.Np;
  HIPCHK(c, hipMemsetAsync(c->gws, 0, need, s));
  HIPCHK(c, launch_pack_one(pack_conv_panel((const float*)w_dev, L.wp, 0, Cout, Cin, Cin, ksize, L.Kp), s));
  if (wino_layer(c->tn, ksize, Cin)) {
    if ((rc = ensure(c, &c->wuws, &c->wuws_bytes, wino_u_floats(Cout, Cin) * sizeof(float)))) return rc;
    L.wu = (float*)c->wuws;
    HIPCHK(c, launch_pack_one(pack_wino((const float*)w_dev, L.wu, Cout, Cin, Cin, 0, c->tn.wino_prec), s));
  }
  return conv2d_launch(c, L, in_dev, B, H, W, bias_dev, scale_dev, shift_dev, relu, out_dev, ld_out, c_off, s);
}

int mgu_conv_transpose2x2_nhwc(mgu_ctx* c, const void* in_dev, int B, int H, int W, int Cin, const void* w_dev,
                               const void* bias_dev, int Cout, void* out_dev, int ld_out, int c_off, void* hip_stream) {
  if (!c) return MGU_ERR_INVALID;
  if (!in_dev || !w_dev || !out_dev || B < 1 || H < 1 || W < 1 || Cout < 1) return fail(c, MGU_ERR_INVALID, "bad convT args");
  if (Cin < 4 || (Cin & 3)) return fail(c, MGU_ERR_INVALID, "convT needs Cin %% 4 == 0 (got %d)", Cin);
  if (ld_out < c_off + Cout) return fail(c, MGU_ERR_INVALID, "ld_out %d < c_off %d + Cout %d", ld_out, c_off, Cout);
  if ((int64_t)B * H * W * 4 >= (1ll << 31)) return fail(c, MGU_ERR_INVALID, "4*B*H*W must be < 2^31");
  HIPCHK(c, hipSetDevice(c->device));
  hipStream_t s = (hipStream_t)hip_stream;
  Layer U = make_layer(MGU_DTYPE_F32, Cin, Cin, Cout, 1, true);
  const bool x3_shape = convt_x3_layer(c->tn, Cin, Cout);
  const size_t panel = (size_t)U.Np * U.Kp + 2 * (size_t)U.Np;
  int rc = ensure(c, &c->gws, &c->gws_bytes, (panel + (x3_shape ? convt_x3_floats(Cin, Cout) : 0)) * sizeof(float));
  if (rc) return rc;
  U.wp = (float*)c->gws;
  U.shift = U.wp + (size_t)U.Np * U.Kp + U.Np;
  U.wu = x3_shape ? U.wp + panel : nullptr;
  HIPCHK(c, hipMemsetAsync(c->gws, 0, panel * sizeof(float), s));
  HIPCHK(c, launch_pack_one(pack_convt_panel((const float*)w_dev, U.wp, 0, Cin, Cout, U.Kp), s));
  IgemmDesc d = layer_desc(c, U, in_dev, Cin, B, H, W, out_dev, ld_out, c_off);
  d.Hout = 2 * H, d.Wout = 2 * W;
  if (bias_dev) {
    HIPCHK(c, launch_pack_one(pack_bias_tile((const float*)bias_dev, U.shift, Cout, 4), s));
    d.shift = U.shift;
  }
  const ConvKernel k = pick_conv(d, 0);
  if (conv_reads_convt_x3(k)) HIPCHK(c, launch_pack_one(pack_convt_x3((const float*)w_dev, U.wu, Cin, Cout, 0), s));
  ProfScope ps(c, s, conv_kernel_name(k, d));
  HIPCHK(c, launch_conv(d, k, 0, s));
  c->convt_asm_launches += k == ConvKernel::ConvtX3Asm;
  return MGU_OK;
}

int mgu_maxpool2x2_nhwc(mgu_ctx* c, const void* in_dev, int ld_in, int B, int H, int W, int Cc, void* out_dev,
                        void* hip_stream) {
  if (!c) return MGU_ERR_INVALID;
  if (!in_dev || !out_dev || B < 1 || H < 2 || W < 2 || Cc < 4 || (Cc & 3) || ld_in < Cc || (ld_in & 3))
    return fail(c, MGU_ERR_INVALID, "bad maxpool args (C and ld_in must be multiples of 4, H,W >= 2)");
  HIPCHK(c, hipSetDevice(c->device));
  HIPCHK(c, launch_maxpool2(in_dev, ld_in, out_dev, 0, B, H, W, Cc, (hipStream_t)hip_stream));
  return MGU_OK;
}

int mgu_argmax_classes(mgu_ctx* c, const void* logits_dev, int64_t npix, int num_classes, int64_t* pred_dev,
                       void* hip_stream) {
  if (!c || !logits_dev || !pred_dev || num_classes < 1 || npix < 0) return fail(c, MGU_ERR_INVALID, "bad argmax args");
  HIPCHK(c, hipSetDevice(c->device));
  HIPCHK(c, launch_argmax((const float*)logits_dev, npix, num_classes, pred_dev, (hipStream_t)hip_stream));
  return MGU_OK;
}

int mgu_patch_mean(mgu_ctx* c, const void* feat_dev, int feat_dtype, int B, int H, int W, int C, int patch, void* out_dev,
                   void* hip_stream) {
  if (!c || !feat_dev || !out_dev || B < 1 || H < 1 || W < 1 || patch < 1)
    return fail(c, MGU_ERR_INVALID, "bad patch_mean args");
  if (feat_dtype != MGU_DTYPE_F32 && feat_dtype != MGU_DTYPE_BF16) return fail(c, MGU_ERR_INVALID, "unknown dtype %d", feat_dtype);
  const int vec = feat_dtype == MGU_DTYPE_BF16 ? 8 : 4;
  if ((C % vec) || C < vec || C > 256)
    return fail(c, MGU_ERR_INVALID, "patch_mean needs C %% %d == 0 and C <= 256 (got %d)", vec, C);
  HIPCHK(c, hipSetDevice(c->device));
  HIPCHK(c, launch_patch_mean(feat_dev, feat_dtype, (float*)out_dev, B, H, W, C, patch, (hipStream_t)hip_stream));
  return MGU_OK;
}

static double net_flops(const mgu_ctx* c, int B, int H, int W, bool mfma) {
  std::vector<int> hs, wsz;
  level_dims(H, W, c->depth, hs, wsz);
  double fl = 0;
  for (const Layer& L : c->layers) {
    const int h = hs[L.level], w = wsz[L.level];
    if (mfma && L.wino) fl += 2.0 * ((h + 1) / 2) * ((w + 1) / 2) * 16.0 * L.Cp * L.Cout;
    else fl += 2.0 * h * w * L.KS * L.KS * L.Cin * L.Cout * (L.convt ? 4.0 : 1.0);
  }
  return fl * B;
}

double mgu_unet_flops(mgu_ctx* c, int B, int H, int W) { return c && c->configured ? net_flops(c, B, H, W, false) : -1.0; }

double mgu_unet_mfma_flops(mgu_ctx* c, int B, int H, int W) { return c && c->configured ? net_flops(c, B, H, W, true) : -1.0; }

int mgu_profile_enable(mgu_ctx* c, int on) {
  if (!c) return MGU_ERR_INVALID;
  c->prof = on != 0;
  c->ev_used = 0;
  return MGU_OK;
}

int mgu_profile_read_kernels(mgu_ctx* c, mgu_kernel_stat* out, int cap, int* n_out) {
  if (!c || !n_out || (cap > 0 && !out)) return MGU_ERR_INVALID;
  int n = 0;
  for (int i = 0; i < c->ev_used; ++i) {
    float ms = 0;
    HIPCHK(c, hipEventSynchronize(c->ev[2 * i + 1]));
    HIPCHK(c, hipEventElapsedTime(&ms, c->ev[2 * i], c->ev[2 * i + 1]));
    const mgu_ctx::ProfRec& r = c->prec[i];
    int k = 0;
    while (k < n && strcmp(out[k].name, r.name) != 0) ++k;
    if (k == n) {
      if (n == cap) continue;
      out[n].name = r.name, out[n].ms = 0, out[n].flops_alg = 0, out[n].flops_mfma = 0, out[n].launches = 0, out[n].pipe = r.pipe;
      ++n;
    }
    out[k].ms += ms, out[k].flops_alg += r.alg, out[k].flops_mfma += r.mfma, out[k].launches += 1;
  }
  *n_out = n;
  c->ev_used = 0;
  return MGU_OK;
}

int64_t mgu_convt_asm_launches(mgu_ctx* c) { return c ? c->convt_asm_launches : 0; }

int mgu_profile_read(mgu_ctx* c, double* conv_ms, int* conv_launches, double* total_ms) {
  if (!c) return MGU_ERR_INVALID;
  if (c->ev_used == 0 || !c->ev_total[1]) return fail(c, MGU_ERR_STATE, "no profiled forward to read");
  HIPCHK(c, hipEventSynchronize(c->ev_total[1]));
  double sum = 0;
  for (int i = 0; i < c->ev_used; ++i) {
    float ms = 0;
    HIPCHK(c, hipEventSynchronize(c->ev[2 * i + 1]));
    HIPCHK(c, hipEventElapsedTime(&ms, c->ev[2 * i], c->ev[2 * i + 1]));
    sum += ms;
  }
  float tot = 0;
  HIPCHK(c, hipEventElapsedTime(&tot, c->ev_total[0], c->ev_total[1]));
  if (conv_ms) *conv_ms = sum;
  if (conv_launches) *conv_launches = c->ev_used;
  if (total_ms) *total_ms = tot;
  return MGU_OK;
}

}
```

### mingraph-unet_amd/mgunet/engine.py

```python
from __future__ import annotations

import contextlib
import ctypes as C
import math

import torch
import torch.nn as nn

from . import _lib
from ._args import check_masks, nhwc_storage
from .border import border_options
from .gat import GATNetwork, _csr_cache, _layer_forward, _LayerCall
from .losses import _LOVASZ_CLASSES, pixel_ce_options
from .patch_graph import PatchGraphConstructor
from .unet import UNet

LOSSES = ("ce", "ce+dice", "ce+lovasz", "ce+dice+lovasz")


class MinGraphUNet(nn.Module):

    def __init__(self, unet: UNet, gat: GATNetwork, patch_size: int = 16):
        super().__init__()
        self.unet, self.gat = unet, gat
        self.graph = PatchGraphConstructor(patch_size)

    def forward(self, x):
        B, _, H, W = x.shape
        X = None
        if isinstance(x, torch.Tensor) and x.is_cuda and x.dim() == 4:
            p = self.graph.patch_size
            X = torch.empty((B * ((H + p - 1) // p) * ((W + p - 1) // p), self.unet.init_features), device=x.device,
                            dtype=torch.float32)
            ctx = self.unet._context(x.device)
            _lib.call("mgu_unet_request_patch_mean", x.device, p, X, ctx=ctx)
        try:
            logits, skips, feats = self.unet(x)
        except Exception:
            if X is not None:
                _lib.call("mgu_unet_request_patch_mean", x.device, 0, None, ctx=ctx)
            raise
        if X is None:
            X = self.graph.patch_mean_features(feats[0])
        rowptr, col, gp, N, E = self.graph.batched_csr(H, W, B, x.device)
        emb = gat_forward_csr(self.gat, X, rowptr, col, gp)
        return logits, skips, feats, emb


class MinGraphUNetE2E(nn.Module):

    def __init__(self, unet: UNet, patch_gat: GATNetwork, segment_predictor, mincut, region_gat: GATNetwork, detection_head,
                 num_segments: int, patch_size: int = 16, partition: str = "predictor", foreground: int = 1):
        super().__init__()
        if partition not in ("predictor", "mincut", "expansion"):
            raise ValueError(f'partition must be "predictor", "mincut" or "expansion", got {partition!r}')
        if partition == "mincut" and num_segments != 2:
            raise ValueError(f'partition="mincut" is a binary cut: num_segments must be 2, got {num_segments}')
        if partition == "expansion" and num_segments < 2:
            raise ValueError(f'partition="expansion" needs num_segments >= 2, got {num_segments}')
        self.partition, self.foreground = partition, foreground
        self.core = MinGraphUNet(unet, patch_gat, patch_size)
        self.segment_predictor, self.mincut, self.region_gat, self.detection_head = segment_predictor, mincut, region_gat, detection_head
        self.num_segments = num_segments

    @torch.no_grad()
    def forward(self, x, images_u8=None):
        from .region import region_stage
        B, _, H, W = x.shape
        if self.partition != "predictor" and images_u8 is None:
            raise ValueError(f'partition="{self.partition}" needs the uint8 batch: forward(x, images_u8=...)')
        logits, skips, feats, emb = self.core(x)
        if self.partition == "expansion" and logits.shape[1] != self.num_segments:
            raise ValueError(f'partition="expansion" labels the patches with the U-Net\'s classes: the logits have {logits.shape[1]} classes, '
                             f"num_segments is {self.num_segments}")
        graph = self.core.graph
        nph, npw = graph.grid(H, W)
        K = self.num_segments
        ei_one = graph.edge_index(H, W, x.device)
        if getattr(self.segment_predictor, "use_gnn", False):
            ei_all = graph.edge_index(H, W, x.device, B)
            gp = graph.batched_csr(H, W, B, x.device)[2]
            seg_logits = self.segment_predictor.gnn_predictor(emb, ei_all, graph_ptr=gp)
        else:
            seg_logits = self.segment_predictor(emb)
        losses, soft, hard = self.mincut.forward_batched(emb, ei_one, B, K, seg_logits.contiguous())
        cut = None
        if self.partition == "mincut":
            cut = self.mincut.refine_patches(logits, images_u8, emb, graph.patch_size, self.foreground)
            hard = cut[0]
        elif self.partition == "expansion":
            cut = self.mincut.refine_patches_multi(logits, images_u8, emb, graph.patch_size)
            hard = cut[0]
        region_emb, fused = region_stage(emb, hard, B, K, self.region_gat, nph, npw, H, W, f_u=feats[0])
        det = self.detection_head(fused)
        out = {"logits": logits, "skips": skips, "decoder_feats": feats, "node_embeddings": emb, "loss_partition": losses.mean(),
               "soft_assignments": soft, "hard_labels": hard, "region_embeddings": region_emb, "fused": fused,
               "bboxes": det[0], "confidence": det[1]}
        if len(det) > 2:
            out["class_scores"] = det[2]
        if cut is not None:
            out["cut_labels"], out["cut_energy"] = cut[0], cut[1]
        return out


def gat_forward_csr(gat: GATNetwork, X, rowptr, col, graph_ptr):
    h = X
    for layer in gat.gat_layers:
        if layer.training and layer.dropout_rate > 0:
            raise RuntimeError("gat_forward_csr is the inference schedule on a prebuilt CSR: call .eval(), or run the layer through "
                               "GATNetwork.forward(X, edge_index) for train-mode dropout (see mgunet.gat)")
        heads = list(layer.heads)
        if heads[0].W.weight.shape[1] != h.shape[1]:
            raise ValueError("node feature width must match W")
        h = _layer_forward(_LayerCall(heads, h, layer.concat, layer.alpha, _csr_cache(layer), graph_ptr, csr=(rowptr, col)), None)
    return h


def argmax_classes(logits_nchw: torch.Tensor) -> torch.Tensor:
    _lib.require_hip(logits_nchw, "argmax_classes")
    B, Cc, H, W = logits_nchw.shape
    nhwc = nhwc_storage(logits_nchw)
    pred = torch.empty((B, H, W), device=logits_nchw.device, dtype=torch.int64)
    _lib.call("mgu_argmax_classes", logits_nchw.device, nhwc, B * H * W, Cc, pred)
    return pred


@torch.no_grad()
def segment_batch(model: UNet, images: torch.Tensor):
    logits, _, _ = model(images)
    return logits, argmax_classes(logits)


def shard_batch(global_batch: int, rank: int, world_size: int):
    base, rem = divmod(global_batch, world_size)
    lo = rank * base + min(rank, rem)
    return lo, lo + base + (1 if rank < rem else 0)


def allreduce_mean_(flat: torch.Tensor, group=None) -> float:
    import torch.distributed as dist
    if not (dist.is_available() and dist.is_initialized()):
        return 1.0
    world = dist.get_world_size(group)
    if world == 1:
        return 1.0
    if flat.is_cuda and dist.get_backend(group) == "gloo":
        host = flat.cpu()
        dist.all_reduce(host, op=dist.ReduceOp.SUM, group=group)
        flat.copy_(host)
    else:
        dist.all_reduce(flat, op=dist.ReduceOp.SUM, group=group)
    return 1.0 / world


def adam_state_dict(params, exp_avg_flat, exp_avg_sq_flat, step, lr, betas, eps, weight_decay, decoupled=False) -> dict:
    state, off = {}, 0
    for i, p in enumerate(params):
        k = p.numel()
        if step > 0:
            state[i] = {"step": torch.tensor(float(step)), "exp_avg": exp_avg_flat[off:off + k].detach().clone().view_as(p),
                        "exp_avg_sq": exp_avg_sq_flat[off:off + k].detach().clone().view_as(p)}
        off += k
    group = {"lr": lr, "betas": tuple(betas), "eps": eps, "weight_decay": weight_decay, "amsgrad": False, "maximize": False, "foreach": None,
             "capturable": False, "differentiable": False, "fused": None, "decoupled_weight_decay": bool(decoupled), "params": list(range(len(params)))}
    return {"state": state, "param_groups": [group]}


class StepLR:

    def __init__(self, trainer, step_size: int, gamma: float = 0.1):
        self.trainer, self.step_size, self.gamma = trainer, int(step_size), float(gamma)
        self.base_lr, self.last_epoch = trainer.lr, 0

    def step(self) -> None:
        self.last_epoch += 1
        self.trainer.set_lr(self.base_lr * self.gamma ** (self.last_epoch // self.step_size))

    def get_last_lr(self):
        return [self.trainer.lr]

    def state_dict(self) -> dict:
        return {"step_size": self.step_size, "gamma": self.gamma, "base_lrs": [self.base_lr], "last_epoch": self.last_epoch}

    def load_state_dict(self, sd: dict) -> None:
        self.step_size, self.gamma, self.base_lr, self.last_epoch = sd["step_size"], sd["gamma"], sd["base_lrs"][0], sd["last_epoch"]
        self.trainer.set_lr(self.base_lr * self.gamma ** (self.last_epoch // self.step_size))


class CosineAnnealingLR:

    def __init__(self, trainer, T_max: int, eta_min: float = 0.0):
        self.trainer, self.T_max, self.eta_min = trainer, int(T_max), float(eta_min)
        self.base_lr, self.last_epoch = trainer.lr, 0

    def step(self) -> None:
        m, T, lr = math, self.T_max, self.trainer.lr
        self.last_epoch += 1
        if (self.last_epoch - 1 - T) % (2 * T) == 0:
            lr = lr + (self.base_lr - self.eta_min) * (1 - m.cos(m.pi / T)) / 2
        else:
            lr = (1 + m.cos(m.pi * self.last_epoch / T)) / (1 + m.cos(m.pi * (self.last_epoch - 1) / T)) * (lr - self.eta_min) + self.eta_min
        self.trainer.set_lr(lr)

    def get_last_lr(self):
        return [self.trainer.lr]

    def state_dict(self) -> dict:
        return {"T_max": self.T_max, "eta_min": self.eta_min, "base_lrs": [self.base_lr], "last_epoch": self.last_epoch,
                "_last_lr": [self.trainer.lr]}

    def load_state_dict(self, sd: dict) -> None:
        self.T_max, self.eta_min, self.base_lr, self.last_epoch = sd["T_max"], sd["eta_min"], sd["base_lrs"][0], sd["last_epoch"]
        self.trainer.set_lr(sd["_last_lr"][0])


class ReduceLROnPlateau:

    def __init__(self, trainer, mode="min", factor=0.1, patience=10, threshold=1e-4, threshold_mode="rel", cooldown=0, min_lr=0.0,
                 eps=1e-8):
        if factor >= 1.0:
            raise ValueError("Factor should be < 1.0.")
        if mode not in ("min", "max"):
            raise ValueError(f"mode {mode} is unknown!")
        if threshold_mode not in ("rel", "abs"):
            raise ValueError(f"threshold mode {threshold_mode} is unknown!")
        self.trainer, self.mode, self.factor, self.patience = trainer, mode, float(factor), int(patience)
        self.threshold, self.threshold_mode, self.cooldown, self.min_lr, self.eps = threshold, threshold_mode, int(cooldown), float(min_lr), eps
        self.best = float("inf") if mode == "min" else -float("inf")
        self.cooldown_counter, self.num_bad_epochs, self.last_epoch = 0, 0, 0

    def _is_better(self, a, best) -> bool:
        if self.mode == "min" and self.threshold_mode == "rel":
            return a < best * (1.0 - self.threshold)
        if self.mode == "min":
            return a < best - self.threshold
        if self.threshold_mode == "rel":
            return a > best * (self.threshold + 1.0)
        return a > best + self.threshold

    def step(self, metrics) -> None:
        current = float(metrics)
        self.last_epoch += 1
        if self._is_better(current, self.best):
            self.best, self.num_bad_epochs = current, 0
        else:
            self.num_bad_epochs += 1
        if self.cooldown_counter > 0:
            self.cooldown_counter -= 1
            self.num_bad_epochs = 0
        if self.num_bad_epochs > self.patience:
            old = float(self.trainer.lr)
            new = max(old * self.factor, self.min_lr)
            if old - new > self.eps:
                self.trainer.set_lr(new)
            self.cooldown_counter, self.num_bad_epochs = self.cooldown, 0

    def get_last_lr(self):
        return [self.trainer.lr]

    _KEYS = ("mode", "factor", "patience", "threshold", "threshold_mode", "cooldown", "min_lr", "eps", "best", "cooldown_counter",
             "num_bad_epochs", "last_epoch")

    def state_dict(self) -> dict:
        return {**{k: getattr(self, k) for k in self._KEYS}, "_last_lr": [self.trainer.lr]}

    def load_state_dict(self, sd: dict) -> None:
        for k in self._KEYS:
            setattr(self, k, sd[k])
        self.trainer.set_lr(sd["_last_lr"][0])


class _DeviceStep:

    def _init_device_step(self, kind, max_grad_norm, skip_nonfinite, ema_decay, ema_warmup, always=False) -> None:
        self.optim_kind = kind
        self.max_grad_norm, self.skip_nonfinite = float(max_grad_norm), bool(skip_nonfinite)
        self.ema_decay, self.ema_warmup = float(ema_decay), bool(ema_warmup)
        self.device_step = bool(always or kind == "adamw" or self.max_grad_norm > 0.0 or self.skip_nonfinite or self.ema_decay > 0.0)
        self.ctrl = self.ema = None

    @staticmethod
    def _check_step_options(max_grad_norm, ema_decay) -> None:
        if not (float(max_grad_norm) >= 0.0 and float(max_grad_norm) != float("inf")):
            raise ValueError(f"max_grad_norm must be finite and >= 0 (0: no clipping), got {max_grad_norm}")
        if not 0.0 <= float(ema_decay) < 1.0:
            raise ValueError(f"ema_decay must lie in [0, 1) (0: no EMA), got {ema_decay}")

    def _alloc_device_step(self) -> None:
        if self.device_step:
            self.ctrl = torch.zeros(_lib.OPTIM_CTRL_BYTES // 8, device=self.device, dtype=torch.int64)
        if self.ema_decay > 0.0:
            self.ema = self.flat.detach().clone()

    def _device_optim_step(self, grad, grad_scale, ctx=None) -> None:
        d = _lib.OptimDesc(_lib.OPTIM_KINDS[self.optim_kind], self.lr, self.betas[0], self.betas[1], self.eps, self.wd,
                           getattr(self, "momentum", 0.0), grad_scale, self.max_grad_norm, int(self.skip_nonfinite), self.ema_decay,
                           int(self.ema_warmup))
        _lib.call("mgu_optim_step", self.device, C.byref(d), self.flat, grad, self.exp_avg,
                  None if self.optim_kind == "sgd" else self.exp_avg_sq, self.ema, self.ctrl, self.flat.numel(), ctx=ctx)

    def _need_record(self) -> None:
        if self.ctrl is None:
            raise RuntimeError("this optimizer steps through mgu_adam_step / mgu_sgd_step and keeps no control record: it has one with "
                               "optimizer='adamw', max_grad_norm, skip_nonfinite or ema_decay")

    @property
    def grad_norm(self) -> torch.Tensor:
        self._need_record()
        return self.ctrl.view(torch.float64)[3]

    def applied_steps(self) -> int:
        self._need_record()
        return int(self.ctrl[0])

    def skipped_steps(self) -> int:
        self._need_record()
        return int(self.ctrl[1])

    def _set_device_steps(self, step: int) -> None:
        if self.ctrl is not None:
            self.ctrl[0] = int(step)


class Trainer(_DeviceStep):

    def __init__(self, model: UNet, lr=1e-3, weight_decay=1e-4, betas=(0.9, 0.999), eps=1e-8, process_group=None, comm="auto",
                 loss="ce", dice_smooth=1.0, optimizer="adam", momentum=0.9, lovasz_per_image=False, lovasz_classes="present",
                 ce_weight=None, label_smoothing=0.0, focal_gamma=0.0, hard_fraction=1.0, hard_min_kept=0, hard_per_image=False,
                 border_w0=0.0, border_sigma=5.0, border_connectivity=2, border_separate=False, max_grad_norm=0.0,
                 skip_nonfinite=False, ema_decay=0.0, ema_warmup=False, accumulate=1):
        if optimizer not in _lib.OPTIM_KINDS:
            raise ValueError(f"unknown optimizer {optimizer!r}: 'adam', 'adamw' or 'sgd'")
        self._check_step_options(max_grad_norm, ema_decay)
        if int(accumulate) != accumulate or accumulate < 1:
            raise ValueError(f"accumulate must be an integer >= 1, got {accumulate}")
        if comm == "rccl" and accumulate > 1:
            raise ValueError('comm="rccl" exchanges each backward\'s gradient inside that backward: it cannot be combined with accumulate > 1 '
                             '(use comm="auto")')
        if loss not in LOSSES:
            raise ValueError(f"unknown loss {loss!r}: " + ", ".join(repr(k) for k in LOSSES[:-1]) + f" or {LOSSES[-1]!r}")
        if lovasz_classes not in _LOVASZ_CLASSES:
            raise ValueError(f"unknown lovasz_classes {lovasz_classes!r}: 'present' or 'all'")
        pixel_ce = pixel_ce_options(ce_weight, label_smoothing, focal_gamma, hard_fraction, hard_min_kept, hard_per_image, getattr(model, "num_classes", None))
        if border_connectivity not in (1, 2):
            raise ValueError(f"border_connectivity must be 1 (4-neighbours) or 2 (8-neighbours), got {border_connectivity}")
        w0, sigma = border_options(border_w0, border_sigma)
        if w0 > 0.0:
            border_options(w0, sigma, getattr(model, "num_classes", None), ce_weight)
        self.optimizer, self.momentum = optimizer, float(momentum)
        params = list(model.named_parameters())
        _lib.require_hip(params[0][1], "Trainer")
        self.model, self.group = model, process_group
        self.lr, self.wd, self.betas, self.eps = lr, weight_decay, betas, eps
        dev = params[0][1].device
        self.device = dev
        ctx = model._context(dev)
        n = int(_lib.lib().mgu_unet_param_count(ctx.handle))
        if n != sum(p.numel() for _, p in params):
            raise RuntimeError("parameter count mismatch between the module tree and libmgunet")
        self.flat = torch.empty(n, device=dev, dtype=torch.float32)
        self.grad = torch.zeros(n, device=dev, dtype=torch.float32)
        self.exp_avg = torch.zeros(n, device=dev, dtype=torch.float32)
        self.exp_avg_sq = torch.zeros(n, device=dev, dtype=torch.float32)
        off = 0
        for name, p in params:
            lo = int(_lib.lib().mgu_unet_param_offset(ctx.handle, name.encode()))
            if lo != off:
                raise RuntimeError(f"flat parameter layout mismatch at {name}: {lo} != {off}")
            k = p.numel()
            self.flat[off:off + k].copy_(p.detach().reshape(-1))
            p.data = self.flat[off:off + k].view_as(p)
            p.grad = self.grad[off:off + k].view_as(p)
            off += k
        model.mark_parameters_changed()
        model._slots = None
        self.step_count = 0
        self.accumulate, self._micro = int(accumulate), 0
        self.acc = torch.zeros(n, device=dev, dtype=torch.float32) if self.accumulate > 1 else None
        self._init_device_step(optimizer, max_grad_norm, skip_nonfinite, ema_decay, ema_warmup, always=self.accumulate > 1)
        self._alloc_device_step()
        self.loss_kind, self.dice_smooth = loss, float(dice_smooth)
        self.lovasz_mode, self.lovasz_per_image = _LOVASZ_CLASSES[lovasz_classes], int(bool(lovasz_per_image))
        self._lovasz = torch.zeros(1, device=dev, dtype=torch.float32)
        self.pixel_ce = None if ce_weight is None and pixel_ce == (0.0, 0.0, 1.0, 0, 0) else pixel_ce
        self.ce_weight = None if ce_weight is None else ce_weight.detach().to(device=dev, dtype=torch.float32).contiguous()
        self.border = None if w0 == 0.0 else (w0, sigma, int(border_connectivity), bool(border_separate))
        self._loss = torch.zeros(1, device=dev, dtype=torch.float32)
        self._dice = torch.zeros(1, device=dev, dtype=torch.float32)
        self._rccl = False
        if comm not in ("auto", "rccl", None):
            raise ValueError(f"unknown comm {comm!r}: 'auto', 'rccl' or None")
        self.comm = comm
        if comm == "rccl":
            self.attach_rccl()

    def _dist_world(self) -> int:
        import torch.distributed as dist
        return dist.get_world_size(self.group) if dist.is_available() and dist.is_initialized() else 1

    def _dist_backend(self):
        import torch.distributed as dist
        return dist.get_backend(self.group) if dist.is_available() and dist.is_initialized() else None

    def attach_rccl(self) -> None:
        import torch.distributed as dist
        ctx = self.model._context(self.device)
        world, rank = self._dist_world(), (dist.get_rank(self.group) if self._dist_world() > 1 else 0)
        buf = C.create_string_buffer(128)
        if rank == 0:
            _lib.call("mgu_comm_get_unique_id", None, buf)
        if world > 1:
            box = [bytes(buf.raw)]
            with torch.cuda.device(self.device):
                dist.broadcast_object_list(box, src=dist.get_global_rank(self.group, 0) if self.group is not None else 0, group=self.group)
            buf = C.create_string_buffer(box[0], 128)
        _lib.call("mgu_comm_init_rank", self.device, buf, rank, world, ctx=ctx)
        self._rccl = True
# ... 364 lines not shown
```

### mingraph-unet_amd/mgunet/gat.py

```python
from __future__ import annotations

import torch
import torch.nn as nn
import torch.nn.functional as F

from . import _lib


def coo_to_csr_device(edge_index: torch.Tensor, num_nodes: int):
    if edge_index.dim() != 2 or edge_index.shape[0] != 2:
        raise ValueError("edge_index must have shape (2, E)")
    if edge_index.dtype != torch.int64:
        raise TypeError("edge_index must be int64 (torch.long) like the reference's")
    _lib.require_hip(edge_index, "mgunet GAT")
    dev = edge_index.device
    ei = edge_index.contiguous()
    E = ei.shape[1]
    rowptr = torch.empty(num_nodes + 1, dtype=torch.int32, device=dev)
    col = torch.empty(E, dtype=torch.int32, device=dev)
    status = torch.empty(1, dtype=torch.int32, device=dev)
    _lib.call("mgu_coo_to_csr_device", dev, ei if E else None, E, num_nodes, rowptr, col if E else None, status)
    if int(status.item()):
        raise IndexError(f"edge_index values must be in [0, {num_nodes})")
    return rowptr, col


class GraphAttentionLayer(nn.Module):

    def __init__(self, in_features, out_features, dropout_rate, alpha, concat=True):
        super().__init__()
        self.in_features, self.out_features = in_features, out_features
        self.dropout_rate, self.alpha, self.concat = dropout_rate, alpha, concat
        self.W = nn.Linear(in_features, out_features, bias=False)
        self.a = nn.Linear(2 * out_features, 1, bias=False)
        self.leakyrelu = nn.LeakyReLU(self.alpha)
        self.dropout = nn.Dropout(self.dropout_rate)
        nn.init.xavier_uniform_(self.W.weight, gain=1.414)
        nn.init.xavier_uniform_(self.a.weight, gain=1.414)

    def forward(self, node_features, edge_index, graph_ptr=None):
        return _gat_layer_forward([self], node_features, edge_index, True, self.alpha, self.training,
                                  self.dropout_rate, graph_ptr, _csr_cache(self), owner=self, out_dropout=False)


def _csr_cache(mod):
    c = mod.__dict__.get("_mgu_csr_cache")
    if c is None:
        c = {}
        mod.__dict__["_mgu_csr_cache"] = c
    return c


_context, _CTX = _lib.context, _lib._CTX


def stacked_head_weights(heads, cache):
    sig = tuple((h.W.weight.data_ptr(), h.W.weight._version, h.a.weight.data_ptr(), h.a.weight._version) for h in heads)
    ent = cache.get("weights")
    if ent is None or ent[0] != sig:
        Fh = heads[0].out_features
        pad = (-Fh) % 4
        Ws = [F.pad(h.W.weight.detach(), (0, 0, 0, pad)) for h in heads]
        As = [torch.cat([F.pad(h.a.weight.detach()[:, :Fh], (0, pad)), F.pad(h.a.weight.detach()[:, Fh:], (0, pad))], 1) for h in heads]
        W = torch.cat(Ws, 0)
        a = torch.cat(As, 0).contiguous()
        if W.shape[1] % 4:
            W = F.pad(W, (0, 4 - W.shape[1] % 4))
        ent = cache["weights"] = (sig, W.contiguous(), a)
    return ent[1], ent[2]


def prepared_head_weights(heads, cache, dev, has_edges: bool):
    W, a = stacked_head_weights(heads, cache)
    sig = (cache["weights"][0], str(dev), bool(has_edges))
    ent = cache.get("prepared")
    if ent is None or ent.key != sig:
        Fh = (heads[0].out_features + 3) // 4 * 4
        ent = cache["prepared"] = _lib.Prepared("mgu_gat_prepare", dev, W, a, len(heads), Fh, W.shape[1], 1 if has_edges else 0, key=sig)
    return ent.handle


_DROPOUT = {"seed": 0x6D67756E6574, "stream": 0}


def seed_dropout(seed: int) -> None:
    _DROPOUT["seed"], _DROPOUT["stream"] = int(seed) & (2 ** 64 - 1), 0


def _rank_key() -> int:
    try:
        import torch.distributed as dist
        return dist.get_rank() if dist.is_available() and dist.is_initialized() else 0
    except Exception:
        return 0


def _draw_mask(dev, shape, p: float) -> torch.Tensor:
    m = torch.empty(shape, device=dev, dtype=torch.float32)
    _DROPOUT["stream"] += 1
    key = (_DROPOUT["seed"] + 0x9E3779B97F4A7C15 * (_rank_key() * 64 + (dev.index or 0))) & (2 ** 64 - 1)
    _lib.call("mgu_dropout_mask", dev, key, _DROPOUT["stream"], m.numel(), float(p), m)
    return m


def _gat_layer_forward(heads, X, edge_index, concat, alpha, training, dropout_rate, graph_ptr, cache, owner=None, out_dropout=True):
    _lib.require_hip(X, "mgunet GAT")
    if X.dtype != torch.float32:
        raise TypeError(f"expected float32 node features, got {X.dtype}")
    if X.dim() != 2:
        raise ValueError("node_features must be (N, F)")
    if heads[0].W.weight.shape[1] != X.shape[1]:
        raise RuntimeError(f"mat1 and mat2 shapes cannot be multiplied ({X.shape[0]}x{X.shape[1]} and "
                           f"{heads[0].W.weight.shape[1]}x{heads[0].out_features})")
    params = [t for h in heads for t in (h.W.weight, h.a.weight)]
    train = training and dropout_rate > 0
    injected = getattr(owner, "dropout_masks", None) if train and owner is not None else None
    m = _LayerCall(heads, X, concat, alpha, cache, graph_ptr, edge_index=edge_index, with_perm=injected is not None)
    if train:
        return _GatLayerFn.apply(X, m, _dropout_masks(m, float(dropout_rate), injected, out_dropout), *params)
    if torch.is_grad_enabled() and (X.requires_grad or any(t.requires_grad for t in params)):
        return _GatLayerFn.apply(X, m, None, *params)
    return _layer_forward(m, None)


class _LayerCall:

    def __init__(self, heads, X, concat, alpha, cache, graph_ptr, edge_index=None, csr=None, with_perm=False):
        self.heads, self.concat, self.alpha, self.cache, self.dev = heads, 1 if concat else 0, float(alpha), cache, X.device
        self.N, self.Fin = X.shape
        self.H, self.Fh_true = len(heads), heads[0].out_features
        self.Fh = (self.Fh_true + 3) // 4 * 4
        self.W, self.a = stacked_head_weights(heads, cache)
        if self.W.device != self.dev:
            raise RuntimeError(f"GAT parameters are on {self.W.device}, node features on {self.dev}")
        Xc = X.detach().contiguous()
        self.X = F.pad(Xc, (0, 4 - self.Fin % 4)) if self.Fin % 4 else Xc
        if csr is None:
            self.rowptr, self.col, self.perm = _cached_csr(cache, edge_index, self.N, self.dev, with_perm)
        else:
            (self.rowptr, self.col), self.perm = csr, None
        self.E = self.col.numel()
        self.gp, self.G = None, 1
        if graph_ptr is not None:
            self.gp = graph_ptr.to(device=self.dev, dtype=torch.int32).contiguous()
            self.G = self.gp.numel() - 1


def _cached_csr(cache, edge_index, N, dev, with_perm):
    key = (edge_index.data_ptr(), tuple(edge_index.shape), edge_index._version, N, str(edge_index.device))
    ent = cache.get("csr")
    if ent is None or ent[0] != key:
        rowptr, col = coo_to_csr_device(edge_index.to(dev), N)
        ent = cache["csr"] = (key, rowptr, col, edge_index)
        cache.pop("csr_t", None)
        cache.pop("perm", None)
    if not with_perm:
        return ent[1], ent[2], None
    pe = cache.get("perm")
    if pe is None or pe[0] != key:
        pe = cache["perm"] = (key, torch.sort(edge_index.to(dev)[1], stable=True).indices)
    return ent[1], ent[2], pe[1]


def _transposed_csr(cache, rowptr, col, N, dev):
    ent = cache.get("csr_t")
    if ent is None or ent[0] is not rowptr:
        E = col.numel()
        rp = torch.empty(N + 1, dtype=torch.int32, device=dev)
        eid = torch.empty(max(E, 1), dtype=torch.int32, device=dev)
        tgt = torch.empty(max(E, 1), dtype=torch.int32, device=dev)
        _lib.call("mgu_csr_transpose_device", dev, rowptr, col if E else None, E, N, rp, eid, tgt)
        ent = cache["csr_t"] = (rowptr, rp, eid, tgt)
    return ent[1], ent[2], ent[3]


def _dropout_masks(m, p, injected, out_dropout):
    N, H, E = m.N, m.H, m.E
    Fo_true = H * m.Fh_true if m.concat else m.Fh_true
    if injected is not None:
        em_coo, om = injected
        if tuple(em_coo.shape) != (H, E) or (om is not None and tuple(om.shape) != (N, Fo_true)):
            raise ValueError(f"dropout_masks must be ((heads, E) = {(H, E)}, (N, F_out) = {(N, Fo_true)} or None)")
        edge_mask = em_coo.to(device=m.dev, dtype=torch.float32)[:, m.perm].t().contiguous()
        om = om.to(device=m.dev, dtype=torch.float32) if om is not None else None
    else:
        edge_mask = _draw_mask(m.dev, (max(E, 1), H), p)
        om = _draw_mask(m.dev, (N, Fo_true), p) if out_dropout else None
    if om is not None and m.Fh != m.Fh_true:
        om = F.pad(om.view(N, -1, m.Fh_true), (0, m.Fh - m.Fh_true), value=1.0).reshape(N, -1)
    return edge_mask, om.contiguous() if om is not None else None


def _layer_forward(m, masks):
    out = torch.empty((m.N, m.H * m.Fh if m.concat else m.Fh), device=m.dev, dtype=torch.float32)
    col = m.col if m.E else None
    if masks is None:
        handle = prepared_head_weights(m.heads, m.cache, m.dev, m.E > 0)
        _lib.call("mgu_gat_layer_forward_prepared", m.dev, handle, m.X, m.N, m.rowptr, col, m.E, m.gp, m.G, m.concat, m.alpha, out)
    else:
        _lib.call("mgu_gat_layer_forward_train", m.dev, m.X, m.N, m.X.shape[1], m.rowptr, col, m.E, m.gp, m.G, m.W, m.a, m.H, m.Fh,
                  m.concat, m.alpha, *masks, out)
    if m.Fh != m.Fh_true:
        out = out.view(m.N, -1, m.Fh)[:, :, :m.Fh_true].reshape(m.N, -1).contiguous()
    return out


class _GatLayerFn(torch.autograd.Function):

    @staticmethod
    def forward(ctx_, X, m, masks, *params):
        ctx_.m, ctx_.masks = m, masks
        return _layer_forward(m, masks)

    @staticmethod
    def backward(ctx_, gout):
        m = ctx_.m
        N, Fh, Fh_true = m.N, m.Fh, m.Fh_true
        g = gout.detach().float()
        if Fh != Fh_true:
            g = F.pad(g.view(N, -1, Fh_true), (0, Fh - Fh_true)).reshape(N, -1)
        rps, eid, tgt = _transposed_csr(m.cache, m.rowptr, m.col, N, m.dev)
        dX = torch.empty_like(m.X) if ctx_.needs_input_grad[0] else None
        dW, da = torch.empty_like(m.W), torch.empty_like(m.a)
        args = (m.X, N, m.X.shape[1], m.rowptr, m.col if m.E else None, m.E, rps, eid, tgt, m.gp, m.G, m.W, m.a, m.H, Fh, m.concat, m.alpha)
        if ctx_.masks is None:
            _lib.call("mgu_gat_layer_backward", m.dev, *args, g.contiguous(), dX, dW, da)
        else:
            _lib.call("mgu_gat_layer_backward_train", m.dev, *args, *ctx_.masks, g.contiguous(), dX, dW, da)
        grads = []
        for h in range(m.H):
            grads.append(dW[h * Fh:h * Fh + Fh_true, :m.Fin].contiguous())
            grads.append(torch.cat([da[h:h + 1, :Fh_true], da[h:h + 1, Fh:Fh + Fh_true]], 1).contiguous())
        return (dX[:, :m.Fin].contiguous() if dX is not None else None, None, None, *grads)


class MultiHeadGATLayer(nn.Module):

    def __init__(self, in_features, out_features, num_heads, dropout_rate, alpha, concat=True):
        super().__init__()
        self.num_heads, self.concat = num_heads, concat
        self.alpha, self.dropout_rate = alpha, dropout_rate
        if concat:
            assert out_features % num_heads == 0, "out_features must be divisible by num_heads if concatenating"
            self.head_out_features = out_features // num_heads
        else:
            self.head_out_features = out_features
        self.heads = nn.ModuleList(
            [GraphAttentionLayer(in_features, self.head_out_features, dropout_rate, alpha) for _ in range(num_heads)])
        self.dropout = nn.Dropout(dropout_rate)

    def forward(self, node_features, edge_index, graph_ptr=None):
        return _gat_layer_forward(list(self.heads), node_features, edge_index, self.concat, self.alpha,
                                  self.training, self.dropout_rate, graph_ptr, _csr_cache(self), owner=self)


class GATNetwork(nn.Module):

    def __init__(self, node_feature_dim, hidden_dim, output_dim, num_heads, num_gat_layers=1, dropout_rate=0.1,
                 alpha=0.2):
        super().__init__()
        self.num_gat_layers = num_gat_layers
        self.gat_layers = nn.ModuleList()
        if num_gat_layers == 1:
            self.gat_layers.append(MultiHeadGATLayer(node_feature_dim, output_dim, num_heads, dropout_rate, alpha, concat=False))
        else:
            self.gat_layers.append(MultiHeadGATLayer(node_feature_dim, hidden_dim, num_heads, dropout_rate, alpha, concat=True))
            for _ in range(num_gat_layers - 2):
                self.gat_layers.append(MultiHeadGATLayer(hidden_dim * num_heads, hidden_dim, num_heads, dropout_rate, alpha, concat=True))
            self.gat_layers.append(MultiHeadGATLayer(hidden_dim * num_heads, output_dim, num_heads, dropout_rate, alpha, concat=False))

    def forward(self, node_features, edge_index, graph_ptr=None):
        h = node_features
        for layer in self.gat_layers:
            h = layer(h, edge_index, graph_ptr)
        return h
```

Baseline: 822.3.

## Feed UNet patch partial sums directly into first GAT layer

Drops the separate patch_sum_combine kernel. The first GAT layer's stmax and fused kernels now read the eight per-patch partial sums straight from the UNet workspace and reduce them inline, dividing by 256. This removes one kernel launch and one round trip of the patch-mean tensor through memory. In exchange every neighbour gather reads eight rows instead of one, the fused kernel gives up X prefetch, and its occupancy hint drops to 2 blocks per SIMD group. It only applies when Fin=32, there are 4 heads, Fout=64 and the node count is small enough.

Result: no change. 825.1, median of 6 (+0.3%).

```diff
diff --git a/include/mgunet.h b/include/mgunet.h
--- a/include/mgunet.h
+++ b/include/mgunet.h
@@ -130,6 +130,8 @@
 int mgu_unet_backward_allreduce(mgu_ctx* ctx, const void* dlogits_dev, void* flat_grad_dev, void* hip_stream);
 
 int mgu_unet_request_patch_mean(mgu_ctx* ctx, int patch, void* out_dev);
+int mgu_unet_request_patch_partials(mgu_ctx* ctx, int patch, void* out_dev);
+int mgu_unet_patch_partials(mgu_ctx* ctx, const void** psum_dev_out, int* nodes_out);
 
 int mgu_csr_transpose_device(mgu_ctx* ctx, const int32_t* rowptr_dev, const int32_t* col_dev, int64_t E, int num_nodes,
                              int32_t* rowptr_src_dev, int32_t* eid_src_dev, int32_t* tgt_of_edge_dev, void* hip_stream);
@@ -168,6 +170,10 @@
 int mgu_gat_layer_forward_prepared(mgu_ctx* ctx, const mgu_gat_weights* w, const void* X_dev, int N, const int32_t* rowptr_dev,
                                    const int32_t* col_dev, int64_t E, const int32_t* graph_ptr_dev, int num_graphs, int concat,
                                    float alpha, void* out_dev, void* hip_stream);
+int mgu_gat_takes_partials(const mgu_gat_weights* w);
+int mgu_gat_layer_forward_prepared_partials(mgu_ctx* ctx, const mgu_gat_weights* w, const void* psum_dev, int N,
+                                            const int32_t* rowptr_dev, const int32_t* col_dev, int64_t E, const int32_t* graph_ptr_dev,
+                                            int num_graphs, int concat, float alpha, void* out_dev, void* hip_stream);
 
 int mgu_ncut_edge_weights(mgu_ctx* ctx, const float* feats_dev, int N, int D, const int64_t* edge_index_dev, int64_t E,
                           float* w_dev, void* hip_stream);
diff --git a/mingraph-unet_amd/csrc/common.h b/mingraph-unet_amd/csrc/common.h
--- a/mingraph-unet_amd/csrc/common.h
+++ b/mingraph-unet_amd/csrc/common.h
@@ -29,6 +29,7 @@
   bool wino_dgrad = true;
   bool gat_fused = true;
   bool head_fused = true;
+  bool gat_partials = true;
   bool wino_asm = true;
   bool convt_asm = true;
   int fwd_groups = 2;
@@ -267,10 +268,12 @@
 hipError_t launch_gat_prep(const float* W, const float* a, float* wa, unsigned* Wx, int heads, int Fh, int Fin, hipStream_t s);
 hipError_t launch_gat_stmax(const float* x, const float* wa, int N, int Fin, int heads, const int32_t* rowptr, const int32_t* col,
                             const int32_t* gp, int G, float alpha, float* st, int32_t* node_graph, unsigned long long* gmax, int gstride,
-                            unsigned gen, hipStream_t s);
+                            unsigned gen, hipStream_t s, bool partials = false);
 hipError_t launch_gat_fused(const float* x, int Fin, const float* st, const int32_t* rowptr, const int32_t* col, const int32_t* gp, int G,
                             const unsigned long long* gmax, const unsigned* Wx, int N, int heads, int Fh, int concat, float alpha, float* out,
-                            int gstride, unsigned gen, hipStream_t s);
+                            int gstride, unsigned gen, hipStream_t s, bool partials = false);
+bool gat_partials_applicable(int Fin, int heads, int Fh);
+constexpr int GAT_PARTIALS_MAX_NODES = 512 * 32;
 hipError_t launch_gat_node_graph(const int32_t* gp, int G, int nodes_per_graph, int N, int32_t* node_graph, hipStream_t s);
 hipError_t launch_gat_edge_max(const float* st, const int32_t* rowptr, const int32_t* col, const int32_t* node_graph, int N,
                                int heads, float alpha, unsigned long long* gmax_enc, int gstride, unsigned gen, hipStream_t s);
diff --git a/mingraph-unet_amd/csrc/ctx.h b/mingraph-unet_amd/csrc/ctx.h
--- a/mingraph-unet_amd/csrc/ctx.h
+++ b/mingraph-unet_amd/csrc/ctx.h
@@ -70,6 +70,9 @@
   int pm_patch = 0;
   void* pmws = nullptr;
   size_t pmws_bytes = 0;
+  bool pm_partials = false;
+  const void* pm_part = nullptr;
+  int pm_part_nodes = 0;
   void* wuws = nullptr;
   size_t wuws_bytes = 0;
   unsigned long long* gmaxbuf = nullptr;
diff --git a/mingraph-unet_amd/csrc/gat_api.hip b/mingraph-unet_amd/csrc/gat_api.hip
--- a/mingraph-unet_amd/csrc/gat_api.hip
+++ b/mingraph-unet_amd/csrc/gat_api.hip
@@ -83,7 +83,7 @@
 }
 
 int forward_prepared(mgu_ctx* c, const mgu_gat_weights* p, const float* X, int N, const int32_t* rowptr, const int32_t* col, int64_t E,
-                     const int32_t* graph_ptr, int num_graphs, int concat, float alpha, float* out, hipStream_t s) {
+                     const int32_t* graph_ptr, int num_graphs, int concat, float alpha, float* out, hipStream_t s, bool partials = false) {
   const int heads = p->heads, Fh = p->Fh, Fin = p->Fin, HF = heads * Fh;
   unsigned long long* gmax;
   unsigned gen;
@@ -99,12 +99,15 @@
     const unsigned* wx = reinterpret_cast<const unsigned*>(p->buf + (size_t)2 * heads * Fin);
     {
       ProfScope ps(c, s, "gat_stmax_kernel");
-      HIPCHK(c, launch_gat_stmax(X, wa, N, Fin, heads, rowptr, col, graph_ptr, num_graphs, alpha, st, node_graph, gmax, c->gmax_cap, gen, s));
+      HIPCHK(c, launch_gat_stmax(X, wa, N, Fin, heads, rowptr, col, graph_ptr, num_graphs, alpha, st, node_graph, gmax, c->gmax_cap, gen, s,
+                                 partials));
     }
     ProfScope ps(c, s, "gat_fused2_kernel");
-    HIPCHK(c, launch_gat_fused(X, Fin, st, rowptr, col, graph_ptr, num_graphs, gmax, wx, N, heads, Fh, concat, alpha, out, c->gmax_cap, gen, s));
+    HIPCHK(c, launch_gat_fused(X, Fin, st, rowptr, col, graph_ptr, num_graphs, gmax, wx, N, heads, Fh, concat, alpha, out, c->gmax_cap, gen, s,
+                               partials));
     return MGU_OK;
   }
+  if (partials) return fail(c, MGU_ERR_STATE, "internal: partial sums on the gather path");
   if (p->fused) return fail(c, MGU_ERR_STATE, "internal: aggregate-first weights on the gather path");
   const size_t o_wh = cv.take((size_t)N * HF * 4), o_st = cv.take((size_t)N * 2 * heads * 4), o_ng = cv.take((size_t)N * 4);
   if ((rc = ensure(c, &c->gws, &c->gws_bytes, cv.off))) return rc;
@@ -160,6 +163,23 @@
                           (hipStream_t)hip_stream);
 }
 
+int mgu_gat_takes_partials(const mgu_gat_weights* p) { return p && p->fused && gat_partials_applicable(p->Fin, p->heads, p->Fh) ? 1 : 0; }
+
+int mgu_gat_layer_forward_prepared_partials(mgu_ctx* c, const mgu_gat_weights* p, const void* psum_dev, int N, const int32_t* rowptr_dev,
+                                            const int32_t* col_dev, int64_t E, const int32_t* graph_ptr_dev, int num_graphs, int concat,
+                                            float alpha, void* out_dev, void* hip_stream) {
+  if (!c) return MGU_ERR_INVALID;
+  if (!p || N < 0 || E < 0) return fail(c, MGU_ERR_INVALID, "bad GAT arguments");
+  if (!mgu_gat_takes_partials(p))
+    return fail(c, MGU_ERR_INVALID, "the partial-sums form needs aggregate-first weights with Fin = 32, 4 heads, Fout_head = 64 (got Fin=%d heads=%d "
+                                    "Fout=%d%s)", p->Fin, p->heads, p->Fh, p->fused ? "" : ", gather schedule");
+  if (N == 0) return MGU_OK;
+  if (!psum_dev || !rowptr_dev || !out_dev || !col_dev || E == 0) return fail(c, MGU_ERR_INVALID, "NULL buffer");
+  HIPCHK(c, hipSetDevice(c->device));
+  return forward_prepared(c, p, (const float*)psum_dev, N, rowptr_dev, col_dev, E, graph_ptr_dev, num_graphs, concat, alpha, (float*)out_dev,
+                          (hipStream_t)hip_stream, true);
+}
+
 int mgu_gat_layer_forward(mgu_ctx* c, const void* X_dev, int N, int Fin, const int32_t* rowptr_dev, const int32_t* col_dev, int64_t E,
                           const int32_t* graph_ptr_dev, int num_graphs, const void* W_dev, const void* a_dev, int heads,
                           int Fout_head, int concat, float alpha, void* out_dev, void* hip_stream) {
diff --git a/mingraph-unet_amd/csrc/gat_fused.hip b/mingraph-unet_amd/csrc/gat_fused.hip
--- a/mingraph-unet_amd/csrc/gat_fused.hip
+++ b/mingraph-unet_amd/csrc/gat_fused.hip
@@ -29,7 +29,23 @@
   return v;
 }
 
-template <int FIN, int H>
+template <int FIN, bool PART>
+__device__ __forceinline__ f32x4 gf_row(const float* __restrict__ x, const int node, const int q) {
+  if constexpr (!PART) {
+    return *reinterpret_cast<const f32x4*>(x + (size_t)node * FIN + 4 * q);
+  } else {
+    const float* p = x + (size_t)node * (8 * FIN) + 4 * q;
+    f32x4 v[8];
+#pragma unroll
+    for (int r = 0; r < 8; ++r) v[r] = *reinterpret_cast<const f32x4*>(p + r * FIN);
+    f32x4 sum = v[0];
+#pragma unroll
+    for (int r = 1; r < 8; ++r) sum += v[r];
+    return sum / 256.f;
+  }
+}
+
+template <int FIN, int H, bool PART = false>
 __global__ __launch_bounds__(256) void gat_stmax_kernel(const float* __restrict__ x, const float* __restrict__ wa, int N,
                                                         const int32_t* __restrict__ rowptr, const int32_t* __restrict__ col,
                                                         const int32_t* __restrict__ gp, int G, float alpha, float* __restrict__ st,
@@ -50,7 +66,7 @@
   }
   auto dot = [](const f32x4 a, const f32x4 b) { return fmaf(a[0], b[0], fmaf(a[1], b[1], fmaf(a[2], b[2], a[3] * b[3]))); };
   const int k0 = rowptr[nd], deg = (rowptr[nd + 1] - k0) & (live ? -1 : 0);
-  const f32x4 xv = *reinterpret_cast<const f32x4*>(x + (size_t)nd * FIN + 4 * q);
+  const f32x4 xv = gf_row<FIN, PART>(x, nd, q);
   float s[H], t[H], m[H];
 #pragma unroll
   for (int h = 0; h < H; ++h) {
@@ -79,7 +95,7 @@
 #pragma unroll
     for (int u = 0; u < EPT; ++u) {
       const int j = col[e0 + u < deg ? k0 + e0 + u : 0];
-      xs[u] = *reinterpret_cast<const f32x4*>(x + (size_t)j * FIN + 4 * q);
+      xs[u] = gf_row<FIN, PART>(x, j, q);
     }
 #pragma unroll
     for (int u = 0; u < EPT; ++u)
@@ -135,12 +151,16 @@
 
 hipError_t launch_gat_stmax(const float* x, const float* wa, int N, int Fin, int heads, const int32_t* rowptr, const int32_t* col,
                             const int32_t* gp, int G, float alpha, float* st, int32_t* node_graph, unsigned long long* gmax, int gstride,
-                            unsigned gen, hipStream_t s) {
+                            unsigned gen, hipStream_t s, bool partials) {
   if (N == 0) return hipSuccess;
   const int npw = 64 / (Fin / 4);
   const dim3 grid((N + 4 * npw - 1) / (4 * npw)), block(256);
-#define MGU_SM(FIN, H) hipLaunchKernelGGL((gat_stmax_kernel<FIN, H>), grid, block, 0, s, x, wa, N, rowptr, col, gp, G, alpha, st, node_graph, gmax, gstride, gen)
-  if (Fin == 32 && heads == 1) MGU_SM(32, 1);
+#define MGU_SM(FIN, H, ...) \
+  hipLaunchKernelGGL((gat_stmax_kernel<FIN, H, ##__VA_ARGS__>), grid, block, 0, s, x, wa, N, rowptr, col, gp, G, alpha, st, node_graph, gmax, gstride, gen)
+  if (partials) {
+    if (Fin == 32 && heads == 4) MGU_SM(32, 4, true);
+    else return hipErrorInvalidValue;
+  } else if (Fin == 32 && heads == 1) MGU_SM(32, 1);
   else if (Fin == 32 && heads == 2) MGU_SM(32, 2);
   else if (Fin == 32 && heads == 4) MGU_SM(32, 4);
   else if (Fin == 64 && heads == 1) MGU_SM(64, 1);
@@ -197,8 +217,9 @@
 }
 
 
-template <int FIN, int NT, int H>
-__global__ __launch_bounds__(256, FIN == 32 ? 3 : 2) void gat_fused2_kernel(const float* __restrict__ x, const float* __restrict__ st,
+
+template <int FIN, int NT, int H, bool PART = false>
+__global__ __launch_bounds__(256, FIN == 32 && !PART ? 3 : 2) void gat_fused2_kernel(const float* __restrict__ x, const float* __restrict__ st,
                                                          const int32_t* __restrict__ rowptr, const int32_t* __restrict__ col,
                                                          const int32_t* __restrict__ gp, int G, const gmax_t* __restrict__ gmax,
                                                          const unsigned* __restrict__ Wx, int N, int ntiles, int concat, float alpha,
@@ -261,7 +282,7 @@
   int g_cur = 0, g_hi = (gp && G > 1) ? 0 : N;
   int g_cached = -1;
   fH gm_cached = {0.f, 0.f, 0.f, 0.f};
-  constexpr bool XPF = FIN == 32;
+  constexpr bool XPF = FIN == 32 && !PART;
   struct Meta {
     int rs[PASSES], deg[PASSES], c0[PASSES];
     fH tj[PASSES];
@@ -303,7 +324,7 @@
     }
 #pragma unroll
     for (int u = 0; u < TRIP; ++u)
-      xr[u] = *reinterpret_cast<const f32x4*>(x + (size_t)cs[u] * FIN + 4 * q);
+      xr[u] = gf_row<FIN, PART>(x, cs[u], q);
     __builtin_amdgcn_wave_barrier();
   };
   auto fetch_trip0 = [&](const Meta& m) {
@@ -497,7 +518,9 @@
   return (Fin == 32 || Fin == 64) && (Fh == 32 || Fh == 64) && (heads == 1 || heads == 2 || heads == 4) && Fin <= Fh && E > 0;
 }
 
-template <int FIN, int NT, int H>
+bool gat_partials_applicable(int Fin, int heads, int Fh) { return Fin == 32 && heads == 4 && Fh == 64; }
+
+template <int FIN, int NT, int H, bool PART = false>
 static hipError_t launch_fused2_t(const float* x, const float* st, const int32_t* rowptr, const int32_t* col, const int32_t* gp, int G,
                                   const unsigned long long* gmax, const unsigned* Wx, int N, int concat, float alpha, float* out, int gstride,
                                   unsigned gen, hipStream_t s) {
@@ -510,21 +533,25 @@
   if (!resident) {
     int cus = 256, occ = 2;
     (void)hipDeviceGetAttribute(&cus, hipDeviceAttributeMultiprocessorCount, dev);
-    if (hipOccupancyMaxActiveBlocksPerMultiprocessor(&occ, reinterpret_cast<const void*>(&gat_fused2_kernel<FIN, NT, H>), 256, 0) != hipSuccess || occ < 1)
+    if (hipOccupancyMaxActiveBlocksPerMultiprocessor(&occ, reinterpret_cast<const void*>(&gat_fused2_kernel<FIN, NT, H, PART>), 256, 0) != hipSuccess || occ < 1)
       occ = 2;
     resident = std::max(8, cus * occ / 8 * 8);
     slot.store(resident, std::memory_order_relaxed);
   }
   const int nwg = std::min((ntiles + 7) / 8 * 8, resident);
-  hipLaunchKernelGGL((gat_fused2_kernel<FIN, NT, H>), dim3(nwg), dim3(256), 0, s, x, st, rowptr, col, gp, G, gmax, Wx, N, ntiles,
+  hipLaunchKernelGGL((gat_fused2_kernel<FIN, NT, H, PART>), dim3(nwg), dim3(256), 0, s, x, st, rowptr, col, gp, G, gmax, Wx, N, ntiles,
                      concat, alpha, out, gstride, gen);
   return hipGetLastError();
 }
 
 hipError_t launch_gat_fused(const float* x, int Fin, const float* st, const int32_t* rowptr, const int32_t* col, const int32_t* gp, int G,
                             const unsigned long long* gmax, const unsigned* Wx, int N, int heads, int Fh, int concat, float alpha, float* out,
-                            int gstride, unsigned gen, hipStream_t s) {
+                            int gstride, unsigned gen, hipStream_t s, bool partials) {
   if (N == 0) return hipSuccess;
+  if (partials) {
+    if (!gat_partials_applicable(Fin, heads, Fh)) return hipErrorInvalidValue;
+    return launch_fused2_t<32, 2, 4, true>(x, st, rowptr, col, gp, G, gmax, Wx, N, concat, alpha, out, gstride, gen, s);
+  }
 #define MGU_GF2(FIN, NT, H) return launch_fused2_t<FIN, NT, H>(x, st, rowptr, col, gp, G, gmax, Wx, N, concat, alpha, out, gstride, gen, s)
 #define MGU_GF2_H(FIN, NT)               \
   do {                                   \
diff --git a/mingraph-unet_amd/csrc/mgunet_api.hip b/mingraph-unet_amd/csrc/mgunet_api.hip
--- a/mingraph-unet_amd/csrc/mgunet_api.hip
+++ b/mingraph-unet_amd/csrc/mgunet_api.hip
@@ -102,6 +102,7 @@
   t.wino_asm = num("MGU_WINO_ASM", 1) > 0;
   t.convt_asm = num("MGU_CONVT_ASM", 1) > 0;
   t.head_fused = num("MGU_HEAD_FUSED", 1) > 0;
+  t.gat_partials = num("MGU_GAT_PARTIALS", 1) > 0;
   t.fwd_groups = num("MGU_FWD_GROUPS", t.fwd_groups) >= 2 ? 2 : 1;
   t.lovasz_passes = num("MGU_LOVASZ_PASSES", t.lovasz_passes) == 3 ? 3 : 4;
   *out = c;
@@ -438,6 +439,9 @@
     if (!cat_dev[i] || !feat_dev[i]) return fail(c, MGU_ERR_INVALID, "NULL cat/feat buffer %d", i);
   HIPCHK(c, hipSetDevice(c->device));
   hipStream_t s = (hipStream_t)hip_stream;
+  const bool hand_over = c->pm_out && c->pm_partials && c->tn.gat_partials && (int64_t)B * (H / 16) * (W / 16) <= GAT_PARTIALS_MAX_NODES;
+  c->pm_partials = false;
+  c->pm_part = nullptr, c->pm_part_nodes = 0;
   if (training && c->dtype != MGU_DTYPE_F32)
     return fail(c, MGU_ERR_STATE, "training runs in fp32 only (bf16 storage is an inference mode)");
   if (training) {
@@ -568,7 +572,10 @@
   const int cur_ld = c->layers[c->dec.back().conv1].Cout;
   {
     const int pm_dtype = c->dtype;
-    if (head_done) {
+    if (head_done && hand_over) {
+      c->pm_part = c->pmws, c->pm_part_nodes = B * (H / 16) * (W / 16);
+      c->pm_out = nullptr;
+    } else if (head_done) {
       ProfScope ps(c, s, "patch_sum_combine_kernel", 0, 0, -1);
       HIPCHK(c, launch_patch_sum_combine((const float*)c->pmws, (float*)c->pm_out, B * (H / 16) * (W / 16), s));
       c->pm_out = nullptr;
@@ -597,6 +604,7 @@
 int mgu_unet_request_patch_mean(mgu_ctx* c, int patch, void* out_dev) {
   if (!c) return MGU_ERR_INVALID;
   if (!c->configured) return fail(c, MGU_ERR_STATE, "not configured");
+  c->pm_partials = false;
   if (!out_dev) {
     c->pm_out = nullptr;
     return MGU_OK;
@@ -606,6 +614,19 @@
   if ((C % vec) || C > 256) return fail(c, MGU_ERR_INVALID, "patch means need init_features %% %d == 0 and <= 256 (got %d)", vec, C);
   c->pm_patch = patch;
   c->pm_out = out_dev;
+  return MGU_OK;
+}
+
+int mgu_unet_request_patch_partials(mgu_ctx* c, int patch, void* out_dev) {
+  const int rc = mgu_unet_request_patch_mean(c, patch, out_dev);
+  if (rc == MGU_OK && out_dev) c->pm_partials = true;
+  return rc;
+}
+
+int mgu_unet_patch_partials(mgu_ctx* c, const void** psum_dev_out, int* nodes_out) {
+  if (!c) return MGU_ERR_INVALID;
+  if (!psum_dev_out || !nodes_out) return fail(c, MGU_ERR_INVALID, "NULL output");
+  *psum_dev_out = c->pm_part, *nodes_out = c->pm_part_nodes;
   return MGU_OK;
 }
 
diff --git a/mingraph-unet_amd/mgunet/engine.py b/mingraph-unet_amd/mgunet/engine.py
--- a/mingraph-unet_amd/mgunet/engine.py
+++ b/mingraph-unet_amd/mgunet/engine.py
@@ -10,7 +10,7 @@
 from . import _lib
 from ._args import check_masks, nhwc_storage
 from .border import border_options
-from .gat import GATNetwork, _csr_cache, _layer_forward, _LayerCall
+from .gat import GATNetwork, _csr_cache, _layer_forward, _LayerCall, prepared_head_weights
 from .losses import _LOVASZ_CLASSES, pixel_ce_options
 from .patch_graph import PatchGraphConstructor
 from .unet import UNet
@@ -25,15 +25,26 @@
         self.unet, self.gat = unet, gat
         self.graph = PatchGraphConstructor(patch_size)
 
+    def _gat_takes_partials(self, dev, has_edges: bool) -> bool:
+        layer = self.gat.gat_layers[0]
+        W = layer.heads[0].W.weight
+        if (layer.training and layer.dropout_rate > 0) or W.device != dev or W.shape[1] != self.unet.init_features:
+            return False
+        handle = prepared_head_weights(list(layer.heads), _csr_cache(layer), dev, has_edges)
+        return bool(_lib.lib().mgu_gat_takes_partials(handle))
+
     def forward(self, x):
         B, _, H, W = x.shape
-        X = None
+        X = psum = None
+        partials = False
         if isinstance(x, torch.Tensor) and x.is_cuda and x.dim() == 4:
             p = self.graph.patch_size
             X = torch.empty((B * ((H + p - 1) // p) * ((W + p - 1) // p), self.unet.init_features), device=x.device,
                             dtype=torch.float32)
             ctx = self.unet._context(x.device)
-            _lib.call("mgu_unet_request_patch_mean", x.device, p, X, ctx=ctx)
+            rowptr, col, gp, _, _ = self.graph.batched_csr(H, W, B, x.device)
+            partials = self._gat_takes_partials(x.device, col.numel() > 0)
+            _lib.call("mgu_unet_request_patch_partials" if partials else "mgu_unet_request_patch_mean", x.device, p, X, ctx=ctx)
         try:
             logits, skips, feats = self.unet(x)
         except Exception:
@@ -42,8 +53,15 @@
             raise
         if X is None:
             X = self.graph.patch_mean_features(feats[0])
-        rowptr, col, gp, N, E = self.graph.batched_csr(H, W, B, x.device)
-        emb = gat_forward_csr(self.gat, X, rowptr, col, gp)
+            rowptr, col, gp, _, _ = self.graph.batched_csr(H, W, B, x.device)
+        elif partials:
+            ptr, nodes = C.c_void_p(), C.c_int()
+            _lib.call("mgu_unet_patch_partials", x.device, C.byref(ptr), C.byref(nodes), ctx=ctx)
+            if ptr.value:
+                if nodes.value != X.shape[0]:
+                    raise RuntimeError(f"mgu_unet_patch_partials: {nodes.value} nodes, the patch graph has {X.shape[0]}")
+                psum = ptr.value
+        emb = gat_forward_csr(self.gat, X, rowptr, col, gp, psum=psum)
         return logits, skips, feats, emb
 
 
@@ -103,7 +121,7 @@
         return out
 
 
-def gat_forward_csr(gat: GATNetwork, X, rowptr, col, graph_ptr):
+def gat_forward_csr(gat: GATNetwork, X, rowptr, col, graph_ptr, psum=None):
     h = X
     for layer in gat.gat_layers:
         if layer.training and layer.dropout_rate > 0:
@@ -112,7 +130,8 @@
         heads = list(layer.heads)
         if heads[0].W.weight.shape[1] != h.shape[1]:
             raise ValueError("node feature width must match W")
-        h = _layer_forward(_LayerCall(heads, h, layer.concat, layer.alpha, _csr_cache(layer), graph_ptr, csr=(rowptr, col)), None)
+        h = _layer_forward(_LayerCall(heads, h, layer.concat, layer.alpha, _csr_cache(layer), graph_ptr, csr=(rowptr, col)), None, psum=psum)
+        psum = None
     return h
 
 
diff --git a/mingraph-unet_amd/mgunet/gat.py b/mingraph-unet_amd/mgunet/gat.py
--- a/mingraph-unet_amd/mgunet/gat.py
+++ b/mingraph-unet_amd/mgunet/gat.py
@@ -191,12 +191,15 @@
     return edge_mask, om.contiguous() if om is not None else None
 
 
-def _layer_forward(m, masks):
+def _layer_forward(m, masks, psum=None):
     out = torch.empty((m.N, m.H * m.Fh if m.concat else m.Fh), device=m.dev, dtype=torch.float32)
     col = m.col if m.E else None
     if masks is None:
         handle = prepared_head_weights(m.heads, m.cache, m.dev, m.E > 0)
-        _lib.call("mgu_gat_layer_forward_prepared", m.dev, handle, m.X, m.N, m.rowptr, col, m.E, m.gp, m.G, m.concat, m.alpha, out)
+        if psum is not None:
+            _lib.call("mgu_gat_layer_forward_prepared_partials", m.dev, handle, psum, m.N, m.rowptr, col, m.E, m.gp, m.G, m.concat, m.alpha, out)
+        else:
+            _lib.call("mgu_gat_layer_forward_prepared", m.dev, handle, m.X, m.N, m.rowptr, col, m.E, m.gp, m.G, m.concat, m.alpha, out)
     else:
         _lib.call("mgu_gat_layer_forward_train", m.dev, m.X, m.N, m.X.shape[1], m.rowptr, col, m.E, m.gp, m.G, m.W, m.a, m.H, m.Fh,
                   m.concat, m.alpha, *masks, out)
```
